# dwang0721/SfM-GMS

Hardware: AMD Instinct MI355X
Metric: gms_filtered_image_pairs_per_sec (higher is better)
Workload: dtype i32

## Files before the change

### include/gms.h

```cpp
#ifndef MI355_GMS_H
#define MI355_GMS_H

#include <stddef.h>
#include <stdint.h>

#ifdef __cplusplus
extern "C" {
#endif

#define GMS_OK             0
#define GMS_ERR_BAD_ARG   (-1)
#define GMS_ERR_DOMAIN    (-2)
#define GMS_ERR_HIP       (-3)
#define GMS_ERR_NO_DEVICE (-4)
#define GMS_ERR_CAPACITY  (-5)
#define GMS_ERR_IO        (-7)
#define GMS_ERR_NO_MODEL  (-8)
#define GMS_ERR_NOT_RESERVED (-6)


typedef struct gms_keypoint {
    float x, y;
    float size;
    float angle;
    float response;
    int32_t octave;
    int32_t class_id;
} gms_keypoint;

typedef struct gms_dmatch {
    int32_t queryIdx;
    int32_t trainIdx;
    int32_t imgIdx;
    float   distance;
} gms_dmatch;

typedef struct gms_pair {
    int32_t frame_a;
    int32_t frame_b;
    int32_t m;
    int32_t reserved;
    int64_t match_off;
} gms_pair;

typedef struct gms_pair_result {
    int32_t n_inliers;
    int32_t best_scale;
    int32_t best_rot;
    int32_t status;
} gms_pair_result;

typedef struct gms_ctx gms_ctx;

int gms_match(const gms_keypoint* kp1, int n1, int w1, int h1,
              const gms_keypoint* kp2, int n2, int w2, int h2,
              const gms_dmatch* matches, int m,
              int with_rotation, int with_scale, double threshold_factor,
              gms_dmatch* out, int* n_out);

int gms_match_ctx(gms_ctx* ctx,
                  const gms_keypoint* kp1, int n1, int w1, int h1,
                  const gms_keypoint* kp2, int n2, int w2, int h2,
                  const gms_dmatch* matches, int m,
                  int with_rotation, int with_scale, double threshold_factor,
                  gms_dmatch* out, int* n_out, gms_pair_result* result);

int  gms_ctx_create(int device, gms_ctx** out_ctx);
int  gms_ctx_destroy(gms_ctx* ctx);
int  gms_ctx_set_stream(gms_ctx* ctx, void* hip_stream);
int  gms_ctx_synchronize(gms_ctx* ctx);
int  gms_ctx_reserve(gms_ctx* ctx, int n_pairs, int max_m, int with_rotation, int with_scale);
#define GMS_QUERY_LAST_DEALT        1
#define GMS_QUERY_LAST_SCALE_PROBE  2
#define GMS_QUERY_LAST_KPT          3
#define GMS_QUERY_LAUNCHES          4
#define GMS_QUERY_CUS               5
#define GMS_QUERY_PREFETCH_TYPE     6
#define GMS_QUERY_PREFETCH_AHEAD    7
#define GMS_QUERY_STAGGER_TICKS     8
int  gms_ctx_query(gms_ctx* ctx, int what, int64_t* value);
#define GMS_OPTION_DEAL         1
#define GMS_OPTION_SCALE_PROBE  2
int  gms_ctx_set_option(gms_ctx* ctx, int option, int value);

#define GMS_FRAME_TABLE_HEADER_BYTES 16
int64_t gms_frame_table_bytes(int64_t total_kp);
int gms_normalize_device(gms_ctx* ctx, const gms_keypoint* d_kp, const int64_t* d_frame_off,
                         const int32_t* d_wh, int n_frames, int64_t total_kp, float* d_pts);

int gms_filter_device(gms_ctx* ctx, const float* d_pts, const int64_t* d_frame_off, int n_frames,
                      const gms_pair* d_pairs, int n_pairs, int max_m,
                      const gms_dmatch* d_matches,
                      int with_rotation, int with_scale, double threshold_factor,
                      gms_dmatch* d_out, gms_pair_result* d_results, uint8_t* d_mask);

int gms_filter_host_batch(gms_ctx* ctx, const gms_keypoint* kp, const int64_t* frame_off, const int32_t* wh,
                          int n_frames, const gms_pair* pairs, int n_pairs, const gms_dmatch* matches,
                          int with_rotation, int with_scale, double threshold_factor,
                          gms_dmatch* out, gms_pair_result* results);

#define GMS_DESC_NONE      (-1)
#define GMS_DESC_HAMMING256  0
#define GMS_DESC_L2_F32X128  1
int64_t gms_bf_prepared_bytes(int desc_kind, int64_t total_desc, int n_frames);
int gms_bf_prepare_device(gms_ctx* ctx, int desc_kind, const void* d_desc, const int64_t* d_frame_off, int n_frames,
                          int64_t total_desc, void* d_prepared);
int gms_bfmatch_device(gms_ctx* ctx, int desc_kind, const void* d_desc, const void* d_prepared, int64_t total_desc,
                       const int64_t* d_frame_off, int n_frames, const gms_pair* d_pairs, int n_pairs, int max_query,
                       gms_dmatch* d_matches);

typedef struct gms_bf_result {
    int64_t n_candidates;
    int64_t n_ratio;
    int64_t n_out;
    float   d_min;
    int32_t status;
} gms_bf_result;

size_t gms_bf_select_workspace_bytes(int n_pairs, int max_rows, int64_t total_backward_rows);
int gms_bf_select_device(gms_ctx* ctx, int desc_kind, const void* d_desc, const void* d_prepared, int64_t total_desc,
                         const int64_t* d_frame_off, int n_frames, const gms_pair* d_pairs, int n_pairs, int max_rows, int cross_check,
                         double distance_coef, int max_size, void* d_ws, size_t ws_bytes, gms_dmatch* d_out, gms_bf_result* d_bf_results,
                         gms_pair_result* d_pair_results);
int gms_bf_match_select(int desc_kind, const void* desc1, int n1, const void* desc2, int n2, int cross_check, double distance_coef,
                        int max_size, gms_dmatch* out, int64_t out_cap, int64_t* n_out, gms_bf_result* result);
int gms_bf_select_host_batch(gms_ctx* ctx, int desc_kind, const void* desc, const int64_t* frame_off, int n_frames, const gms_pair* pairs,
                             int n_pairs, int cross_check, double distance_coef, int max_size, gms_dmatch* out, gms_bf_result* results);

typedef struct gms_disparity_stats {
    int64_t count;
    int64_t sum_sq;
    int32_t max_abs;
    int32_t status;
} gms_disparity_stats;
int gms_disparity_device(gms_ctx* ctx, const gms_keypoint* d_kp1, int n1, const gms_keypoint* d_kp2, int n2,
                         const gms_dmatch* d_matches, const int32_t* d_n_matches, int max_matches, int width, int height,
                         const uint8_t* d_gt, int disp_ratio, uint8_t* d_disparity, uint32_t* d_work,
                         gms_disparity_stats* d_stats);
int gms_gather_points_device(gms_ctx* ctx, const gms_keypoint* d_kp1, int n1, const gms_keypoint* d_kp2, int n2,
                             const gms_dmatch* d_matches, const int32_t* d_n_matches, int max_matches,
                             float* d_coords1, float* d_coords2, int32_t* d_status);

typedef struct gms_triangulation_stats {
    double  sum_sq_err1, sum_sq_err2;
    int64_t count, behind;
} gms_triangulation_stats;
int gms_triangulate_device(gms_ctx* ctx, const double camera[4], const double dist[5], const double P1[12], const double P2[12],
                           const float* d_coords1, const float* d_coords2, const int32_t* d_n_matches, int max_matches,
                           double* d_points3d, gms_triangulation_stats* d_stats);

typedef struct gms_pose {
    double  R[9], t[3];
    int32_t n_good, which;
} gms_pose;
int gms_recover_pose_device(gms_ctx* ctx, const double E[9], const double camera[4], const float* d_coords1, const float* d_coords2,
                            const int32_t* d_n_matches, int max_matches, const uint8_t* d_in_mask, gms_pose* d_pose,
                            uint8_t* d_out_mask);

typedef struct gms_camera {
    double fx, fy, cx, cy;
    double k1, k2, p1, p2, k3;
} gms_camera;
typedef struct gms_two_view {
    double  E[9];
    double  R[9], t[3];
    double  sum_sq_err1, sum_sq_err2;
    int64_t n_finite, n_behind;
    int32_t n_points;
    int32_t n_ransac;
    int32_t ransac_iters;
    int32_t n_pose;
    int32_t pose_which;
    int32_t n_triangulated;
    int32_t status;
    int32_t reserved;
} gms_two_view;
int gms_gather_points_batch_device(gms_ctx* ctx, const gms_keypoint* d_kp, const int64_t* d_frame_off, int n_frames,
                                   const gms_pair* d_pairs, int n_pairs, int max_m, const gms_dmatch* d_filtered,
                                   const gms_pair_result* d_results, float* d_coords1, float* d_coords2, gms_two_view* d_tv);
int gms_find_essential_batch_device(gms_ctx* ctx, const gms_camera* camera, double prob, double threshold, int max_iters,
                                    const gms_pair* d_pairs, int n_pairs, const float* d_coords1, const float* d_coords2,
                                    uint8_t* d_mask, gms_two_view* d_tv);
int gms_recover_pose_batch_device(gms_ctx* ctx, const gms_camera* camera, int use_in_mask, const gms_pair* d_pairs, int n_pairs,
                                  const float* d_coords1, const float* d_coords2, uint8_t* d_mask, gms_two_view* d_tv);
int gms_triangulate_batch_device(gms_ctx* ctx, const gms_camera* camera, const gms_pair* d_pairs, int n_pairs,
                                 const float* d_coords1, const float* d_coords2, const uint8_t* d_mask, double* d_points3d,
                                 gms_two_view* d_tv);
int gms_two_view_batch_device(gms_ctx* ctx, const gms_camera* camera, double prob, double threshold, int max_iters,
                              const gms_keypoint* d_kp, const int64_t* d_frame_off, int n_frames, const gms_pair* d_pairs, int n_pairs,
                              int max_m, const gms_dmatch* d_filtered, const gms_pair_result* d_results, float* d_coords1,
                              float* d_coords2, uint8_t* d_mask, double* d_points3d, gms_two_view* d_tv);
int gms_disparity_batch_device(gms_ctx* ctx, const gms_keypoint* d_kp, const int64_t* d_frame_off, const int32_t* d_wh, int n_frames,
                               const gms_pair* d_pairs, int n_pairs, int max_m, const gms_dmatch* d_filtered,
                               const gms_pair_result* d_results, const uint8_t* d_gt, int64_t gt_stride, int disp_ratio,
                               uint8_t* d_disparity, int64_t map_stride, uint32_t* d_work, gms_disparity_stats* d_stats);

#define GMS_SFM_SKIPPED 1
typedef struct gms_sfm_plan_entry {
    int32_t registers;
    int32_t link;
    int32_t role;
    int32_t depth;
} gms_sfm_plan_entry;
typedef struct gms_sfm_view {
    double  R[9], t[3];
    int32_t registered;
    int32_t pair;
} gms_sfm_view;
typedef struct gms_sfm_pair_reg {
    double  r, S;
    int32_t n_links;
    int32_t depth, link, role;
    int32_t status;
    int32_t reserved;
} gms_sfm_pair_reg;
typedef struct gms_sfm_summary {
    int64_t n_tracks;
    int64_t n_points;
    int64_t n_multi;
    int32_t n_registered;
    int32_t n_ok_pairs;
} gms_sfm_summary;
int gms_sfm_plan(const gms_pair* pairs, int n_pairs, int n_frames, int root, gms_sfm_plan_entry* plan);
size_t gms_sfm_register_workspace_bytes(int n_frames, int n_pairs, int64_t total_kp, int64_t total_matches);
int gms_sfm_register_device(gms_ctx* ctx, const int64_t* d_frame_off, int n_frames, int64_t total_kp, const gms_pair* d_pairs,
                            const gms_sfm_plan_entry* d_plan, int n_pairs, int max_m, int64_t total_matches, const gms_dmatch* d_filtered,
                            const uint8_t* d_mask, const double* d_points3d, const gms_two_view* d_tv, int root, int min_links,
                            void* d_ws, size_t ws_bytes, gms_sfm_view* d_views, gms_sfm_pair_reg* d_reg, double* d_points_world,
                            int32_t* d_track, int64_t cloud_cap, double* d_cloud, int32_t* d_cloud_id, int32_t* d_cloud_obs,
                            int32_t* d_cloud_est, double* d_cloud_spread, gms_sfm_summary* d_summary);
int gms_sfm_register(const int64_t* frame_off, int n_frames, const gms_pair* pairs, int n_pairs, const gms_dmatch* filtered,
                     const uint8_t* mask, const double* points3d, const gms_two_view* tv, int root, int min_links, gms_sfm_view* views,
                     gms_sfm_pair_reg* reg, double* points_world, int32_t* track, int64_t cloud_cap, double* cloud, int32_t* cloud_id,
                     int32_t* cloud_obs, int32_t* cloud_est, double* cloud_spread, gms_sfm_summary* summary);

typedef struct gms_sfm_ba_params {
    double  lambda0, cg_tol, ftol, huber_px;
    int32_t n_iters, n_cg, retriangulate;
    int32_t reserved;
} gms_sfm_ba_params;
typedef struct gms_sfm_ba_summary {
// ... 265 lines not shown
```

### sfm-gms_amd/api.py

```python
import ctypes as C

import numpy as np

from .capi import load_library
from .types import (BF_RESULT_DTYPE, DMATCH_DTYPE, LOGOS_DICT_RESULT_DTYPE, KEYPOINT_DTYPE, PAIR_DTYPE, RESULT_DTYPE, GMS_OK, GMS_ERR_CAPACITY,
                    GmsError, SFM_PAIR_REG_DTYPE, SFM_PLAN_DTYPE, SFM_SUMMARY_DTYPE, SFM_VIEW_DTYPE, TWO_VIEW_DTYPE, concat_frames, desc_layout,
                    portrait_params, stereo_bm_params, stereo_sgm_params, GMS_ERR_BAD_ARG, RECTIFY_PLAN_DTYPE, STEREO_SGM_DENSE, RectifyPlan,
                    make_camera, rectify_plan_records)


def _as(arr, dtype, name):
    a = np.ascontiguousarray(arr)
    if a.dtype != dtype:
        raise TypeError(f"{name} must have dtype {dtype}, got {a.dtype}")
    return a


def _check(rc, lib, what):
    if rc != GMS_OK:
        msg = lib.gms_error_string(rc).decode()
        if rc == -3:
            msg += f" (hipError {lib.gms_last_hip_error()})"
        raise GmsError(rc, f"{what}: {msg}")


class GmsContext:

    def __init__(self, device=0):
        self._lib = load_library()
        h = C.c_void_p()
        _check(self._lib.gms_ctx_create(int(device), C.byref(h)), self._lib, "gms_ctx_create")
        self._h = h
        self.device = int(device)

    def close(self):
        if getattr(self, "_h", None):
            self._lib.gms_ctx_destroy(self._h)
            self._h = None

    def __del__(self):
        try:
            self.close()
        except Exception:
            pass

    def __enter__(self):
        return self

    def __exit__(self, *exc):
        self.close()

    @property
    def max_matches(self):
        return int(self._lib.gms_max_matches())

    def set_stream(self, hip_stream_handle):
        _check(self._lib.gms_ctx_set_stream(self._h, C.c_void_p(hip_stream_handle or 0)), self._lib, "set_stream")

    def synchronize(self):
        _check(self._lib.gms_ctx_synchronize(self._h), self._lib, "synchronize")

    def set_option(self, option, value):
        _check(self._lib.gms_ctx_set_option(self._h, int(option), int(value)), self._lib, "gms_ctx_set_option")

    def query(self, what):
        v = C.c_int64(0)
        _check(self._lib.gms_ctx_query(self._h, int(what), C.byref(v)), self._lib, "gms_ctx_query")
        return int(v.value)

    def match(self, size1, size2, keypoints1, keypoints2, matches1to2, withRotation=False, withScale=False,
              thresholdFactor=6.0, return_result=False):
        kp1 = _as(keypoints1, KEYPOINT_DTYPE, "keypoints1")
        kp2 = _as(keypoints2, KEYPOINT_DTYPE, "keypoints2")
        mt = _as(matches1to2, DMATCH_DTYPE, "matches1to2")
        out = np.empty(max(len(mt), 1), dtype=DMATCH_DTYPE)
        n_out = C.c_int(0)
        res = np.zeros(1, dtype=RESULT_DTYPE)
        rc = self._lib.gms_match_ctx(self._h, kp1.ctypes.data, len(kp1), int(size1[0]), int(size1[1]),
                                     kp2.ctypes.data, len(kp2), int(size2[0]), int(size2[1]),
                                     mt.ctypes.data, len(mt), int(bool(withRotation)), int(bool(withScale)),
                                     float(thresholdFactor), out.ctypes.data, C.byref(n_out), res.ctypes.data)
        _check(rc, self._lib, "gms_match_ctx")
        kept = out[: n_out.value].copy()
        return (kept, res[0]) if return_result else kept

    def filter_host_batch(self, keypoints_per_frame, sizes, pairs, matches, withRotation=False, withScale=False,
                          thresholdFactor=6.0, out=None, results=None):
        if isinstance(keypoints_per_frame, tuple):
            kp, frame_off = keypoints_per_frame
            n_kp = len(kp)
            kp = _as(kp, KEYPOINT_DTYPE, "keypoints") if n_kp else np.zeros(1, dtype=KEYPOINT_DTYPE)
            frame_off = np.ascontiguousarray(frame_off, dtype=np.int64)
            n_frames = len(np.asarray(sizes).reshape(-1, 2))
            if (frame_off.shape != (n_frames + 1,) or frame_off[0] != 0 or (np.diff(frame_off) < 0).any()
                    or frame_off[-1] > n_kp):
                raise ValueError("frame_off: one offset per frame and one more, from 0, never decreasing, the last at most len(keypoints)")
        else:
            kp, frame_off = concat_frames([_as(k, KEYPOINT_DTYPE, "keypoints") for k in keypoints_per_frame])
            kp = kp if len(kp) else np.zeros(1, dtype=KEYPOINT_DTYPE)
            n_frames = len(frame_off) - 1
        wh = np.ascontiguousarray(np.asarray(sizes, dtype=np.int32).reshape(-1, 2))
        if wh.shape[0] != n_frames:
            raise ValueError("one (width, height) per frame")
        pairs = _as(pairs, PAIR_DTYPE, "pairs")
        mt = _as(matches, DMATCH_DTYPE, "matches")
        if out is None:
            out = np.zeros(max(len(mt), 1), dtype=DMATCH_DTYPE)
        if results is None:
            results = np.zeros(max(len(pairs), 1), dtype=RESULT_DTYPE)
        if (out.dtype != DMATCH_DTYPE or results.dtype != RESULT_DTYPE or len(out) < len(mt) or len(results) < len(pairs)
                or not out.flags["C_CONTIGUOUS"] or not results.flags["C_CONTIGUOUS"]):
            raise ValueError("out / results: contiguous DMATCH_DTYPE / RESULT_DTYPE arrays of at least len(matches) / len(pairs)")
        rc = self._lib.gms_filter_host_batch(self._h, kp.ctypes.data, frame_off.ctypes.data, wh.ctypes.data, n_frames,
                                             pairs.ctypes.data, len(pairs), mt.ctypes.data, int(bool(withRotation)),
                                             int(bool(withScale)), float(thresholdFactor), out.ctypes.data, results.ctypes.data)
        _check(rc, self._lib, "gms_filter_host_batch")
        return out[: len(mt)], results[: len(pairs)]

    def reserve(self, n_pairs, max_m, withRotation=False, withScale=False):
        _check(self._lib.gms_ctx_reserve(self._h, int(n_pairs), int(max_m), int(bool(withRotation)), int(bool(withScale))),
               self._lib, "gms_ctx_reserve")

    def frame_table_bytes(self, total_kp):
        return int(self._lib.gms_frame_table_bytes(int(total_kp)))

    def normalize_device(self, d_kp, d_frame_off, d_wh, n_frames, total_kp, d_pts):
        _check(self._lib.gms_normalize_device(self._h, d_kp, d_frame_off, d_wh, int(n_frames), int(total_kp), d_pts),
               self._lib, "gms_normalize_device")

    def filter_device(self, d_pts, d_frame_off, n_frames, d_pairs, n_pairs, max_m, d_matches, d_out, d_results,
                      d_mask=None, withRotation=False, withScale=False, thresholdFactor=6.0):
        _check(self._lib.gms_filter_device(self._h, d_pts, d_frame_off, int(n_frames), d_pairs, int(n_pairs),
                                           int(max_m), d_matches, int(bool(withRotation)), int(bool(withScale)),
                                           float(thresholdFactor), d_out, d_results, d_mask or None),
               self._lib, "gms_filter_device")

    def bf_prepared_bytes(self, desc_kind, total_desc, n_frames):
        return int(self._lib.gms_bf_prepared_bytes(int(desc_kind), int(total_desc), int(n_frames)))

    def bf_prepare_device(self, desc_kind, d_desc, d_frame_off, n_frames, total_desc, d_prepared):
        _check(self._lib.gms_bf_prepare_device(self._h, int(desc_kind), d_desc, d_frame_off, int(n_frames), int(total_desc),
                                               d_prepared or None), self._lib, "gms_bf_prepare_device")

    def bfmatch_device(self, desc_kind, d_desc, d_prepared, total_desc, d_frame_off, n_frames, d_pairs, n_pairs, max_query,
                       d_matches):
        _check(self._lib.gms_bfmatch_device(self._h, int(desc_kind), d_desc, d_prepared or None, int(total_desc), d_frame_off,
                                            int(n_frames), d_pairs, int(n_pairs), int(max_query), d_matches),
               self._lib, "gms_bfmatch_device")

    def bf_select_workspace_bytes(self, n_pairs, max_rows, total_backward_rows):
        return int(self._lib.gms_bf_select_workspace_bytes(int(n_pairs), int(max_rows), int(total_backward_rows)))

    def bf_select_device(self, desc_kind, d_desc, d_prepared, total_desc, d_frame_off, n_frames, d_pairs, n_pairs, max_rows, cross_check,
                         distance_coef, max_size, d_ws, ws_bytes, d_out, d_bf_results, d_pair_results=None):
        _check(self._lib.gms_bf_select_device(self._h, int(desc_kind), d_desc or None, d_prepared or None, int(total_desc), d_frame_off,
                                              int(n_frames), d_pairs, int(n_pairs), int(max_rows), int(bool(cross_check)),
                                              float(distance_coef), int(max_size), d_ws, int(ws_bytes), d_out, d_bf_results,
                                              d_pair_results or None), self._lib, "gms_bf_select_device")

    def disparity_device(self, d_kp1, n1, d_kp2, n2, d_matches, d_n_matches, max_matches, width, height, d_gt, disp_ratio,
                         d_disparity, d_work, d_stats):
        _check(self._lib.gms_disparity_device(self._h, d_kp1, int(n1), d_kp2, int(n2), d_matches, d_n_matches, int(max_matches),
                                              int(width), int(height), d_gt or None, int(disp_ratio), d_disparity, d_work,
                                              d_stats), self._lib, "gms_disparity_device")

    def gather_points_device(self, d_kp1, n1, d_kp2, n2, d_matches, d_n_matches, max_matches, d_coords1, d_coords2, d_status):
        _check(self._lib.gms_gather_points_device(self._h, d_kp1, int(n1), d_kp2, int(n2), d_matches, d_n_matches,
                                                  int(max_matches), d_coords1, d_coords2, d_status),
               self._lib, "gms_gather_points_device")

    def triangulate_device(self, camera, dist, P1, P2, d_coords1, d_coords2, d_n_matches, max_matches, d_points3d, d_stats):
        cam = np.ascontiguousarray(camera, dtype=np.float64).reshape(4)
        dc = None if dist is None else np.ascontiguousarray(dist, dtype=np.float64).reshape(5)
        p1 = np.ascontiguousarray(P1, dtype=np.float64).reshape(12)
        p2 = np.ascontiguousarray(P2, dtype=np.float64).reshape(12)
        _check(self._lib.gms_triangulate_device(self._h, cam.ctypes.data, None if dc is None else dc.ctypes.data, p1.ctypes.data,
                                                p2.ctypes.data, d_coords1, d_coords2, d_n_matches, int(max_matches), d_points3d,
                                                d_stats), self._lib, "gms_triangulate_device")

    def recover_pose_device(self, E, camera, d_coords1, d_coords2, d_n_matches, max_matches, d_in_mask, d_pose, d_out_mask):
        e = np.ascontiguousarray(E, dtype=np.float64).reshape(9)
        cam = np.ascontiguousarray(camera, dtype=np.float64).reshape(4)
        _check(self._lib.gms_recover_pose_device(self._h, e.ctypes.data, cam.ctypes.data, d_coords1, d_coords2, d_n_matches,
                                                 int(max_matches), d_in_mask, d_pose, d_out_mask), self._lib, "gms_recover_pose_device")

    def gather_points_batch_device(self, d_kp, d_frame_off, n_frames, d_pairs, n_pairs, max_m, d_filtered, d_results, d_coords1,
                                   d_coords2, d_tv):
        _check(self._lib.gms_gather_points_batch_device(self._h, d_kp, d_frame_off, int(n_frames), d_pairs, int(n_pairs), int(max_m),
                                                        d_filtered, d_results, d_coords1, d_coords2, d_tv),
               self._lib, "gms_gather_points_batch_device")

    def find_essential_batch_device(self, camera, d_pairs, n_pairs, d_coords1, d_coords2, d_mask, d_tv, prob=0.999, threshold=1.0,
                                    max_iters=1000):
        _check(self._lib.gms_find_essential_batch_device(self._h, camera.ctypes.data, float(prob), float(threshold), int(max_iters),
                                                         d_pairs, int(n_pairs), d_coords1, d_coords2, d_mask, d_tv),
               self._lib, "gms_find_essential_batch_device")

    def recover_pose_batch_device(self, camera, d_pairs, n_pairs, d_coords1, d_coords2, d_mask, d_tv, use_in_mask=True):
        _check(self._lib.gms_recover_pose_batch_device(self._h, camera.ctypes.data, int(bool(use_in_mask)), d_pairs, int(n_pairs),
                                                       d_coords1, d_coords2, d_mask, d_tv), self._lib, "gms_recover_pose_batch_device")

    def triangulate_batch_device(self, camera, d_pairs, n_pairs, d_coords1, d_coords2, d_mask, d_points3d, d_tv):
        _check(self._lib.gms_triangulate_batch_device(self._h, camera.ctypes.data, d_pairs, int(n_pairs), d_coords1, d_coords2,
                                                      d_mask or None, d_points3d, d_tv), self._lib, "gms_triangulate_batch_device")

    def two_view_batch_device(self, camera, d_kp, d_frame_off, n_frames, d_pairs, n_pairs, max_m, d_filtered, d_results, d_coords1,
                              d_coords2, d_mask, d_points3d, d_tv, prob=0.999, threshold=1.0, max_iters=1000):
        _check(self._lib.gms_two_view_batch_device(self._h, camera.ctypes.data, float(prob), float(threshold), int(max_iters), d_kp,
                                                   d_frame_off, int(n_frames), d_pairs, int(n_pairs), int(max_m), d_filtered, d_results,
                                                   d_coords1, d_coords2, d_mask, d_points3d, d_tv), self._lib, "gms_two_view_batch_device")

    def disparity_batch_device(self, d_kp, d_frame_off, d_wh, n_frames, d_pairs, n_pairs, max_m, d_filtered, d_results, d_gt, gt_stride,
                               disp_ratio, d_disparity, map_stride, d_work, d_stats):
        _check(self._lib.gms_disparity_batch_device(self._h, d_kp, d_frame_off, d_wh, int(n_frames), d_pairs, int(n_pairs), int(max_m),
                                                    d_filtered, d_results, d_gt or None, int(gt_stride), int(disp_ratio), d_disparity,
                                                    int(map_stride), d_work, d_stats), self._lib, "gms_disparity_batch_device")

    def sfm_register_workspace_bytes(self, n_frames, n_pairs, total_kp, total_matches):
        return int(self._lib.gms_sfm_register_workspace_bytes(int(n_frames), int(n_pairs), int(total_kp), int(total_matches)))

    def sfm_register_device(self, d_frame_off, n_frames, total_kp, d_pairs, d_plan, n_pairs, max_m, total_matches, d_filtered, d_mask,
                            d_points3d, d_tv, root, min_links, d_ws, ws_bytes, d_views, d_reg, d_points_world, d_track, cloud_cap, d_cloud,
                            d_cloud_id, d_cloud_obs, d_cloud_est, d_cloud_spread, d_summary):
        _check(self._lib.gms_sfm_register_device(self._h, d_frame_off, int(n_frames), int(total_kp), d_pairs, d_plan, int(n_pairs), int(max_m),
                                                 int(total_matches), d_filtered, d_mask, d_points3d, d_tv, int(root), int(min_links), d_ws,
                                                 int(ws_bytes), d_views, d_reg, d_points_world, d_track, int(cloud_cap), d_cloud, d_cloud_id,
                                                 d_cloud_obs, d_cloud_est, d_cloud_spread, d_summary), self._lib, "gms_sfm_register_device")

    def sfm_ba_workspace_bytes(self, n_frames, n_pairs, total_kp, cloud_cap):
        return int(self._lib.gms_sfm_ba_workspace_bytes(int(n_frames), int(n_pairs), int(total_kp), int(cloud_cap)))

    def sfm_ba_device(self, camera, params, d_kp, d_frame_off, n_frames, total_kp, d_pairs, n_pairs, total_matches, d_filtered, d_mask, d_views,
                      d_reg, d_track, cloud_cap, d_cloud, d_cloud_id, d_reg_summary, d_ws, ws_bytes, d_views_out, d_cloud_out, d_track_status,
                      d_summary):
        _check(self._lib.gms_sfm_ba_device(self._h, None if camera is None else camera.ctypes.data, None if params is None else params.ctypes.data,
                                           d_kp, d_frame_off, int(n_frames), int(total_kp), d_pairs, int(n_pairs), int(total_matches), d_filtered,
                                           d_mask, d_views, d_reg, d_track, int(cloud_cap), d_cloud, d_cloud_id, d_reg_summary, d_ws, int(ws_bytes),
                                           d_views_out, d_cloud_out, d_track_status, d_summary), self._lib, "gms_sfm_ba_device")

    def detect_workspace_bytes(self, width, height, n_images, max_keypoints):
        return int(self._lib.gms_detect_workspace_bytes(int(width), int(height), int(n_images), int(max_keypoints)))

    def detect_batch_device(self, d_images, n_images, width, height, threshold, max_keypoints, d_ws, ws_bytes, d_kp, d_desc, d_counts):
        _check(self._lib.gms_detect_batch_device(self._h, d_images, int(n_images), int(width), int(height), int(threshold), int(max_keypoints),
                                                 d_ws, int(ws_bytes), d_kp, d_desc, d_counts), self._lib, "gms_detect_batch_device")

    def describe_device(self, d_image, width, height, d_kp, n, d_ws, ws_bytes, d_desc, d_status):
        _check(self._lib.gms_describe_device(self._h, d_image, int(width), int(height), d_kp, int(n), d_ws, int(ws_bytes), d_desc, d_status),
               self._lib, "gms_describe_device")

    def pyramid_level_sizes(self, width, height, n_levels):
        n_levels = int(n_levels)
        ww, hh = np.zeros(max(n_levels, 1), np.int32), np.zeros(max(n_levels, 1), np.int32)
        n = self._lib.gms_pyramid_level_sizes(int(width), int(height), n_levels, ww.ctypes.data, hh.ctypes.data)
        _check(min(n, 0), self._lib, "gms_pyramid_level_sizes")
        return [(int(ww[l]), int(hh[l])) for l in range(n)]

    def detect_pyramid_workspace_bytes(self, width, height, n_images, max_keypoints, n_levels):
        return int(self._lib.gms_detect_pyramid_workspace_bytes(int(width), int(height), int(n_images), int(max_keypoints), int(n_levels)))

    def detect_pyramid_batch_device(self, d_images, n_images, width, height, threshold, max_keypoints, n_levels, d_ws, ws_bytes, d_kp, d_desc,
                                    d_counts, d_level_counts):
        _check(self._lib.gms_detect_pyramid_batch_device(self._h, d_images, int(n_images), int(width), int(height), int(threshold),
                                                         int(max_keypoints), int(n_levels), d_ws, int(ws_bytes), d_kp, d_desc, d_counts,
                                                         d_level_counts), self._lib, "gms_detect_pyramid_batch_device")

    def pyramid_build_device(self, d_images, n_images, width, height, n_levels, d_levels, levels_bytes):
        _check(self._lib.gms_pyramid_build_device(self._h, d_images, int(n_images), int(width), int(height), int(n_levels), d_levels,
                                                  int(levels_bytes)), self._lib, "gms_pyramid_build_device")

    def detect_pyramid_grad_workspace_bytes(self, width, height, n_images, max_keypoints, n_levels):
        return int(self._lib.gms_detect_pyramid_grad_workspace_bytes(int(width), int(height), int(n_images), int(max_keypoints), int(n_levels)))

    def detect_pyramid_grad_batch_device(self, d_images, n_images, width, height, threshold, max_keypoints, n_levels, d_ws, ws_bytes, d_kp,
                                         d_desc, d_counts, d_level_counts, d_rows128):
        _check(self._lib.gms_detect_pyramid_grad_batch_device(self._h, d_images, int(n_images), int(width), int(height), int(threshold),
                                                              int(max_keypoints), int(n_levels), d_ws, int(ws_bytes), d_kp, d_desc, d_counts,
                                                              d_level_counts, d_rows128), self._lib, "gms_detect_pyramid_grad_batch_device")

    def describe_grad_device(self, d_image, width, height, d_kp, n, d_ws, ws_bytes, d_rows128, d_status):
        _check(self._lib.gms_describe_grad_device(self._h, d_image, int(width), int(height), d_kp, int(n), d_ws, int(ws_bytes), d_rows128,
                                                  d_status), self._lib, "gms_describe_grad_device")
# ... 712 lines not shown
```

### sfm-gms_amd/capi.py

```python
import ctypes as C
import os

_HERE = os.path.dirname(os.path.abspath(__file__))

vp, i32, i64, u64, sz, dbl, cstr, P = C.c_void_p, C.c_int, C.c_int64, C.c_uint64, C.c_size_t, C.c_double, C.c_char_p, C.POINTER

SIGNATURES = {
    "gms_match": (i32, [vp, i32, i32, i32, vp, i32, i32, i32, vp, i32, i32, i32, dbl, vp, P(i32)]),
    "gms_match_ctx": (i32, [vp, vp, i32, i32, i32, vp, i32, i32, i32, vp, i32, i32, i32, dbl, vp, P(i32), vp]),
    "gms_ctx_create": (i32, [i32, P(vp)]),
    "gms_ctx_destroy": (i32, [vp]),
    "gms_ctx_set_stream": (i32, [vp, vp]),
    "gms_ctx_synchronize": (i32, [vp]),
    "gms_ctx_reserve": (i32, [vp, i32, i32, i32, i32]),
    "gms_ctx_query": (i32, [vp, i32, P(i64)]),
    "gms_ctx_set_option": (i32, [vp, i32, i32]),
    "gms_frame_table_bytes": (i64, [i64]),
    "gms_normalize_device": (i32, [vp, vp, vp, vp, i32, i64, vp]),
    "gms_filter_device": (i32, [vp, vp, vp, i32, vp, i32, i32, vp, i32, i32, dbl, vp, vp, vp]),
    "gms_filter_host_batch": (i32, [vp, vp, vp, vp, i32, vp, i32, vp, i32, i32, dbl, vp, vp]),
    "gms_bf_prepared_bytes": (i64, [i32, i64, i32]),
    "gms_bf_prepare_device": (i32, [vp, i32, vp, vp, i32, i64, vp]),
    "gms_bfmatch_device": (i32, [vp, i32, vp, vp, i64, vp, i32, vp, i32, i32, vp]),
    "gms_disparity_device": (i32, [vp, vp, i32, vp, i32, vp, vp, i32, i32, i32, vp, i32, vp, vp, vp]),
    "gms_gather_points_device": (i32, [vp, vp, i32, vp, i32, vp, vp, i32, vp, vp, vp]),
    "gms_triangulate_device": (i32, [vp, vp, vp, vp, vp, vp, vp, vp, i32, vp, vp]),
    "gms_recover_pose_device": (i32, [vp, vp, vp, vp, vp, vp, i32, vp, vp, vp]),
    "gms_gather_points_batch_device": (i32, [vp, vp, vp, i32, vp, i32, i32, vp, vp, vp, vp, vp]),
    "gms_find_essential_batch_device": (i32, [vp, vp, dbl, dbl, i32, vp, i32, vp, vp, vp, vp]),
    "gms_recover_pose_batch_device": (i32, [vp, vp, i32, vp, i32, vp, vp, vp, vp]),
    "gms_triangulate_batch_device": (i32, [vp, vp, vp, i32, vp, vp, vp, vp, vp]),
    "gms_two_view_batch_device": (i32, [vp, vp, dbl, dbl, i32, vp, vp, i32, vp, i32, i32, vp, vp, vp, vp, vp, vp, vp]),
    "gms_disparity_batch_device": (i32, [vp, vp, vp, vp, i32, vp, i32, i32, vp, vp, vp, i64, i32, vp, i64, vp, vp]),
    "gms_sfm_plan": (i32, [vp, i32, i32, i32, vp]),
    "gms_sfm_register_workspace_bytes": (sz, [i32, i32, i64, i64]),
    "gms_sfm_register_device": (i32, [vp, vp, i32, i64, vp, vp, i32, i32, i64, vp, vp, vp, vp, i32, i32, vp, sz, vp, vp, vp, vp, i64, vp, vp, vp,
                                      vp, vp, vp]),
    "gms_sfm_register": (i32, [vp, i32, vp, i32, vp, vp, vp, vp, i32, i32, vp, vp, vp, vp, i64, vp, vp, vp, vp, vp, vp]),
    "gms_sfm_ba_workspace_bytes": (sz, [i32, i32, i64, i64]),
    "gms_sfm_ba_device": (i32, [vp, vp, vp, vp, vp, i32, i64, vp, i32, i64, vp, vp, vp, vp, vp, i64, vp, vp, vp, vp, sz, vp, vp, vp, vp]),
    "gms_sfm_ba": (i32, [vp, vp, vp, vp, i32, vp, i32, vp, vp, vp, vp, vp, i64, vp, vp, i64, vp, vp, vp, vp]),
    "gms_dataset_write": (i32, [cstr, vp]),
    "gms_dataset_read": (i32, [cstr, vp]),
    "gms_dataset_free": (None, [vp]),
    "gms_max_matches": (i32, []),
    "gms_last_hip_error": (i32, []),
    "gms_error_string": (cstr, [i32]),
    "gms_version": (cstr, []),
    "gms_selftest_threshold": (i32, [vp, vp, vp, vp, dbl, i32, vp]),
    "gms_selftest_five_point": (i32, [vp, vp, i32, vp, vp]),
    "gms_detect_workspace_bytes": (sz, [i32, i32, i32, i32]),
    "gms_detect_batch_device": (i32, [vp, vp, i32, i32, i32, i32, i32, vp, sz, vp, vp, vp]),
    "gms_describe_device": (i32, [vp, vp, i32, i32, vp, i32, vp, sz, vp, vp]),
    "gms_logos_match": (i32, [vp, i32, vp, i32, vp, vp, vp, i64, P(i64), vp]),
    "gms_logos_table_bytes": (i64, [i64, i32, i32]),
    "gms_logos_workspace_bytes": (sz, [i64, i32, i64]),
    "gms_logos_prepare_device": (i32, [vp, vp, vp, i32, i64, vp, i32, vp, sz, vp]),
    "gms_logos_filter_device": (i32, [vp, vp, vp, i32, vp, sz, vp, vp, vp]),
    "gms_logos_words_device": (i32, [vp, i32, vp, i64, vp, i32, vp]),
    "gms_logos_host_batch": (i32, [vp, vp, vp, i32, vp, i32, vp, i32, vp, vp]),
    "gms_bf_select_workspace_bytes": (sz, [i32, i32, i64]),
    "gms_bf_select_device": (i32, [vp, i32, vp, vp, i64, vp, i32, vp, i32, i32, i32, dbl, i32, vp, sz, vp, vp, vp]),
    "gms_bf_match_select": (i32, [i32, vp, i32, vp, i32, i32, dbl, i32, vp, i64, P(i64), vp]),
    "gms_bf_select_host_batch": (i32, [vp, i32, vp, vp, i32, vp, i32, i32, dbl, i32, vp, vp]),
    "gms_stereo_bm_workspace_bytes": (sz, [i32, i32, i32, vp]),
    "gms_stereo_bm_device": (i32, [vp, vp, vp, vp, i32, i32, i32, i32, vp, sz, vp, vp]),
    "gms_stereo_bm_normalize_device": (i32, [vp, vp, i32, i32, i32, vp]),
    "gms_stereo_bm": (i32, [vp, vp, vp, i32, i32, i32, vp, vp, vp]),
    "gms_stereo_sgm_workspace_bytes": (sz, [i32, i32, i32, vp]),
    "gms_stereo_sgm_device": (i32, [vp, vp, vp, vp, i32, i32, i32, i32, vp, sz, vp, vp]),
    "gms_stereo_sgm": (i32, [vp, vp, vp, i32, i32, i32, vp, vp, vp]),
    "gms_portrait_workspace_bytes": (sz, [i32, i32, i32, vp]),
    "gms_portrait_device": (i32, [vp, vp, vp, vp, i32, i32, i32, i32, i32, vp, sz, vp, vp, vp, vp]),
    "gms_median_blur_device": (i32, [vp, vp, i32, i32, i32, i32, i32, i32, vp]),
    "gms_portrait": (i32, [vp, vp, vp, i32, i32, vp, vp, vp, vp]),
    "gms_portrait_profile_device": (i32, [vp, vp, vp, vp, i32, i32, i32, i32, i32, vp, sz, vp, vp, vp, vp, vp]),
    "gms_median_blur": (i32, [vp, i32, i32, i32, i32, vp]),
    "gms_resize_device": (i32, [vp, vp, i32, i32, i32, i32, i32, vp, i32, i32, i32]),
    "gms_warp_affine_device": (i32, [vp, vp, i32, i32, i32, i32, i32, vp, i32, vp, i32, i32, i32]),
    "gms_rotation_matrix_2d": (i32, [dbl, dbl, dbl, dbl, vp]),
    "gms_resize": (i32, [vp, i32, i32, i32, vp, i32, i32]),
    "gms_warp_affine": (i32, [vp, i32, i32, i32, vp, vp, i32, i32]),
    "gms_img_rotate": (i32, [vp, i32, i32, i32, dbl, vp]),
    "gms_rectify_plan_host": (i32, [vp, vp, vp, i32, i32, i32, i32, vp]),
    "gms_rectify_plan_device": (i32, [vp, vp, vp, i32, i32, i32, i32, i32, vp]),
    "gms_rectify_q": (i32, [vp, vp]),
    "gms_rectify_device": (i32, [vp, vp, vp, i32, i32, i32, i32, i32, vp, i32, i32, vp, i32, i32, i32, vp]),
    "gms_rectify": (i32, [vp, vp, i32, vp, i32, i32, i32, vp, vp]),
    "gms_undistort": (i32, [vp, vp, i32, i32, i32, vp]),
    "gms_dense_cloud_workspace_bytes": (sz, [i32, i32, i32]),
    "gms_dense_cloud_device": (i32, [vp, vp, vp, vp, i32, i32, i32, i32, i32, vp, i32, i32, vp, vp, vp, i32, vp, sz, i32, vp, vp, vp, vp]),
    "gms_dense_pairs_workspace_bytes": (sz, [i32, i32, i32, i32, i32, i32, vp]),
    "gms_dense_pairs_device": (i32, [vp, vp, vp, vp, vp, i32, i32, i32, i32, vp, i32, i32, i32, vp, vp, vp, i32, vp, sz, vp, vp, vp, vp, vp, vp,
                                     i32, vp, vp, vp, vp]),
    "gms_dense_pair": (i32, [vp, vp, vp, vp, i32, i32, i32, vp, vp, i32, i32, i32, vp, vp, vp, vp, vp, vp, i32, vp, vp, vp, vp]),
    "gms_chess_candidates_workspace_bytes": (sz, [i32, i32, i32]),
    "gms_chess_candidates_device": (i32, [vp, vp, i32, i32, i32, i32, vp, sz, vp, vp]),
    "gms_corner_subpix_device": (i32, [vp, vp, i32, i32, i32, vp, vp, i32, i32, i32, dbl, vp]),
    "gms_find_chessboard_corners": (i32, [vp, i32, i32, i32, i32, vp, vp]),
    "gms_order_chessboard": (i32, [vp, i32, i32, vp, vp]),
    "gms_corner_subpix": (i32, [vp, i32, i32, vp, i32, i32, i32, dbl, vp]),
    "gms_calibrate_camera": (i32, [vp, vp, vp, i32, i32, i32, vp, vp, vp, vp, vp]),
    "gms_pyramid_level_sizes": (i32, [i32, i32, i32, vp, vp]),
    "gms_detect_pyramid_workspace_bytes": (sz, [i32, i32, i32, i32, i32]),
    "gms_detect_pyramid_batch_device": (i32, [vp, vp, i32, i32, i32, i32, i32, i32, vp, sz, vp, vp, vp, vp]),
    "gms_pyramid_build_device": (i32, [vp, vp, i32, i32, i32, i32, vp, sz]),
    "gms_detect_pyramid_grad_workspace_bytes": (sz, [i32, i32, i32, i32, i32]),
    "gms_detect_pyramid_grad_batch_device": (i32, [vp, vp, i32, i32, i32, i32, i32, i32, vp, sz, vp, vp, vp, vp, vp]),
    "gms_describe_grad_device": (i32, [vp, vp, i32, i32, vp, i32, vp, sz, vp, vp]),
    "gms_detect_dog_workspace_bytes": (sz, [i32, i32, i32, i32, i32]),
    "gms_detect_dog_batch_device": (i32, [vp, vp, i32, i32, i32, i32, i32, i32, vp, sz, vp, vp, vp, vp, vp]),
    "gms_dog_candidates_device": (i32, [vp, vp, i32, i32, i32, i32, vp]),
    "gms_detect_dog_refined_workspace_bytes": (sz, [i32, i32, i32, i32, i32]),
    "gms_detect_dog_refined_batch_device": (i32, [vp, vp, i32, i32, i32, i32, i32, i32, vp, sz, vp, vp, vp, vp, vp]),
    "gms_dog_offsets_device": (i32, [vp, vp, i32, i32, i32, i32, vp]),
    "gms_bgr_to_gray_device": (i32, [vp, vp, i32, i32, i32, vp]),
    "gms_detect_pack_device": (i32, [vp, vp, vp, vp, vp, i32, i32, vp, vp, vp, vp]),
    "gms_logos_dict_workspace_bytes": (sz, [i32, i64, i32, i32, i32, i32]),
    "gms_logos_dict_train_device": (i32, [vp, i32, vp, vp, i32, i64, i32, i32, i32, u64, vp, sz, vp, vp, vp]),
    "gms_logos_dict_train": (i32, [i32, vp, vp, i32, i32, i32, i32, u64, vp, vp, vp]),
}
EXPORTED_SYMBOLS = list(SIGNATURES)

_lib = None


def library_path():
    return os.path.join(_HERE, "csrc", "libgms_hip.so")


def load_library():
    global _lib
    if _lib is not None:
        return _lib
    path = library_path()
    if not os.path.exists(path):
        raise ImportError(f"{path} not found: the HIP extension is not built "
                          f"(run `python -c 'import __graft_entry__ as g; g.build()'`)")
    try:
        import torch
    except ImportError:
        pass
    lib = C.CDLL(path)
    for name, (restype, argtypes) in SIGNATURES.items():
        fn = getattr(lib, name)
        fn.restype, fn.argtypes = restype, argtypes
    _lib = lib
    return lib
```

### sfm-gms_amd/csrc/gms_capi.cpp

```cpp
#include <hip/hip_runtime.h>

#include <algorithm>
#include <atomic>
#include <cmath>
#include <condition_variable>
#include <cstdio>
#include <cstddef>
#include <cstdlib>
#include <cstring>
#include <mutex>
#include <new>
#include <thread>
#include <vector>

#include "block_layout.h"
#include "copy_pool.h"
#include "gms.h"
#include "gms_kernels.h"
#include "logos_batch.h"
#include "logos_dict_core.h"
#include "portrait_core.h"
#include "stereo_bm_core.h"
#include "sfm_ba_core.h"
#include "sfm_register_core.h"
#include "stereo_sgm_core.h"
#include "twoview_core.h"
#include "rectify_core.h"
#include "warp_core.h"
#include "calib_core.h"

static_assert(sizeof(gms_keypoint) == 28, "gms_keypoint must match cv::KeyPoint (stride 0x1c)");
static_assert(sizeof(gms_dmatch) == 16, "gms_dmatch must match cv::DMatch (stride 0x10)");
static_assert(sizeof(gms_pair) == 24, "gms_pair layout");
static_assert(sizeof(gms_pair_result) == 16, "gms_pair_result layout");
static_assert(sizeof(gms_two_view) == 232 && sizeof(gms_camera) == 72, "two-view records");

static thread_local int t_last_hip = 0;
namespace gms {
void record_hip_error(int e) { t_last_hip = e; }
}
#ifdef GMS_PHASE_TIMING
static unsigned long long* g_diag = nullptr;
extern "C" int gms_diag_set_buffer(void* d_buf) { g_diag = (unsigned long long*)d_buf; return 0; }
#endif

#define GMS_HIP(call)                         \
    do {                                      \
        hipError_t e_ = (call);               \
        if (e_ != hipSuccess) {               \
            t_last_hip = (int)e_;             \
            return GMS_ERR_HIP;               \
        }                                     \
    } while (0)
#define GMS_TRY(call)                \
    do {                             \
        const int rc_ = (call);      \
        if (rc_ != GMS_OK) return rc_; \
    } while (0)

namespace {

struct Knobs {
    bool dense_on = true, band_on = true, stream_on = true;
    int probe_nibble = 16;
    bool probe_nibble_set = false;
    int stagger_us = -1, deal = -1, scale_probe = -1, check_pairs = -1;
    int prefetch_type = 3, prefetch_ahead = 0;
    size_t band_ws_budget = (size_t)4 << 30;
};
const Knobs& knobs()
{
    static const Knobs k = [] {
        Knobs v;
        if (const char* e = std::getenv("GMS_DENSE")) v.dense_on = std::atoi(e) != 0;
        if (const char* e = std::getenv("GMS_BAND")) v.band_on = std::atoi(e) != 0;
        if (const char* e = std::getenv("GMS_STREAM")) v.stream_on = std::atoi(e) != 0;
        if (const char* e = std::getenv("GMS_PROBE_NIBBLE")) { v.probe_nibble = (int)std::strtol(e, nullptr, 0) & 24; v.probe_nibble_set = true; }
        if (const char* e = std::getenv("GMS_STAGGER_US")) v.stagger_us = std::atoi(e);
        if (const char* e = std::getenv("GMS_DEAL")) v.deal = std::atoi(e) != 0 ? 1 : 0;
        if (const char* e = std::getenv("GMS_SCALE_PROBE")) v.scale_probe = std::atoi(e) != 0 ? 1 : 0;
        if (const char* e = std::getenv("GMS_CHECK_PAIRS")) v.check_pairs = std::atoi(e) != 0 ? 1 : 0;
        if (const char* e = std::getenv("GMS_PREFETCH")) {
            v.prefetch_type = std::atoi(e);
            if (const char* comma = std::strchr(e, ',')) v.prefetch_ahead = std::atoi(comma + 1);
        }
        if (const char* e = std::getenv("GMS_BAND_WS_BYTES")) {
            const long long b = std::atoll(e);
            if (b > 0) v.band_ws_budget = (size_t)b;
        }
        return v;
    }();
    return k;
}

void right_grids(int rw[5], int rh[5])
{
    const double ratio[5] = {1.0, 1.0 / 2, 1.0 / std::sqrt(2.0), std::sqrt(2.0), 2.0};
    for (int s = 0; s < 5; ++s) {
        rw[s] = (int)std::lrint(gms::kLeftW * ratio[s]);
        rh[s] = (int)std::lrint(gms::kLeftH * ratio[s]);
    }
}

inline hipError_t device_alloc(void** p, size_t bytes) { return hipMalloc(p, bytes); }
inline hipError_t pinned_alloc(void** p, size_t bytes) { return hipHostMalloc(p, bytes, hipHostMallocDefault); }

template <hipError_t (*Alloc)(void**, size_t), hipError_t (*Free)(void*), size_t kMin>
struct GrowBuf {
    void* p = nullptr;
    size_t cap = 0;
    hipError_t reserve(size_t bytes)
    {
        if (bytes <= cap) return hipSuccess;
        release();
        const size_t want = bytes < kMin ? kMin : bytes + bytes / 4;
        const hipError_t e = Alloc(&p, want);
        if (e == hipSuccess) cap = want;
        return e;
    }
    void release()
    {
        if (p) (void)Free(p);
        p = nullptr;
        cap = 0;
    }
};
using DevBuf = GrowBuf<device_alloc, hipFree, 4096>;
using PinBuf = GrowBuf<pinned_alloc, hipHostFree, 65536>;

struct WsNeed {
    size_t partial = 0, big = 0, band = 0;
    size_t slice = 0, per_pair = 0;
    int kpt = 0, mcap = 0;
    bool stream = false;
};

}

struct Lane {
    hipStream_t stream = nullptr;
    PinBuf hin, hout;
    DevBuf din, dout;
    hipEvent_t ev_res = nullptr, ev_out = nullptr;
};

struct gms_ctx {
    int device = 0;
    hipStream_t own_stream = nullptr;
    hipStream_t stream = nullptr;
    std::mutex mu;
    DevBuf aux, big_ws, band_ws, partial_ws, pose_ws;
    uint32_t* verdict = nullptr;
    unsigned dense_launches = 0;
    int use_dealt = 0, use_probe = 0x1D | (16 << 8), last_dealt = 0, last_probe = 0, last_kpt = 0, last_stagger_ticks = 0;
    hipEvent_t verdict_event = nullptr;
    bool verdict_pending = false;
    unsigned filter_launches = 0;
    uint32_t overflow_seen = 0;
    int stream_penalty = 0;
    int opt_deal = -1, opt_probe = -1;
    DevBuf probe_stats;
    unsigned scale_launches = 0;
    hipEvent_t ws_event = nullptr;
    hipStream_t ws_stream = nullptr;
    bool ws_pending = false;
    Lane lane[3];
    gms::CopyPool* pool = nullptr;
    DevBuf tab_kp, tab_pts, tab_small;
    int n_cus = 256;
};

namespace {

int plan_workspace(const gms_ctx* c, int n_pairs, int max_m, bool rot, bool scale, bool need_mask_ws, bool allow_stream, WsNeed* w)
{
    *w = WsNeed();
    w->kpt = gms::filter_pick_kpt(max_m);
    if (w->kpt) {
        if (scale && knobs().dense_on) w->partial = (size_t)n_pairs * gms::kPartialStrideDw * 4;
        return GMS_OK;
    }
    if (max_m > gms::kBigMaxMatches) return GMS_ERR_CAPACITY;
    w->mcap = gms::big_mcap(max_m);
    const int n_wg = n_pairs < c->n_cus ? n_pairs : c->n_cus;
    w->big = (size_t)n_wg * gms::big_ws_stride_dwords(w->mcap) * 4;
    if (knobs().band_on) {
        gms::FilterParams p{};
        p.with_rotation = rot;
        p.with_scale = scale;
        right_grids(p.right_w, p.right_h);
        w->stream = knobs().stream_on && max_m <= gms::stream_max_matches() && allow_stream;
        w->per_pair = w->stream ? std::max(gms::stream_ws_bytes_per_pair(p, w->mcap, need_mask_ws), scale ? (size_t)0 : gms::stream_dense_ws_bytes_per_pair(w->mcap))
                                : (!rot && !scale) ? gms::band_ws_bytes_per_pair(w->mcap, need_mask_ws)
                                                   : gms::tile_ws_bytes_per_pair(p, w->mcap, need_mask_ws);
        size_t slice = knobs().band_ws_budget / w->per_pair;
        if (slice < 1) slice = 1;
        if (slice > (size_t)n_pairs) slice = (size_t)n_pairs;
        w->slice = slice;
        w->band = slice * w->per_pair;
    }
    return GMS_OK;
}

int grow_workspace(gms_ctx* c, const WsNeed& w, hipStream_t st)
{
    if (w.partial <= c->partial_ws.cap && w.big <= c->big_ws.cap && w.band <= c->band_ws.cap) return GMS_OK;
    hipStreamCaptureStatus cs = hipStreamCaptureStatusNone;
    if (hipStreamIsCapturing(st, &cs) == hipSuccess && cs != hipStreamCaptureStatusNone) return GMS_ERR_NOT_RESERVED;
    GMS_HIP(hipStreamSynchronize(st));
    if (c->ws_pending) {
        GMS_HIP(hipEventSynchronize(c->ws_event));
        c->ws_pending = false;
    }
    GMS_HIP(c->partial_ws.reserve(w.partial));
    GMS_HIP(c->big_ws.reserve(w.big));
    GMS_HIP(c->band_ws.reserve(w.band));
    return GMS_OK;
}

int grow_pose_ws(gms_ctx* c, size_t bytes, hipStream_t st)
{
    if (bytes <= c->pose_ws.cap) return GMS_OK;
    hipStreamCaptureStatus cs = hipStreamCaptureStatusNone;
    if (hipStreamIsCapturing(st, &cs) == hipSuccess && cs != hipStreamCaptureStatusNone) return GMS_ERR_NOT_RESERVED;
    GMS_HIP(hipStreamSynchronize(st));
    GMS_HIP(hipDeviceSynchronize());
    GMS_HIP(c->pose_ws.reserve(bytes));
    return GMS_OK;
}

int filter_launch(gms_ctx* c, hipStream_t st, const float* d_pts, const int64_t* d_frame_off, int n_frames,
                  const gms_pair* d_pairs, int n_pairs, int max_m, const gms_dmatch* d_matches,
                  int with_rotation, int with_scale, double threshold_factor,
                  gms_dmatch* d_out, gms_pair_result* d_results, uint8_t* d_mask, bool validate_pairs = true)
{
    if (n_pairs < 0 || max_m < 0 || n_frames < 0) return GMS_ERR_BAD_ARG;
    if (n_pairs == 0) return GMS_OK;
    if (!d_frame_off || !d_pairs || !d_results) return GMS_ERR_BAD_ARG;
    if (max_m > 0 && (!d_matches || !d_out || !d_pts)) return GMS_ERR_BAD_ARG;
    hipStreamCaptureStatus cs = hipStreamCaptureStatusNone;
    const bool capturing = hipStreamIsCapturing(st, &cs) == hipSuccess && cs != hipStreamCaptureStatusNone;
    if (gms::filter_pick_kpt(max_m) == 0 && !capturing) {
        const uint32_t now = ((volatile uint32_t*)c->verdict)[2];
        if (now != c->overflow_seen) {
            c->overflow_seen = now;
            c->stream_penalty = 64;
        } else if (c->stream_penalty > 0) {
            --c->stream_penalty;
        }
    }
    WsNeed w;
    GMS_TRY(plan_workspace(c, n_pairs, max_m, with_rotation != 0, with_scale != 0, d_mask == nullptr, c->stream_penalty == 0, &w));
    GMS_TRY(grow_workspace(c, w, st));
    const bool uses_ws = w.partial || w.big || w.band;
    if (uses_ws && !capturing && c->ws_pending && c->ws_stream != st) GMS_HIP(hipStreamWaitEvent(st, c->ws_event, 0));

    gms::FilterParams p{};
    const int kpt = w.kpt;
    p.table_slots = kpt ? gms::filter_table_slots(kpt) : 0;
    p.region_shift = kpt ? gms::filter_region_shift(kpt) : 0;
    p.pts = reinterpret_cast<const float2*>(reinterpret_cast<const char*>(d_pts) + gms::kTableHeaderBytes);
    p.frame_off = d_frame_off;
    p.n_frames = n_frames;
    p.pairs = d_pairs;
    p.n_pairs = n_pairs;
    p.stagger_blocks = c->n_cus;
    p.prefetch_type = knobs().prefetch_type;
    p.prefetch_ahead = knobs().prefetch_ahead > 0 ? knobs().prefetch_ahead : c->n_cus;
    p.matches = d_matches;
    p.out = d_out;
    p.results = d_results;
    p.mask = d_mask;
    p.with_rotation = with_rotation ? 1 : 0;
    p.with_scale = with_scale ? 1 : 0;
    p.threshold_factor = threshold_factor;
    p.pair_flags = nullptr;
    p.partial = nullptr;
    p.dealt = 0;
    right_grids(p.right_w, p.right_h);
    p.dense = (knobs().dense_on && !with_scale) ? 1 : 0;
    if (c->verdict_pending && !capturing && hipEventQuery(c->verdict_event) == hipSuccess) {
        c->use_dealt = c->verdict[0] != 0u ? 1 : 0;
        c->use_probe = (int)c->verdict[1];
        c->verdict_pending = false;
    }
    const int force_deal = c->opt_deal >= 0 ? c->opt_deal : knobs().deal, force_probe = c->opt_probe >= 0 ? c->opt_probe : knobs().scale_probe;
    const bool scales_matrix = kpt && with_scale && knobs().dense_on;
    p.dealt = ((p.dense || scales_matrix) && kpt && (force_deal >= 0 ? force_deal != 0 : c->use_dealt != 0)) ? 1 : 0;
    const bool scales_on_matrix = with_scale && knobs().dense_on;
    p.stagger_ticks = 0;
    if (n_pairs >= 4 * p.stagger_blocks && kpt && max_m >= 2048) {
        const double us10k = knobs().stagger_us >= 0 ? (double)knobs().stagger_us : (scales_on_matrix ? 0.0 : p.dense ? 16.0 : 72.0);
        p.stagger_ticks = (int)(us10k * 100.0 * max_m / 10000.0);
    }
#ifdef GMS_PHASE_TIMING
    p.diag = g_diag;
#endif
    p.probe_scales = 0;
    p.probe_stats = nullptr;
    {
        void* dflag = nullptr;
        p.overflow_events = hipHostGetDevicePointer(&dflag, c->verdict, 0) == hipSuccess ? (uint32_t*)dflag + 2 : nullptr;
    }
    if (kpt && with_scale) {
        const bool measuring = force_probe < 0 && !capturing && (c->scale_launches++ & 15u) == 0u;
        const int all = 0x1D | (24 << 8);
        const int mask = force_probe >= 0 ? (force_probe != 0 ? 0x1D | (knobs().probe_nibble << 8) : 0) : (measuring ? all : c->use_probe);
        p.probe_scales = mask & 0x1D;
        p.probe_nibble = (mask >> 8) & 24 & (knobs().probe_nibble_set ? knobs().probe_nibble : 24);
        p.probe_stats = measuring ? (uint32_t*)c->probe_stats.p : nullptr;
    }
    if (kpt && with_scale && knobs().dense_on) {
        p.partial = (uint32_t*)c->partial_ws.p;
        GMS_HIP(gms::launch_filter_scales(p, kpt, n_pairs, st));
        if (!capturing && p.probe_stats == nullptr && (c->dense_launches++ & 15u) == 0u) {
            void* dflag = nullptr;
            GMS_HIP(hipHostGetDevicePointer(&dflag, c->verdict, 0));
            GMS_HIP(gms::launch_order_probe(p, (uint32_t*)dflag, st));
            GMS_HIP(hipEventRecord(c->verdict_event, st));
            c->verdict_pending = true;
        }
        if (p.probe_stats != nullptr) {
            void* dflag = nullptr;
            GMS_HIP(hipHostGetDevicePointer(&dflag, c->verdict, 0));
            GMS_HIP(gms::launch_probe_verdict(p.probe_stats, (uint32_t*)dflag + 1, st));
            GMS_HIP(hipEventRecord(c->verdict_event, st));
            c->verdict_pending = true;
        }
    } else if (kpt) {
        GMS_HIP(gms::launch_filter(p, kpt, n_pairs, st));
        if (p.dense && !capturing && (c->dense_launches++ & 15u) == 0u) {
            void* dflag = nullptr;
            GMS_HIP(hipHostGetDevicePointer(&dflag, c->verdict, 0));
            GMS_HIP(gms::launch_order_probe(p, (uint32_t*)dflag, st));
            GMS_HIP(hipEventRecord(c->verdict_event, st));
            c->verdict_pending = true;
        }
    } else if (knobs().band_on) {
        const bool plain = !with_rotation && !with_scale;
        for (int s0 = 0; s0 < n_pairs; s0 += (int)w.slice) {
            gms::FilterParams ps = p;
            ps.pairs = d_pairs + s0;
            ps.results = d_results + s0;
            ps.n_pairs = (n_pairs - s0 < (int)w.slice) ? n_pairs - s0 : (int)w.slice;
            const uint32_t* flags = nullptr;
            if (w.stream && (with_scale || ps.n_pairs < c->n_cus)) GMS_HIP(gms::launch_filter_stream(ps, w.mcap, c->band_ws.p, &flags, st));
            else if (w.stream) GMS_HIP(gms::launch_filter_stream_dense(ps, w.mcap, c->band_ws.p, &flags, st));
            else if (plain) GMS_HIP(gms::launch_filter_band(ps, w.mcap, c->band_ws.p, &flags, st));
            else GMS_HIP(gms::launch_filter_tiles(ps, w.mcap, c->band_ws.p, &flags, st));
            ps.pair_flags = flags;
            const int wg = ps.n_pairs < c->n_cus ? ps.n_pairs : c->n_cus;
            GMS_HIP(gms::launch_filter_big(ps, w.mcap, wg, (uint32_t*)c->big_ws.p, st));
        }
    } else {
        const int n_wg = n_pairs < c->n_cus ? n_pairs : c->n_cus;
        GMS_HIP(gms::launch_filter_big(p, w.mcap, n_wg, (uint32_t*)c->big_ws.p, st));
    }
    c->last_dealt = p.dealt;
    c->last_probe = p.probe_scales | (p.probe_scales ? p.probe_nibble << 8 : 0);
    c->last_kpt = kpt;
    c->last_stagger_ticks = p.stagger_ticks;
    if (validate_pairs && n_pairs > 1 && !capturing && knobs().check_pairs != 0 && (knobs().check_pairs == 1 || (c->filter_launches & 15u) == 0u))
        GMS_HIP(gms::launch_check_pairs(d_pairs, n_pairs, d_results, (uint32_t*)c->probe_stats.p + 16 + (c->filter_launches & 7u), st));
    if (!capturing) ++c->filter_launches;
    if (uses_ws && !capturing) {
        GMS_HIP(hipEventRecord(c->ws_event, st));
        c->ws_stream = st;
        c->ws_pending = true;
    }
    return GMS_OK;
}

size_t align16(size_t x) { return (x + 15) & ~(size_t)15; }

using gms::CopyJob;
using gms::CopyPool;
using gms::pack_xy;

bool desc_kind_ok(int kind) { return kind == GMS_DESC_HAMMING256 || kind == GMS_DESC_L2_F32X128; }
size_t desc_row_bytes(int kind) { return kind == GMS_DESC_HAMMING256 ? 32 : 512; }

template <class Launch>
int on_ctx(gms_ctx* c, Launch&& launch)
{
    std::lock_guard<std::mutex> lock(c->mu);
    GMS_HIP(hipSetDevice(c->device));
    GMS_HIP(launch());
    return GMS_OK;
}

class DevBlock {
public:
    DevBlock(const gms::BlockLayout& layout, hipStream_t stream) : st_(stream) { err_ = hipMalloc(&p_, layout.total()); }
    ~DevBlock() { release(); }
    DevBlock(const DevBlock&) = delete;
    DevBlock& operator=(const DevBlock&) = delete;

    template <class T = void>
    T* at(size_t offset) const { return reinterpret_cast<T*>(static_cast<char*>(p_) + offset); }
    bool ok() const { return err_ == hipSuccess; }
    template <class Launch>
    void run(Launch&& launch)
    {
        if (!ok()) return;
        busy_ = true;
        err_ = launch(st_);
    }
    void in(size_t offset, const void* src, size_t bytes) { run([&](hipStream_t st) { return hipMemcpyAsync(at(offset), src, bytes, hipMemcpyHostToDevice, st); }); }
    void out(void* dst, size_t offset, size_t bytes) { run([&](hipStream_t st) { return hipMemcpyAsync(dst, at(offset), bytes, hipMemcpyDeviceToHost, st); }); }
    void sync() { wait([&] { return hipStreamSynchronize(st_); }); }
    void out_now(void* dst, size_t offset, size_t bytes) { wait([&] { return hipMemcpy(dst, at(offset), bytes, hipMemcpyDeviceToHost); }); }
    int finish()
    {
        release();
        GMS_HIP(err_);
        return GMS_OK;
    }

private:
    template <class Wait>
    void wait(Wait&& w)
    {
        if (ok()) err_ = w();
        busy_ = !ok();
    }
    void release()
    {
        if (!p_) return;
        if (busy_) {
            const hipError_t e = hipStreamSynchronize(st_);
            if (ok()) err_ = e;
        }
        (void)hipFree(p_);
        p_ = nullptr;
    }
    void* p_ = nullptr;
    hipStream_t st_;
    hipError_t err_;
    bool busy_ = false;
};

}

extern "C" {

const char* gms_version(void) { return "mi355-gms 0.2 (gfx950)"; }

int gms_last_hip_error(void) { return t_last_hip; }

const char* gms_error_string(int code)
{
    switch (code) {
    case GMS_OK: return "ok";
    case GMS_ERR_BAD_ARG: return "bad argument";
    case GMS_ERR_DOMAIN: return "input outside the domain on which the reference is defined";
    case GMS_ERR_HIP: return "HIP runtime error";
    case GMS_ERR_NO_DEVICE: return "no usable HIP device";
    case GMS_ERR_CAPACITY: return "too many matches per pair for this build";
    case GMS_ERR_IO: return "dataset file: cannot open, truncated, or not a GMSFRM01 file";
    case GMS_ERR_NO_MODEL: return "two-view stage: too few correspondences, or no essential matrix / pose found";
    case GMS_ERR_NOT_RESERVED: return "workspace not reserved for this shape (stream capture in progress)";
    default: return "unknown error";
    }
}

int gms_max_matches(void) { return gms::kBigMaxMatches; }

int gms_ctx_create(int device, gms_ctx** out_ctx)
{
    if (!out_ctx) return GMS_ERR_BAD_ARG;
    *out_ctx = nullptr;
    int n = 0;
    hipError_t e = hipGetDeviceCount(&n);
    if (e != hipSuccess || n <= 0) {
        t_last_hip = (int)e;
        return GMS_ERR_NO_DEVICE;
    }
    if (device < 0 || device >= n) return GMS_ERR_BAD_ARG;
    GMS_HIP(hipSetDevice(device));
    gms_ctx* c = new (std::nothrow) gms_ctx;
    if (!c) return GMS_ERR_BAD_ARG;
    c->device = device;
    const int rc = [c] {
        GMS_HIP(hipStreamCreateWithFlags(&c->own_stream, hipStreamNonBlocking));
        GMS_HIP(hipStreamCreateWithFlags(&c->lane[1].stream, hipStreamNonBlocking));
        GMS_HIP(hipStreamCreateWithFlags(&c->lane[2].stream, hipStreamNonBlocking));
        for (Lane& l : c->lane) {
            GMS_HIP(hipEventCreateWithFlags(&l.ev_res, hipEventDisableTiming));
            GMS_HIP(hipEventCreateWithFlags(&l.ev_out, hipEventDisableTiming));
        }
        GMS_HIP(hipEventCreateWithFlags(&c->ws_event, hipEventDisableTiming));
        GMS_HIP(hipEventCreateWithFlags(&c->verdict_event, hipEventDisableTiming));
        GMS_HIP(hipHostMalloc((void**)&c->verdict, 64, hipHostMallocDefault));
        c->verdict[0] = 0;
        c->verdict[1] = 0x1D | (16 << 8);
        c->verdict[2] = 0;
        GMS_HIP(c->probe_stats.reserve(128));
        GMS_HIP(hipMemset(c->probe_stats.p, 0, 128));
        GMS_HIP(gms::init_filter_kernels());
        GMS_HIP(gms::init_band_kernels());
        GMS_HIP(gms::init_stream_kernels());
        GMS_HIP(gms::init_big_kernels());
        return GMS_OK;
    }();
    if (rc != GMS_OK) {
        if (c->own_stream) (void)hipStreamDestroy(c->own_stream);
        if (c->lane[1].stream) (void)hipStreamDestroy(c->lane[1].stream);
        if (c->lane[2].stream) (void)hipStreamDestroy(c->lane[2].stream);
        for (Lane& l : c->lane) {
            if (l.ev_res) (void)hipEventDestroy(l.ev_res);
            if (l.ev_out) (void)hipEventDestroy(l.ev_out);
        }
        if (c->ws_event) (void)hipEventDestroy(c->ws_event);
        if (c->verdict_event) (void)hipEventDestroy(c->verdict_event);
        if (c->verdict) (void)hipHostFree(c->verdict);
        c->probe_stats.release();
        delete c;
        return rc;
    }
    c->stream = c->own_stream;
    hipDeviceProp_t prop;
    if (hipGetDeviceProperties(&prop, device) == hipSuccess && prop.multiProcessorCount > 0) c->n_cus = prop.multiProcessorCount;
    *out_ctx = c;
    return GMS_OK;
}

int gms_ctx_destroy(gms_ctx* c)
{
    if (!c) return GMS_OK;
    {
        std::lock_guard<std::mutex> lock(c->mu);
        (void)hipSetDevice(c->device);
        (void)hipStreamSynchronize(c->stream);
        (void)hipStreamSynchronize(c->own_stream);
        (void)hipStreamSynchronize(c->lane[1].stream);
        (void)hipStreamSynchronize(c->lane[2].stream);
        if (c->ws_pending) (void)hipEventSynchronize(c->ws_event);
        DevBuf* bufs[] = {&c->aux, &c->big_ws, &c->band_ws, &c->partial_ws, &c->pose_ws, &c->probe_stats, &c->tab_kp, &c->tab_pts, &c->tab_small};
        if (c->verdict) (void)hipHostFree(c->verdict);
        for (DevBuf* b : bufs) b->release();
        for (Lane& l : c->lane) {
            l.hin.release();
            l.hout.release();
            l.din.release();
            l.dout.release();
            (void)hipEventDestroy(l.ev_res);
            (void)hipEventDestroy(l.ev_out);
        }
        delete c->pool;
        c->pool = nullptr;
        (void)hipStreamDestroy(c->lane[1].stream);
        (void)hipStreamDestroy(c->lane[2].stream);
        (void)hipStreamDestroy(c->own_stream);
        (void)hipEventDestroy(c->ws_event);
        (void)hipEventDestroy(c->verdict_event);
    }
    delete c;
    return GMS_OK;
}

int gms_ctx_set_stream(gms_ctx* c, void* hip_stream)
{
    if (!c) return GMS_ERR_BAD_ARG;
    std::lock_guard<std::mutex> lock(c->mu);
    c->stream = hip_stream ? (hipStream_t)hip_stream : c->own_stream;
    return GMS_OK;
}

int gms_ctx_synchronize(gms_ctx* c)
{
    if (!c) return GMS_ERR_BAD_ARG;
    std::lock_guard<std::mutex> lock(c->mu);
    GMS_HIP(hipSetDevice(c->device));
    GMS_HIP(hipStreamSynchronize(c->stream));
    if (c->verdict_pending && hipEventQuery(c->verdict_event) == hipSuccess) {
        c->use_dealt = c->verdict[0] != 0u ? 1 : 0;
        c->use_probe = (int)c->verdict[1];
        c->verdict_pending = false;
    }
    return GMS_OK;
}

int gms_ctx_set_option(gms_ctx* c, int option, int value)
{
    if (!c || value < -1 || value > 1) return GMS_ERR_BAD_ARG;
    std::lock_guard<std::mutex> lock(c->mu);
    switch (option) {
    case GMS_OPTION_DEAL: c->opt_deal = value; return GMS_OK;
    case GMS_OPTION_SCALE_PROBE: c->opt_probe = value; return GMS_OK;
    default: return GMS_ERR_BAD_ARG;
    }
}

int gms_ctx_query(gms_ctx* c, int what, int64_t* value)
{
    if (!c || !value) return GMS_ERR_BAD_ARG;
    std::lock_guard<std::mutex> lock(c->mu);
    switch (what) {
    case GMS_QUERY_LAST_DEALT: *value = c->last_dealt; return GMS_OK;
    case GMS_QUERY_LAST_SCALE_PROBE: *value = c->last_probe; return GMS_OK;
    case GMS_QUERY_LAST_KPT: *value = c->last_kpt; return GMS_OK;
    case GMS_QUERY_LAUNCHES: *value = (int64_t)c->filter_launches; return GMS_OK;
    case GMS_QUERY_CUS: *value = c->n_cus; return GMS_OK;
    case GMS_QUERY_PREFETCH_TYPE: *value = knobs().prefetch_type; return GMS_OK;
    case GMS_QUERY_PREFETCH_AHEAD: *value = knobs().prefetch_ahead > 0 ? knobs().prefetch_ahead : c->n_cus; return GMS_OK;
    case GMS_QUERY_STAGGER_TICKS: *value = c->last_stagger_ticks; return GMS_OK;
    default: return GMS_ERR_BAD_ARG;
    }
}

int gms_ctx_reserve(gms_ctx* c, int n_pairs, int max_m, int with_rotation, int with_scale)
{
    if (!c || n_pairs < 0 || max_m < 0) return GMS_ERR_BAD_ARG;
    std::lock_guard<std::mutex> lock(c->mu);
    GMS_HIP(hipSetDevice(c->device));
    WsNeed w;
    GMS_TRY(plan_workspace(c, n_pairs, max_m, with_rotation != 0, with_scale != 0, true, true, &w));
    for (int variant = 1; variant < 4; ++variant) {
        WsNeed w2;
        GMS_TRY(plan_workspace(c, n_pairs, max_m, with_rotation != 0, with_scale != 0, (variant & 1) == 0, (variant & 2) == 0, &w2));
        w.band = std::max(w.band, w2.band);
    }
    GMS_TRY(grow_workspace(c, w, c->stream));
    return grow_pose_ws(c, (size_t)max_m + 48, c->stream);
}

int64_t gms_frame_table_bytes(int64_t total_kp) { return total_kp < 0 ? 0 : gms::kTableHeaderBytes + total_kp * 16 + 16; }

int gms_normalize_device(gms_ctx* c, const gms_keypoint* d_kp, const int64_t* d_frame_off,
                         const int32_t* d_wh, int n_frames, int64_t total_kp, float* d_pts)
{
    if (!c || n_frames < 0 || total_kp < 0) return GMS_ERR_BAD_ARG;
    if (total_kp == 0 || n_frames == 0) return GMS_OK;
    if (!d_kp || !d_frame_off || !d_wh || !d_pts) return GMS_ERR_BAD_ARG;
    return on_ctx(c, [&] { return gms::launch_normalize(d_kp, (int)sizeof(gms_keypoint), d_frame_off, d_wh, n_frames, total_kp, d_pts, c->stream); });
}

int gms_filter_device(gms_ctx* c, const float* d_pts, const int64_t* d_frame_off, int n_frames,
                      const gms_pair* d_pairs, int n_pairs, int max_m, const gms_dmatch* d_matches,
                      int with_rotation, int with_scale, double threshold_factor,
                      gms_dmatch* d_out, gms_pair_result* d_results, uint8_t* d_mask)
{
    if (!c) return GMS_ERR_BAD_ARG;
    std::lock_guard<std::mutex> lock(c->mu);
    GMS_HIP(hipSetDevice(c->device));
    return filter_launch(c, c->stream, d_pts, d_frame_off, n_frames, d_pairs, n_pairs, max_m, d_matches, with_rotation,
                         with_scale, threshold_factor, d_out, d_results, d_mask);
}

int gms_match_ctx(gms_ctx* c, const gms_keypoint* kp1, int n1, int w1, int h1,
                  const gms_keypoint* kp2, int n2, int w2, int h2, const gms_dmatch* matches, int m,
                  int with_rotation, int with_scale, double threshold_factor,
                  gms_dmatch* out, int* n_out, gms_pair_result* result)
{
    if (n_out) *n_out = 0;
    if (result) *result = gms_pair_result{0, -1, -1, GMS_OK};
    if (!c || !n_out) return GMS_ERR_BAD_ARG;
    if (n1 < 0 || n2 < 0 || m < 0 || w1 <= 0 || h1 <= 0 || w2 <= 0 || h2 <= 0) return GMS_ERR_BAD_ARG;
    if ((n1 > 0 && !kp1) || (n2 > 0 && !kp2) || (m > 0 && (!matches || !out))) return GMS_ERR_BAD_ARG;
    if (m > gms_max_matches()) return GMS_ERR_CAPACITY;

    std::lock_guard<std::mutex> lock(c->mu);
    GMS_HIP(hipSetDevice(c->device));
    hipStream_t st = c->stream;
    Lane& L = c->lane[0];
    struct alignas(8) CallHeader {
        int64_t foff[3];
        int32_t wh[4];
        gms_pair pair;
    };
    static_assert(sizeof(CallHeader) == 64 && offsetof(CallHeader, wh) == 24 && offsetof(CallHeader, pair) == 40, "header layout");
    const size_t nkp = (size_t)n1 + (size_t)n2;
    const size_t off_m = sizeof(CallHeader), off_xy = off_m + (size_t)m * sizeof(gms_dmatch);
    const size_t in_bytes = off_xy + nkp * 8;
    const size_t out_bytes = sizeof(gms_pair_result) + (size_t)m * sizeof(gms_dmatch);
    GMS_HIP(L.hin.reserve(in_bytes));
    GMS_HIP(L.hout.reserve(out_bytes));
    if (in_bytes > L.din.cap || out_bytes > L.dout.cap || (size_t)gms_frame_table_bytes((int64_t)nkp) > c->tab_pts.cap) GMS_HIP(hipDeviceSynchronize());
    GMS_HIP(L.din.reserve(in_bytes));
    GMS_HIP(L.dout.reserve(out_bytes));
    GMS_HIP(c->tab_pts.reserve((size_t)gms_frame_table_bytes((int64_t)nkp)));
    char* hin = (char*)L.hin.p;
    const CallHeader hdr = {{0, n1, (int64_t)n1 + n2}, {w1, h1, w2, h2}, {0, 1, m, 0, 0}};
    std::memcpy(hin, &hdr, sizeof hdr);
    if (m) std::memcpy(hin + off_m, matches, (size_t)m * sizeof(gms_dmatch));
    pack_xy(kp1, (size_t)n1, (float*)(hin + off_xy));
    pack_xy(kp2, (size_t)n2, (float*)(hin + off_xy) + 2 * (size_t)n1);
    const bool zero_copy = m <= 16384;
    const char* din = (const char*)L.din.p;
    char* dout = (char*)L.dout.p;
    if (zero_copy) {
        void *dev_in = nullptr, *dev_out = nullptr;
        GMS_HIP(hipHostGetDevicePointer(&dev_in, L.hin.p, 0));
        GMS_HIP(hipHostGetDevicePointer(&dev_out, L.hout.p, 0));
        din = (const char*)dev_in;
        dout = (char*)dev_out;
    } else {
        GMS_HIP(hipMemcpyAsync(L.din.p, hin, in_bytes, hipMemcpyHostToDevice, st));
    }
    const int64_t* d_foff = (const int64_t*)din;
    const int32_t* d_wh = (const int32_t*)(din + offsetof(CallHeader, wh));
    const gms_pair* d_pair = (const gms_pair*)(din + offsetof(CallHeader, pair));
    gms_pair_result* d_res = (gms_pair_result*)dout;
    gms_dmatch* d_out = (gms_dmatch*)(dout + sizeof(gms_pair_result));
    if (nkp) GMS_HIP(gms::launch_normalize(din + off_xy, 8, d_foff, d_wh, 2, (int64_t)nkp, (float*)c->tab_pts.p, st));
    GMS_TRY(filter_launch(c, st, (const float*)c->tab_pts.p, d_foff, 2, d_pair, 1, m, (const gms_dmatch*)(din + off_m),
                          with_rotation, with_scale, threshold_factor, d_out, d_res, nullptr));
    if (!zero_copy) GMS_HIP(hipMemcpyAsync(L.hout.p, L.dout.p, sizeof(gms_pair_result), hipMemcpyDeviceToHost, st));
    GMS_HIP(hipStreamSynchronize(st));
    const gms_pair_result r = *(const gms_pair_result*)L.hout.p;
    if (result) *result = r;
    if (r.status != GMS_OK) return r.status;
    if (r.n_inliers < 0 || r.n_inliers > m) return GMS_ERR_HIP;
    const size_t keep_bytes = (size_t)r.n_inliers * sizeof(gms_dmatch);
    if (!zero_copy && keep_bytes) {
        GMS_HIP(hipMemcpyAsync((char*)L.hout.p + sizeof(gms_pair_result), d_out, keep_bytes, hipMemcpyDeviceToHost, st));
        GMS_HIP(hipStreamSynchronize(st));
    }
    if (keep_bytes) std::memcpy(out, (const char*)L.hout.p + sizeof(gms_pair_result), keep_bytes);
    *n_out = r.n_inliers;
    return GMS_OK;
}

int gms_match(const gms_keypoint* kp1, int n1, int w1, int h1, const gms_keypoint* kp2, int n2, int w2, int h2,
              const gms_dmatch* matches, int m, int with_rotation, int with_scale, double threshold_factor,
              gms_dmatch* out, int* n_out)
{
    static std::mutex mu;
    static gms_ctx* def = nullptr;
    {
        std::lock_guard<std::mutex> lock(mu);
        if (!def) {
            int rc = gms_ctx_create(0, &def);
            if (rc != GMS_OK) {
                if (n_out) *n_out = 0;
                return rc;
            }
        }
    }
    return gms_match_ctx(def, kp1, n1, w1, h1, kp2, n2, w2, h2, matches, m, with_rotation, with_scale,
                         threshold_factor, out, n_out, nullptr);
}

int gms_filter_host_batch(gms_ctx* c, const gms_keypoint* kp, const int64_t* frame_off, const int32_t* wh, int n_frames,
                          const gms_pair* pairs, int n_pairs, const gms_dmatch* matches,
                          int with_rotation, int with_scale, double threshold_factor,
                          gms_dmatch* out, gms_pair_result* results)
{
    if (!c || n_frames < 0 || n_pairs < 0) return GMS_ERR_BAD_ARG;
    if (n_pairs == 0) return GMS_OK;
    if (!frame_off || !wh || !pairs || !results || n_frames == 0) return GMS_ERR_BAD_ARG;
    if (frame_off[0] != 0) return GMS_ERR_BAD_ARG;
    for (int f = 0; f < n_frames; ++f)
        if (frame_off[f + 1] < frame_off[f]) return GMS_ERR_BAD_ARG;
    const int64_t total_kp = frame_off[n_frames];
    if (total_kp < 0 || (total_kp > 0 && !kp)) return GMS_ERR_BAD_ARG;
    int max_m = 0;
    bool in_order = true;
    for (int i = 0; i < n_pairs; ++i) {
        if (pairs[i].m < 0 || pairs[i].match_off < 0) return GMS_ERR_BAD_ARG;
        if (pairs[i].m > gms_max_matches()) return GMS_ERR_CAPACITY;
        max_m = std::max(max_m, pairs[i].m);
        if (i + 1 < n_pairs && pairs[i].match_off + pairs[i].m > pairs[i + 1].match_off) in_order = false;
    }
    if (max_m > 0 && (!matches || !out)) return GMS_ERR_BAD_ARG;
    if (!in_order) {
        std::vector<std::pair<int64_t, int64_t>> r;
        r.reserve((size_t)n_pairs);
        for (int i = 0; i < n_pairs; ++i)
            if (pairs[i].m > 0) r.emplace_back(pairs[i].match_off, pairs[i].match_off + pairs[i].m);
        std::sort(r.begin(), r.end());
        for (size_t i = 1; i < r.size(); ++i)
            if (r[i - 1].second > r[i].first) return GMS_ERR_BAD_ARG;
    }

    std::lock_guard<std::mutex> lock(c->mu);
    GMS_HIP(hipSetDevice(c->device));
    c->lane[0].stream = c->own_stream;
    GMS_HIP(hipStreamSynchronize(c->stream));
    GMS_HIP(hipStreamSynchronize(c->lane[0].stream));
    GMS_HIP(hipStreamSynchronize(c->lane[1].stream));
    GMS_HIP(hipStreamSynchronize(c->lane[2].stream));

    const size_t kChunkMatches = (size_t)2 << 20;
    const int kChunkPairs = 8192;
    struct Chunk { int first, count; size_t matches; int max_m; };
    std::vector<Chunk> chunks;
    for (int i = 0; i < n_pairs;) {
        Chunk ch{i, 0, 0, 0};
        while (i < n_pairs && ch.count < kChunkPairs && (ch.count == 0 || ch.matches + (size_t)pairs[i].m <= kChunkMatches)) {
            ch.matches += (size_t)pairs[i].m;
            ch.max_m = std::max(ch.max_m, pairs[i].m);
            ++ch.count;
            ++i;
        }
        chunks.push_back(ch);
    }
    size_t cap_m = 0, cap_p = 0;
    for (const Chunk& ch : chunks) {
        cap_m = std::max(cap_m, ch.matches);
        cap_p = std::max(cap_p, (size_t)ch.count);
    }
    const size_t in_pairs_bytes = align16(cap_p * sizeof(gms_pair));
    const size_t in_bytes = std::max(in_pairs_bytes + cap_m * sizeof(gms_dmatch), (size_t)total_kp * 8);
    const size_t out_res_bytes = cap_p * sizeof(gms_pair_result) + 16;
    const size_t out_bytes = out_res_bytes + cap_m * sizeof(gms_dmatch);
    for (Lane& L : c->lane) {
        GMS_HIP(L.hin.reserve(&L == &c->lane[0] ? in_bytes : in_pairs_bytes + cap_m * sizeof(gms_dmatch)));
        GMS_HIP(L.hout.reserve(out_bytes));
        GMS_HIP(L.din.reserve(in_pairs_bytes + cap_m * sizeof(gms_dmatch)));
        GMS_HIP(L.dout.reserve(out_bytes));
    }
    {
        WsNeed w;
        GMS_TRY(plan_workspace(c, (int)cap_p, max_m, with_rotation != 0, with_scale != 0, true, true, &w));
        WsNeed w2;
        GMS_TRY(plan_workspace(c, (int)cap_p, max_m, with_rotation != 0, with_scale != 0, true, false, &w2));
        w.band = std::max(w.band, w2.band);
        GMS_TRY(grow_workspace(c, w, c->lane[0].stream));
    }
    if (!c->pool) c->pool = new (std::nothrow) CopyPool;
    if (!c->pool) return GMS_ERR_BAD_ARG;
    CopyPool& pool = *c->pool;
    std::vector<CopyJob> jobs;

    const size_t small_bytes = align16((size_t)(n_frames + 1) * 8) + (size_t)n_frames * 8;
    GMS_HIP(c->tab_kp.reserve((size_t)total_kp * 8));
    GMS_HIP(c->tab_pts.reserve((size_t)gms_frame_table_bytes(total_kp)));
    GMS_HIP(c->tab_small.reserve(small_bytes));
    {
        hipStream_t st = c->lane[0].stream;
        GMS_HIP(hipMemcpyAsync(c->tab_small.p, frame_off, (size_t)(n_frames + 1) * 8, hipMemcpyHostToDevice, st));
        GMS_HIP(hipMemcpyAsync((char*)c->tab_small.p + align16((size_t)(n_frames + 1) * 8), wh, (size_t)n_frames * 8,
                               hipMemcpyHostToDevice, st));
        if (total_kp) {
            jobs.push_back(CopyJob{c->lane[0].hin.p, kp, (size_t)total_kp * 8, 1});
            pool.run(jobs);
            jobs.clear();
            GMS_HIP(hipMemcpyAsync(c->tab_kp.p, c->lane[0].hin.p, (size_t)total_kp * 8, hipMemcpyHostToDevice, st));
            GMS_HIP(gms::launch_normalize(c->tab_kp.p, 8, (const int64_t*)c->tab_small.p,
                                          (const int32_t*)((char*)c->tab_small.p + align16((size_t)(n_frames + 1) * 8)),
                                          n_frames, total_kp, (float*)c->tab_pts.p, st));
        }
        GMS_HIP(hipStreamSynchronize(st));
    }
    const int64_t* d_foff = (const int64_t*)c->tab_small.p;

    auto in_matches = [&](Lane& L) { return (gms_dmatch*)((char*)L.din.p + in_pairs_bytes); };
    const size_t n_chunks = chunks.size();
    for (size_t k = 0; k < n_chunks + 2; ++k) {
        jobs.clear();
        if (k >= 2) {
            const Chunk& ch = chunks[k - 2];
            Lane& L = c->lane[(k - 2) % 3];
            GMS_HIP(hipEventSynchronize(L.ev_out));
            const gms_pair_result* res = (const gms_pair_result*)L.hout.p;
            const gms_dmatch* o = (const gms_dmatch*)((const char*)L.hout.p + out_res_bytes);
            std::memcpy(results + ch.first, res, (size_t)ch.count * sizeof(gms_pair_result));
            size_t at = 0;
            for (int i = 0; i < ch.count; ++i) {
                if (res[i].status != GMS_OK || res[i].n_inliers <= 0) continue;
                jobs.push_back(CopyJob{out + pairs[ch.first + i].match_off, o + at, (size_t)res[i].n_inliers * sizeof(gms_dmatch), 0});
                at += (size_t)res[i].n_inliers;
            }
        }
        if (k < n_chunks) {
            const Chunk& ch = chunks[k];
            Lane& L = c->lane[k % 3];
            gms_pair* hp = (gms_pair*)L.hin.p;
            gms_dmatch* hm = (gms_dmatch*)((char*)L.hin.p + in_pairs_bytes);
            size_t local = 0;
            for (int i = 0; i < ch.count; ++i) {
                const gms_pair& pr = pairs[ch.first + i];
                hp[i] = gms_pair{pr.frame_a, pr.frame_b, pr.m, 0, (int64_t)local};
                if (pr.m) jobs.push_back(CopyJob{hm + local, matches + pr.match_off, (size_t)pr.m * sizeof(gms_dmatch), 0});
                local += (size_t)pr.m;
            }
        }
        pool.run(jobs);
        if (k < n_chunks) {
            const Chunk& ch = chunks[k];
            Lane& L = c->lane[k % 3];
            gms_pair_result* d_res = (gms_pair_result*)L.dout.p;
            int64_t* d_total = (int64_t*)((char*)L.dout.p + out_res_bytes - 16);
            gms_dmatch* d_out = (gms_dmatch*)((char*)L.dout.p + out_res_bytes);
            GMS_HIP(hipMemcpyAsync(L.din.p, L.hin.p, in_pairs_bytes + ch.matches * sizeof(gms_dmatch), hipMemcpyHostToDevice, L.stream));
            GMS_TRY(filter_launch(c, L.stream, (const float*)c->tab_pts.p, d_foff, n_frames, (const gms_pair*)L.din.p, ch.count, ch.max_m,
                                  in_matches(L), with_rotation, with_scale, threshold_factor, d_out, d_res, nullptr,
                                  false ));
            GMS_HIP(gms::launch_compact_survivors((const gms_pair*)L.din.p, d_res, ch.count, d_out, in_matches(L), d_total, L.stream));
            GMS_HIP(hipMemcpyAsync(L.hout.p, L.dout.p, out_res_bytes, hipMemcpyDeviceToHost, L.stream));
            GMS_HIP(hipEventRecord(L.ev_res, L.stream));
        }
        if (k >= 1 && k - 1 < n_chunks) {
            const Chunk& ch = chunks[k - 1];
            Lane& L = c->lane[(k - 1) % 3];
            GMS_HIP(hipEventSynchronize(L.ev_res));
            const int64_t kept = *(const int64_t*)((const char*)L.hout.p + out_res_bytes - 16);
            if (kept < 0 || (size_t)kept > ch.matches) return GMS_ERR_HIP;
            if (kept)
                GMS_HIP(hipMemcpyAsync((char*)L.hout.p + out_res_bytes, in_matches(L), (size_t)kept * sizeof(gms_dmatch), hipMemcpyDeviceToHost, L.stream));
            GMS_HIP(hipEventRecord(L.ev_out, L.stream));
        }
    }
    return GMS_OK;
}

int64_t gms_bf_prepared_bytes(int desc_kind, int64_t total_desc, int n_frames)
{
    return (int64_t)gms::bf_prepared_bytes(desc_kind, total_desc, n_frames);
}

int gms_bf_prepare_device(gms_ctx* c, int desc_kind, const void* d_desc, const int64_t* d_frame_off, int n_frames,
                          int64_t total_desc, void* d_prepared)
{
    if (!c || n_frames < 0 || total_desc < 0) return GMS_ERR_BAD_ARG;
    if (!desc_kind_ok(desc_kind)) return GMS_ERR_BAD_ARG;
    if (total_desc == 0 || n_frames == 0) return GMS_OK;
    if (!d_desc || !d_frame_off || !d_prepared) return GMS_ERR_BAD_ARG;
    return on_ctx(c, [&] { return gms::launch_bf_prepare(desc_kind, d_desc, d_frame_off, n_frames, total_desc, d_prepared, c->stream); });
}

int gms_bfmatch_device(gms_ctx* c, int desc_kind, const void* d_desc, const void* d_prepared, int64_t total_desc,
                       const int64_t* d_frame_off, int n_frames, const gms_pair* d_pairs, int n_pairs, int max_query,
                       gms_dmatch* d_matches)
{
    if (!c || n_frames < 0 || n_pairs < 0 || max_query < 0 || total_desc < 0) return GMS_ERR_BAD_ARG;
    if (!desc_kind_ok(desc_kind)) return GMS_ERR_BAD_ARG;
    if (n_pairs == 0 || max_query == 0) return GMS_OK;
    if (!d_desc || !d_frame_off || !d_pairs || !d_matches) return GMS_ERR_BAD_ARG;
    if (desc_kind == GMS_DESC_L2_F32X128 && !d_prepared) return GMS_ERR_BAD_ARG;
    if (max_query > (1 << 22)) return GMS_ERR_CAPACITY;
    return on_ctx(c, [&] {
        return gms::launch_bf_match(desc_kind, d_desc, d_prepared, total_desc, d_frame_off, n_frames, d_pairs, n_pairs, max_query, d_matches,
                                    c->stream);
    });
}

size_t gms_bf_select_workspace_bytes(int n_pairs, int max_rows, int64_t total_backward_rows)
{
    if (n_pairs < 0 || max_rows < 0 || max_rows > (1 << 22) || total_backward_rows < 0) return 0;
    return gms::bf_select_ws_bytes(n_pairs, max_rows, total_backward_rows);
}

static bool bf_select_args_ok(int desc_kind, int cross_check, double coef, int max_size)
{
    return desc_kind_ok(desc_kind) && (cross_check == 0 || cross_check == 1) &&
           std::isfinite(coef) && coef >= 1.0 && max_size >= 0;
}

int gms_bf_select_device(gms_ctx* c, int desc_kind, const void* d_desc, const void* d_prepared, int64_t total_desc,
                         const int64_t* d_frame_off, int n_frames, const gms_pair* d_pairs, int n_pairs, int max_rows, int cross_check,
                         double distance_coef, int max_size, void* d_ws, size_t ws_bytes, gms_dmatch* d_out, gms_bf_result* d_bf_results,
                         gms_pair_result* d_pair_results)
{
    if (!c || n_frames < 0 || n_pairs < 0 || max_rows < 0 || max_rows > (1 << 22) || total_desc < 0) return GMS_ERR_BAD_ARG;
    if (!bf_select_args_ok(desc_kind, cross_check, distance_coef, max_size)) return GMS_ERR_BAD_ARG;
    if (n_pairs == 0) return GMS_OK;
    if (!d_frame_off || !d_pairs || !d_ws || !d_out || !d_bf_results || (total_desc > 0 && !d_desc)) return GMS_ERR_BAD_ARG;
    if (desc_kind == GMS_DESC_L2_F32X128 && total_desc > 0 && !d_prepared) return GMS_ERR_BAD_ARG;
    if (reinterpret_cast<uintptr_t>(d_ws) & 255u) return GMS_ERR_BAD_ARG;
    const size_t fixed = gms::bf_select_ws_bytes(n_pairs, max_rows, 0);
    if (ws_bytes < fixed) return GMS_ERR_BAD_ARG;
    const int64_t total_back = (int64_t)((ws_bytes - fixed) / 256) * 16;
    return on_ctx(c, [&] {
        return gms::launch_bf_select(desc_kind, d_desc, d_prepared, total_desc, d_frame_off, n_frames, d_pairs, n_pairs, max_rows, total_back,
                                     cross_check, distance_coef, max_size, d_ws, d_out, d_bf_results, d_pair_results, c->stream);
    });
}

int gms_bf_match_select(int desc_kind, const void* desc1, int n1, const void* desc2, int n2, int cross_check, double distance_coef,
                        int max_size, gms_dmatch* out, int64_t out_cap, int64_t* n_out, gms_bf_result* result)
{
    if (n_out) *n_out = 0;
    if (result) *result = gms_bf_result{0, 0, 0, 0.0f, GMS_OK};
    if (n1 < 0 || n2 < 0 || n1 > (1 << 22) || n2 > (1 << 22) || out_cap < 0 || out_cap > INT32_MAX || !n_out) return GMS_ERR_BAD_ARG;
    if (!bf_select_args_ok(desc_kind, cross_check, distance_coef, max_size)) return GMS_ERR_BAD_ARG;
    if ((n1 > 0 && !desc1) || (n2 > 0 && !desc2) || (out_cap > 0 && !out)) return GMS_ERR_BAD_ARG;
    const size_t row = desc_row_bytes(desc_kind);
    const int64_t total = (int64_t)n1 + n2;
    const int max_rows = std::max(n1, n2);
    const int64_t back_rows = cross_check ? n2 : n1;
    gms::BlockLayout lay;
    const size_t o_desc = lay.add(row * (size_t)total, 16), o_off = lay.add(3 * 8), o_pair = lay.add(sizeof(gms_pair));
    const size_t o_res = lay.add(sizeof(gms_bf_result)), o_prep = lay.add((size_t)gms::bf_prepared_bytes(desc_kind, total, 2), 16);
    const size_t o_ws = lay.add(gms::bf_select_ws_bytes(1, max_rows, back_rows)), o_out = lay.add(sizeof(gms_dmatch) * (size_t)out_cap, 16);
    DevBlock blk(lay, nullptr);
    const int64_t off[3] = {0, n1, total};
    const gms_pair pr{0, 1, (int32_t)out_cap, 0, 0};
    if (n1 > 0) blk.in(o_desc, desc1, row * (size_t)n1);
    if (n2 > 0) blk.in(o_desc + row * (size_t)n1, desc2, row * (size_t)n2);
    blk.in(o_off, off, sizeof(off));
    blk.in(o_pair, &pr, sizeof(pr));
    if (total > 0)
        blk.run([&](hipStream_t st) { return gms::launch_bf_prepare(desc_kind, blk.at(o_desc), blk.at<int64_t>(o_off), 2, total, blk.at(o_prep), st); });
// ... 1431 lines not shown
```

### sfm-gms_amd/csrc/gms_kernel_dense.hip

```cpp
#include <hip/hip_runtime.h>
#include <stdint.h>

#include <type_traits>

#include "gms_kernel_dense.h"
#include "gms_kernel_hash.h"

namespace gms {

template <int KPT, int NT, bool DEALT>
__device__ __forceinline__ bool dense_pair_rot(const FilterParams& p, uint32_t* smem, const int pair_idx, const int tid)
{
    constexpr int kMcap = KPT * NT;
    constexpr int kNRot = 8;
    constexpr int kChunk = (KPT % 5 == 0) ? 5 : 4;
    static_assert(KPT % kChunk == 0, "KPT must be a multiple of the chunk");
    const int lane = tid & 63;
    const int wave = tid >> 6;
    constexpr int kUnitsPerBlock = KPT * (NT / 64);
    constexpr bool dealt = DEALT;
    const int m_base = dealt ? ((((lane >> 3) * kUnitsPerBlock + wave) << 3) | (lane & 7)) : tid;
    const int m_stride = dealt ? (NT / 64) * 8 : NT;
    auto match_of = [&](int k) -> int { return m_base + k * m_stride; };

// ... 268 lines not shown
        {
            const uint4 z4 = make_uint4(0, 0, 0, 0);
            uint4* d4 = reinterpret_cast<uint4*>(smem);
            for (uint32_t i = tid; i < kDenseBytes / 16; i += NT) d4[i] = z4;
            if (tid < kLeftN) nl32[tid] = 0;
            if (tid == 0) misc[11] = 0;
        }
#pragma unroll
        for (int k = 0; k < KPT; ++k) code[k] &= ~(0xFFu << kDAccShift);
        __syncthreads();
        status = run_types(std::true_type{});
    }
    if (status != 0) {
        __syncthreads();
        return false;
    }


    int winner = -1;
    {
        uint32_t cnt[kNRot];
#pragma unroll
        for (int r = 0; r < kNRot; ++r) cnt[r] = 0;
#pragma unroll
        for (int k = 0; k < KPT; ++k)
#pragma unroll
            for (int r = 0; r < kNRot; ++r)
                cnt[r] += (uint32_t)__popcll(__ballot((code[k] >> (kDAccShift + r)) & 1u));
        if (lane == 0) {
#pragma unroll
            for (int r = 0; r < kNRot; ++r)
                if (cnt[r]) atomicAdd(&misc[r], cnt[r]);
        }
        __syncthreads();
        uint32_t best_count = 0;
#pragma unroll
        for (int r = 0; r < kNRot; ++r) {
            const uint32_t c = misc[r];
            if (c > best_count) {
                best_count = c;
                winner = r;
            }
        }
    }
    GMS_STAMP(7);

    constexpr int kWaves = NT / 64;
    uint32_t* cnt_tab = smem;
    unsigned long long keep[KPT];
#pragma unroll
    for (int k = 0; k < KPT; ++k) keep[k] = winner >= 0 ? __ballot((code[k] >> (kDAccShift + max(winner, 0))) & 1u) : 0ull;
    gms_dmatch* __restrict__ out = p.out + pr.match_off;
    uint8_t* mask_out = p.mask ? p.mask + pr.match_off : nullptr;
    uint32_t total = 0;
    if (!dealt) {
        constexpr int kScanRegs = (KPT * kWaves + 63) / 64;
#pragma unroll
        for (int k = 0; k < KPT; ++k)
            if (lane == 0) cnt_tab[k * kWaves + wave] = (uint32_t)__popcll(keep[k]);
        __syncthreads();
        uint32_t excl[kScanRegs];
#pragma unroll
        for (int v = 0; v < kScanRegs; ++v) {
            const int idx = v * 64 + lane;
            const uint32_t c = idx < KPT * kWaves ? cnt_tab[idx] : 0u;
            uint32_t incl = c;
#pragma unroll
            for (int d = 1; d < 64; d <<= 1) {
                const uint32_t t = __shfl_up(incl, d);
                if (lane >= d) incl += t;
            }
            excl[v] = total + incl - c;
            total += __shfl(incl, 63);
        }
        GMS_STAMP(8);
#pragma unroll
        for (int k = 0; k < KPT; ++k) {
            const int i = k * NT + tid;
            const int ch = k * kWaves + wave;
            static_assert(64 % kWaves == 0, "a wave's chunk never straddles two scan registers");
            const uint32_t base = __shfl(excl[(k * kWaves) >> 6], ch & 63);
            if (i < m) {
                const bool in = (keep[k] >> lane) & 1ull;
                if (mask_out) mask_out[i] = in ? 1 : 0;
                if (in) {
                    const uint32_t pos = base + (uint32_t)__popcll(keep[k] & ((1ull << lane) - 1ull));
                    *reinterpret_cast<uint4*>(&out[pos]) = kKeepRec ? rec[k] : *reinterpret_cast<const uint4*>(&matches[i]);
                }
            }
        }
    } else {
        constexpr int kUnits = KPT * NT / 8;
        static_assert(kUnits <= 2 * NT, "two scan entries per thread");
        uint32_t* wave_tot = misc + 16;
#pragma unroll
        for (int k = 0; k < KPT; ++k)
            if ((lane & 7) == 0) cnt_tab[match_of(k) >> 3] = (uint32_t)__popc((uint32_t)(keep[k] >> (lane & 56)) & 0xFFu);
        __syncthreads();
        {
            const uint32_t c0 = 2 * tid < kUnits ? cnt_tab[2 * tid] : 0u, c1 = 2 * tid + 1 < kUnits ? cnt_tab[2 * tid + 1] : 0u;
            uint32_t incl = c0 + c1;
#pragma unroll
            for (int d = 1; d < 64; d <<= 1) {
                const uint32_t t = __shfl_up(incl, d);
                if (lane >= d) incl += t;
            }
            if (lane == 63) wave_tot[wave] = incl;
            __syncthreads();
            uint32_t off = 0;
#pragma unroll
            for (int w = 0; w < kWaves; ++w) {
                const uint32_t tw = wave_tot[w];
                off += w < wave ? tw : 0u;
                total += tw;
            }
            if (2 * tid < kUnits) cnt_tab[2 * tid] = off + incl - c0 - c1;
            if (2 * tid + 1 < kUnits) cnt_tab[2 * tid + 1] = off + incl - c1;
        }
        __syncthreads();
        GMS_STAMP(8);
#pragma unroll
        for (int k = 0; k < KPT; ++k) {
            const int i = match_of(k);
            if (i < m) {
                const uint32_t byte = (uint32_t)(keep[k] >> (lane & 56)) & 0xFFu;
                const bool in = (byte >> (lane & 7)) & 1u;
                if (mask_out) mask_out[i] = in ? 1 : 0;
                if (in) {
                    const uint32_t pos = cnt_tab[i >> 3] + (uint32_t)__popc(byte & ((1u << (lane & 7)) - 1u));
                    *reinterpret_cast<uint4*>(&out[pos]) = kKeepRec ? rec[k] : *reinterpret_cast<const uint4*>(&matches[i]);
                }
            }
        }
    }
    GMS_STAMP(9);
    GMS_STAMP_FLUSH;
    if (tid == 0) {
        gms_pair_result r;
        r.n_inliers = (int)total;
        r.best_scale = total ? 0 : -1;
        r.best_rot = total ? winner + 1 : -1;
        r.status = GMS_OK;
        p.results[pair_idx] = r;
    }
    return true;
}

constexpr uint32_t kPEdgeX = 1u << 1, kPEdgeY = 1u << 3;
constexpr int kPEShift = 5;
constexpr int kPAtShift = 14;
static_assert(kDenseLdsBytes < (1u << 18), "an entry offset is 18 bits");
constexpr uint32_t kPZeroByte = 3u;

template <int KPT, int NT, bool DEALT>
__device__ __forceinline__ bool dense_pair_plain(const FilterParams& p, uint32_t* smem, const int pair_idx, const int tid)
{
    constexpr int kMcap = KPT * NT;
    constexpr int kChunk = (KPT % 5 == 0) ? 5 : 4;
    static_assert(KPT % kChunk == 0, "KPT must be a multiple of the chunk");
    static_assert(NT >= 2 * kLeftN, "verification: two lanes per left cell in one sweep");
    const int lane = tid & 63;
    const int wave = tid >> 6;
    constexpr int kUnitsPerBlock = KPT * (NT / 64);
    constexpr bool dealt = DEALT;
    const int m_base = dealt ? ((((lane >> 3) * kUnitsPerBlock + wave) << 3) | (lane & 7)) : tid;
    const int m_stride = dealt ? (NT / 64) * 8 : NT;
    auto match_of = [&](int k) -> int { return m_base + k * m_stride; };

    if ((uint32_t)(uintptr_t)((lds_u32_t*)smem) != 0u) return false;

    int64_t total_kp;
    const gms_pair pr = load_pair(p.pairs, pair_idx, p, total_kp);
    const int m = pr.m;
    if (p.with_scale || p.with_rotation || p.right_w[0] != kDenseRightW || p.right_h[0] != kDenseRightW || m <= 0 || m > kMcap ||
        pr.frame_a < 0 || pr.frame_a >= p.n_frames || pr.frame_b < 0 || pr.frame_b >= p.n_frames)
        return false;
    const FrameRangeWords fr_words = request_frame_ranges(p.frame_off, pr.frame_a, pr.frame_b);
    const gms_dmatch* __restrict__ matches = p.matches + pr.match_off;
    constexpr int kKeep = KPT <= 10 ? KPT : (DEALT ? 10 : 12);
    uint4 rec[kKeep];
    uint2 qt[KPT > kKeep ? KPT - kKeep : 1];
#pragma unroll
    for (int k = 0; k < KPT; ++k) {
        if (k < kKeep) { const u32x4_t rv = __builtin_nontemporal_load(reinterpret_cast<const u32x4_t*>(&matches[min(match_of(k), m - 1)])); rec[k] = make_uint4(rv.x, rv.y, rv.z, rv.w); }
        else qt[k - kKeep] = *reinterpret_cast<const uint2*>(&matches[min(match_of(k), m - 1)]);
    }
    int64_t offA, offB;
    int nA, nB;
    take_frame_ranges(fr_words, offA, nA, offB, nB);
    if (nA <= 0 || nB <= 0) return false;
    if (total_kp < 0 || offA + nA > total_kp || offB + nB > total_kp) return false;
    const uint16_t* __restrict__ lcodeA = reinterpret_cast<const uint16_t*>(p.pts + total_kp) + offA;
    const uint16_t* __restrict__ rcodeB = reinterpret_cast<const uint16_t*>(p.pts + total_kp) + total_kp + offB;

    uint32_t* nfine32 = smem + kDenseFineOff / 4;
    const uint8_t* nfine8 = reinterpret_cast<const uint8_t*>(nfine32);
    uint32_t* misc = smem + kDenseMiscOff / 4;
    uint32_t* trash = smem + kDenseTrashOff / 4;

    GMS_STAMP_DECL
#ifdef GMS_PHASE_TIMING
    ph_[14] = wall_clock64();
#endif
    if (tid < 32) misc[tid] = 0;
    if (tid < 16) trash[tid] = 0;
    if (tid < kFineN / 4) nfine32[tid] = 0;

    const uint32_t phA = (uint32_t)(reinterpret_cast<uintptr_t>(lcodeA) >> 1) & 7u, phB = (uint32_t)(reinterpret_cast<uintptr_t>(rcodeB) >> 1) & 7u;
    const uint32_t qA = (phA + (uint32_t)nA + 7u) >> 3, qB = (phB + (uint32_t)nB + 7u) >> 3;
    const bool staged = (qA + qB) * 16u <= kDenseBytes;
    const uint4* __restrict__ srcA = reinterpret_cast<const uint4*>(lcodeA - phA);
    const uint4* __restrict__ srcB = reinterpret_cast<const uint4*>(rcodeB - phB);
    constexpr int kStageRegs = 3;
    uint4 tb[kStageRegs];
#pragma unroll
    for (int i = 0; i < kStageRegs; ++i) {
        const uint32_t j = min((uint32_t)(i * NT + tid), qA + qB - 1u);
        const uint4* src = j < qA ? srcA + j : srcB + (j - qA);
        tb[i] = *src;
    }
    auto query_of = [&](int k) -> uint32_t { return k < kKeep ? rec[k < kKeep ? k : 0].x : qt[k < kKeep ? 0 : k - kKeep].x; };
    auto train_of = [&](int k) -> uint32_t { return k < kKeep ? rec[k < kKeep ? k : 0].y : qt[k < kKeep ? 0 : k - kKeep].y; };
    const uint32_t staged16 = staged ? qA + qB : 0u;
    {
        const uint4 z4 = make_uint4(0, 0, 0, 0);
        uint4* d4 = reinterpret_cast<uint4*>(smem);
        for (uint32_t i = (staged ? max(staged16, (uint32_t)(kStageRegs * NT)) : 0u) + tid; i < kDenseBytes / 16; i += NT) d4[i] = z4;
    }
    if (staged) {
        static_assert((size_t)kStageRegs * NT * 16 <= kDenseBytes, "the register-staged slots lie inside the matrix area");
        uint4* d4 = reinterpret_cast<uint4*>(smem);
#pragma unroll
        for (int i = 0; i < kStageRegs; ++i) {
            const bool in = (uint32_t)(i * NT + tid) < qA + qB;
            d4[i * NT + tid] = make_uint4(in ? tb[i].x : 0u, in ? tb[i].y : 0u, in ? tb[i].z : 0u, in ? tb[i].w : 0u);
        }
        for (uint32_t j = kStageRegs * NT + tid; j < qA + qB; j += NT) d4[j] = *(j < qA ? srcA + j : srcB + (j - qA));
    }
    const uint32_t ldsA = 2u * phA, ldsB = 16u * qA + 2u * phB;
    __syncthreads();
#ifdef GMS_PHASE_TIMING
    asm volatile("s_waitcnt vmcnt(0)" ::: "memory");
    GMS_STAMP(4);
    ph_[15] = wall_clock64();
#endif

    uint32_t code[KPT];
    const uint32_t cw_sink = (kDenseTrashOff + 4u * (uint32_t)(lane & 15)) << kPAtShift;
    {
        uint32_t ca[KPT], cb[KPT];
        if (staged) {
#pragma unroll
            for (int k = 0; k < KPT; ++k) ca[k] = ldsa_ld16(ldsA + 2u * min(query_of(k), (uint32_t)(nA - 1)));
#pragma unroll
            for (int k = 0; k < KPT; ++k) cb[k] = ldsa_ld16(ldsB + 2u * min(train_of(k), (uint32_t)(nB - 1)));
        } else {
#pragma unroll
            for (int k = 0; k < KPT; ++k) ca[k] = lcodeA[min(query_of(k), (uint32_t)(nA - 1))];
#pragma unroll
            for (int k = 0; k < KPT; ++k) cb[k] = rcodeB[min(train_of(k), (uint32_t)(nB - 1))];
        }
#ifdef GMS_PHASE_TIMING
        asm volatile("s_waitcnt vmcnt(0) lgkmcnt(0)" ::: "memory");
        GMS_STAMP(12);
#endif
        bool any_bad = false, spill = false;
#pragma unroll
        for (int k = 0; k < KPT; ++k) {
            const bool live = match_of(k) < m;
            const uint32_t e0 = cb[k] & kDEMask;
            const uint32_t cell = ca[k] >> kLCellShift;
            const bool ok = ((int)(query_of(k) < (uint32_t)nA) & (int)(train_of(k) < (uint32_t)nB) & (int)(cell != kLCellBad) & (int)((cb[k] & kRCodeBad) == 0u) & (int)(e0 != 0u)) != 0;
            const bool binned = live & ok & (cell < kLCellNever);
            const uint32_t sh = ((ca[k] & 1u) << 3) | ((ca[k] & 4u) << 2);
            const uint32_t old = ldsa_add_rtn(binned ? kDenseFineOff + 4u * cell : kDenseTrashOff + 4u * (uint32_t)(lane & 7), 1u << sh);
            spill |= binned & (((old >> sh) & 255u) == 255u);
            any_bad |= live & !ok;
            const uint32_t qe = (ca[k] & 21u) | ((ca[k] >> 4) & kPEdgeX) | ((ca[k] >> 3) & kPEdgeY);
            const uint32_t at1 = __umul24(cell, kDenseRow) + e0;
            code[k] = binned ? ((at1 << kPAtShift) | (e0 << kPEShift) | qe) : cw_sink;
        }
        if (any_bad) misc[8] = 1;
        if (spill) misc[13] = 1;
    }
    GMS_STAMP(13);
    __syncthreads();
    GMS_STAMP(0);

    {
        const uint4 z4 = make_uint4(0, 0, 0, 0);
        uint4* d4 = reinterpret_cast<uint4*>(smem);
        for (uint32_t i = tid; i < staged16; i += NT) d4[i] = z4;
        if (tid < 16) trash[tid] = 0x80000000u;
    }
    __syncthreads();
    GMS_STAMP(2);
    if (misc[8] != 0) {
        __syncthreads();
        return false;
    }
    const bool spilled = misc[13] != 0;

    const bool thr_fast = threshold_fast_ok(p.threshold_factor);
    const uint32_t f2i = dense_factor_sq(p.threshold_factor);
    uint32_t acc = 0;

    const uint32_t vi = (uint32_t)tid >> 1;
    const uint32_t viy = (vi * 3277u) >> 16, vix = vi - 20u * viy;
    const bool vodd = (tid & 1) != 0;

    const uint32_t* __restrict__ pf_base = nullptr;
    uint32_t pf_lines = 0, pf_sink = 0, pf_sink2 = 0;
    {
        const int nxt = pair_idx + p.prefetch_ahead;
        if (p.prefetch_ahead > 0 && nxt < p.n_pairs) {
            const gms_pair pn = load_pair(p.pairs, nxt);
            if (pn.m > 0 && pn.m <= kMcap && pn.match_off >= 0 && pn.frame_a >= 0 && pn.frame_a < p.n_frames && pn.frame_b >= 0 &&
                pn.frame_b < p.n_frames) {
                pf_base = reinterpret_cast<const uint32_t*>(p.matches + pn.match_off);
                pf_lines = min(((uint32_t)pn.m * 16u + 127u) >> 7, 2u * NT);
            }
        }
    }

    auto run_types = [&](auto crowded_c) -> int {
    constexpr bool CROWDED = decltype(crowded_c)::value;
    for (int g = 0; g < 4; ++g) {
        const int gx = g & 1, gy = g >> 1;
        const uint32_t q_mask = (uint32_t)(gx + 20 * gy);
        const uint32_t x_mask = (gx ? kPEdgeX : 0u) | (gy ? kPEdgeY : 0u);
        const uint32_t key_tag = (uint32_t)g << kDTagShift;
        const uint32_t nl_cur = kDenseFineOff + (uint32_t)(g & 1) * (kLeftN * 2u);
        if (!CROWDED && g == p.prefetch_type && pf_lines) {
            if ((uint32_t)tid < pf_lines) pf_sink = pf_base[32u * (uint32_t)tid];
            if ((uint32_t)tid + NT < pf_lines) pf_sink2 = pf_base[32u * ((uint32_t)tid + NT)];
        }
        if (!CROWDED && tid < kLeftN) {
            const uint32_t n = dense_nleft_cm(nfine8, tid % kLeftW, tid / kLeftW, gx, gy);
            if (n > 255u) misc[11] = 1;
            ldsa_st8(kDenseNleftOff + (uint32_t)tid, n);
        }

        uint32_t ae[KPT];
#pragma unroll
        for (int k0 = 0; k0 < KPT; k0 += kChunk) {
            uint32_t old[kChunk], at[kChunk], cg[kChunk], sh[kChunk];
#pragma unroll
            for (int c = 0; c < kChunk; ++c) {
                const uint32_t cw = code[k0 + c];
                cg[c] = (cw & x_mask) ? cw_sink : cw;
                at[c] = mad24_vsv(cg[c] & q_mask, kDenseRow, cg[c] >> kPAtShift);
                sh[c] = at[c] << 3;
                asm("" : "+v"(sh[c]));
                old[c] = ldsa_add_rtn(at[c] & ~3u, 1u << (sh[c] & 31u));
                if (CROWDED) {
                    const uint32_t l = (((at[c] - ((cg[c] >> kPEShift) & kDEMask)) >> 2) * 649u) >> 16;
                    ldsa_add(nl_cur + 4u * (l >> 1), 1u << ((l & 1u) << 4));
                }
            }
            __builtin_amdgcn_sched_barrier(0);
#pragma unroll
            for (int c = 0; c < kChunk; ++c) {
                const uint32_t e = (cg[c] >> kPEShift) & kDEMask;
                const uint32_t before = __builtin_amdgcn_ubfe(old[c], sh[c], 8);
                if (CROWDED && e != 0u && before == 255u) misc[12] = 1;
                ldsa_max(at[c] - e, key_tag | (before << 11) | e);
                asm("v_lshl_or_b32 %0, %1, 18, %2" : "=v"(ae[k0 + c]) : "v"(e), "v"(at[c]));
            }
        }
        GMS_STAMP(3);
        __syncthreads();
        GMS_STAMP(11);
        if (!CROWDED && misc[11] != 0) return 1;
        if (CROWDED && misc[12] != 0) return 2;

        if (tid < 2 * kLeftN) {
            const int s1 = vodd ? -1 : 1;
            const uint32_t nlb = (CROWDED ? nl_cur + 2u * vi : kDenseNleftOff + vi);
            const uint32_t hdr = vi * kDenseRow;
            const uint32_t ni = CROWDED ? ldsa_ld16(nlb) : ldsa_ld8(nlb);
            const uint32_t hdr_word = ldsa_ld32(hdr);
            uint32_t nl4[4];
            {
                constexpr int kD[4] = {-21, -20, -19, -1};
#pragma unroll
                for (int c = 0; c < 4; ++c) {
                    const uint32_t na = nlb + (uint32_t)((CROWDED ? 2 : 1) * s1 * kD[c]);
                    nl4[c] = CROWDED ? ldsa_ld16(na) : ldsa_ld8(na);
                }
            }
            if (__ballot(ni != 0) != 0ull) {
                const uint32_t best = hdr_word & ((1u << kDTagShift) - 1u);
                const uint32_t ej = ni ? (best & kDEMask) : (uint32_t)(kDenseRightN + 3);
                const uint32_t j = (uint32_t)(kDenseRightN + 3) - ej;
                const uint32_t jy = (j * 3277u) >> 16, jx = j - 20u * jy;
                const uint32_t lo = vodd ? 19u : 0u, hi = 19u - lo;
                const bool okA = (vix != lo) & (jx != lo);
                const bool okB = (vix != hi) & (jx != hi);
                const bool okC = (viy != lo) & (jy != lo);
                const int s403 = vodd ? -403 : 403;
                const uint32_t base = hdr + ej;
                uint32_t score = 0, tn = 0;
                auto side = [&](int c, int d, bool valid) {
                    const uint32_t a = valid ? base + (uint32_t)(s403 * d) : kPZeroByte;
                    score += ldsa_ld8(a);
                    tn += valid ? ((nl4[c] << 4) | 1u) : 0u;
                };
                side(0, -21, okA & okC);
                side(1, -20, okC);
                side(2, -19, okB & okC);
                side(3, -1, okA);
                score += dpp_xor1(score);
                tn += dpp_xor1(tn);
                score += (best >> 11) + 1u;
                tn += (ni << 4) | 1u;
                if (ni != 0 && !vodd) {
                    const bool rej = CROWDED ? threshold_rejects(tn >> 4, tn & 15u, score, p.threshold_factor, thr_fast)
                                             : dense_threshold_rejects(tn >> 4, tn & 15u, score, p.threshold_factor, thr_fast, f2i);
                    ldsa_st32(hdr, rej ? 0u : ej);
                }
            }
        }
        __syncthreads();
        GMS_STAMP(5);

        uint32_t cur = 0;
#pragma unroll
        for (int k = 0; k < KPT; ++k) {
            const uint32_t at = ae[k] & 0x3FFFFu, e = ae[k] >> 18;
            const uint32_t cr = ldsa_ld32(at - e);
            ldsa_st8(at, 0u);
            cur = shift_in_equal(cur, cr, e);
        }
        acc |= cur;
        if (CROWDED && tid < kLeftN / 2) ldsa_st32(kDenseFineOff + (uint32_t)((g + 1) & 1) * (kLeftN * 2u) + 4u * (uint32_t)tid, 0u);
        __syncthreads();
        GMS_STAMP(6);
    }
    return 0;
    };

    int status = 1;
    if (!spilled) status = run_types(std::false_type{});
    if (status == 1) {
        __syncthreads();
        {
            const uint4 z4 = make_uint4(0, 0, 0, 0);
            uint4* d4 = reinterpret_cast<uint4*>(smem);
            for (uint32_t i = tid; i < kDenseBytes / 16; i += NT) d4[i] = z4;
            if (tid < kLeftN) nfine32[tid] = 0;
            if (tid == 0) misc[11] = 0;
        }
        acc = 0;
        if (tid < 16) trash[tid] = 0x80000000u;
        __syncthreads();
        status = run_types(std::true_type{});
    }
    if (status != 0) {
        __syncthreads();
        return false;
    }
    GMS_STAMP(7);
    if (p.prefetch_type == 4 && pf_lines) {
        if ((uint32_t)tid < pf_lines) pf_sink = pf_base[32u * (uint32_t)tid];
        if ((uint32_t)tid + NT < pf_lines) pf_sink2 = pf_base[32u * ((uint32_t)tid + NT)];
    }
    if (p.prefetch_type != 4 && (pf_sink ^ pf_sink2) == 0x9E3779B9u && p.n_pairs < 0) trash[0] = pf_sink;

    constexpr int kWaves = NT / 64;
    uint32_t* cnt_tab = smem;
    unsigned long long keep[KPT];
#pragma unroll
    for (int k = 0; k < KPT; ++k) keep[k] = __ballot((acc >> (KPT - 1 - k)) & 1u);
    gms_dmatch* __restrict__ out = p.out + pr.match_off;
    uint8_t* mask_out = p.mask ? p.mask + pr.match_off : nullptr;
    uint32_t total = 0;
    if (!dealt) {
        uint32_t row_base[KPT];

        constexpr int kScanRegs = (KPT * kWaves + 63) / 64;
        static_assert(kWaves == 16, "one DPP row per k");
#pragma unroll
        for (int k = 0; k < KPT; ++k)
            if (lane == 0) cnt_tab[k * kWaves + wave] = (uint32_t)__popcll(keep[k]);
        __syncthreads();
        uint32_t excl[kScanRegs];
#pragma unroll
        for (int v = 0; v < kScanRegs; ++v) {
            const int idx = v * 64 + lane;
            const uint32_t c = idx < KPT * kWaves ? cnt_tab[idx] : 0u;
            uint32_t incl = c;
            incl += (uint32_t)__builtin_amdgcn_update_dpp(0, (int)incl, 0x111, 0xF, 0xF, true);
            incl += (uint32_t)__builtin_amdgcn_update_dpp(0, (int)incl, 0x112, 0xF, 0xF, true);
            incl += (uint32_t)__builtin_amdgcn_update_dpp(0, (int)incl, 0x114, 0xF, 0xF, true);
            incl += (uint32_t)__builtin_amdgcn_update_dpp(0, (int)incl, 0x118, 0xF, 0xF, true);
            excl[v] = incl - c;
            (void)idx;
#pragma unroll
            for (int r = 0; r < 4; ++r) {
                const int k = v * 4 + r;
                if (k < KPT) {
                    row_base[k] = total;
                    total += (uint32_t)__builtin_amdgcn_readlane((int)incl, r * 16 + 15);
                }
            }
        }
        GMS_STAMP(8);
        const int wave_s = __builtin_amdgcn_readfirstlane(wave);
        auto put = [&](int k, const uint4& rv) {
            const int i = k * NT + tid;
            const uint32_t base = row_base[k] + (uint32_t)__builtin_amdgcn_readlane((int)excl[k >> 2], (k & 3) * 16 + wave_s);
            if (i < m) {
                const bool in = (keep[k] >> lane) & 1ull;
                if (mask_out) mask_out[i] = in ? 1 : 0;
                if (in) {
                    const uint32_t pos = base + (uint32_t)__popcll(keep[k] & ((1ull << lane) - 1ull));
                    __builtin_nontemporal_store(u32x4_t{rv.x, rv.y, rv.z, rv.w}, reinterpret_cast<u32x4_t*>(&out[pos]));
                }
            }
        };
#pragma unroll
        for (int k = 0; k < kKeep; ++k) put(k, rec[k]);
        constexpr int kBatch = 2;
#pragma unroll
        for (int k0 = kKeep; k0 < KPT; k0 += kBatch) {
            uint4 again[kBatch];
#pragma unroll
            for (int j = 0; j < kBatch; ++j) {
                const int k = k0 + j < KPT ? k0 + j : KPT - 1, i = k * NT + tid;
                again[j] = *reinterpret_cast<const uint4*>(&matches[(i < m && ((keep[k] >> lane) & 1ull)) ? i : 0]);
            }
#pragma unroll
            for (int j = 0; j < kBatch; ++j) asm volatile("" : "+v"(again[j].x), "+v"(again[j].y), "+v"(again[j].z), "+v"(again[j].w));
#pragma unroll
            for (int j = 0; j < kBatch; ++j)
                if (k0 + j < KPT) put(k0 + j, again[j]);
        }
    } else {
        constexpr int kUnits = KPT * NT / 8;
        static_assert(kUnits <= 2 * NT, "two scan entries per thread");
        uint32_t* wave_tot = misc + 16;
#pragma unroll
        for (int k = 0; k < KPT; ++k)
            if ((lane & 7) == 0) cnt_tab[match_of(k) >> 3] = (uint32_t)__popc((uint32_t)(keep[k] >> (lane & 56)) & 0xFFu);
        __syncthreads();
        {
            const uint32_t c0 = 2 * tid < kUnits ? cnt_tab[2 * tid] : 0u, c1 = 2 * tid + 1 < kUnits ? cnt_tab[2 * tid + 1] : 0u;
            uint32_t incl = c0 + c1;
#pragma unroll
            for (int d = 1; d < 64; d <<= 1) {
                const uint32_t t = __shfl_up(incl, d);
                if (lane >= d) incl += t;
            }
            if (lane == 63) wave_tot[wave] = incl;
            __syncthreads();
            uint32_t off = 0;
#pragma unroll
            for (int w = 0; w < kWaves; ++w) {
                const uint32_t tw = wave_tot[w];
                off += w < wave ? tw : 0u;
                total += tw;
            }
            if (2 * tid < kUnits) cnt_tab[2 * tid] = off + incl - c0 - c1;
            if (2 * tid + 1 < kUnits) cnt_tab[2 * tid + 1] = off + incl - c1;
        }
        __syncthreads();
        GMS_STAMP(8);
        auto put = [&](int k, const uint4& rv) {
            const int i = match_of(k);
            if (i < m) {
                const uint32_t byte = (uint32_t)(keep[k] >> (lane & 56)) & 0xFFu;
                const bool in = (byte >> (lane & 7)) & 1u;
                if (mask_out) mask_out[i] = in ? 1 : 0;
                if (in) {
                    const uint32_t pos = cnt_tab[i >> 3] + (uint32_t)__popc(byte & ((1u << (lane & 7)) - 1u));
                    __builtin_nontemporal_store(u32x4_t{rv.x, rv.y, rv.z, rv.w}, reinterpret_cast<u32x4_t*>(&out[pos]));
                }
            }
        };
#pragma unroll
        for (int k = 0; k < kKeep; ++k) put(k, rec[k]);
        constexpr int kBatch = 2;
#pragma unroll
        for (int k0 = kKeep; k0 < KPT; k0 += kBatch) {
            uint4 again[kBatch];
#pragma unroll
            for (int j = 0; j < kBatch; ++j) {
                const int k = k0 + j < KPT ? k0 + j : KPT - 1, i = match_of(k);
                const bool in = i < m && (((uint32_t)(keep[k] >> (lane & 56)) >> (lane & 7)) & 1u) != 0u;
                again[j] = *reinterpret_cast<const uint4*>(&matches[in ? i : 0]);
            }
#pragma unroll
            for (int j = 0; j < kBatch; ++j) asm volatile("" : "+v"(again[j].x), "+v"(again[j].y), "+v"(again[j].z), "+v"(again[j].w));
#pragma unroll
            for (int j = 0; j < kBatch; ++j)
                if (k0 + j < KPT) put(k0 + j, again[j]);
        }
    }
    GMS_STAMP(9);
    GMS_STAMP_FLUSH;
    if (p.prefetch_type == 4 && (pf_sink ^ pf_sink2) == 0x9E3779B9u && p.n_pairs < 0) trash[0] = pf_sink;
    if (tid == 0) {
        gms_pair_result r;
        r.n_inliers = (int)total;
        r.best_scale = total ? 0 : -1;
        r.best_rot = total ? 1 : -1;
        r.status = GMS_OK;
        p.results[pair_idx] = r;
    }
    return true;
}

template <int KPT, bool ROT, int NT, bool DEALT>
__global__ void __launch_bounds__(NT)
filter_kernel_dense(FilterParams p)
{
    extern __shared__ __attribute__((aligned(16))) uint32_t smem[];
    first_round_stagger(p);
    bool done;
    if constexpr (ROT) done = dense_pair_rot<KPT, NT, DEALT>(p, smem, (int)blockIdx.x, (int)threadIdx.x);
    else done = dense_pair_plain<KPT, NT, DEALT>(p, smem, (int)blockIdx.x, (int)threadIdx.x);
    if (!done) hash_pair<KPT, ROT, NT>(p, smem, (int)blockIdx.x, (int)threadIdx.x);
}

__global__ void threshold_kernel(const int32_t* T, const int32_t* n, const int32_t* score, double factor,
                                 int count, uint8_t* out)
{
    int i = blockIdx.x * blockDim.x + threadIdx.x;
    if (i < count) {
        const uint32_t t = (uint32_t)T[i], nn = (uint32_t)n[i], sc = (uint32_t)score[i];
        const bool general = threshold_rejects(t, nn, sc, factor, threshold_fast_ok(factor));
        uint8_t r = general ? 1 : 0;
        if (t <= 9u * 255u && sc <= 9u * 255u && nn >= 1u && nn <= 9u &&
            dense_threshold_rejects(t, nn, sc, factor, threshold_fast_ok(factor), dense_factor_sq(factor)) != general)
            r = 2;
        out[i] = r;
    }
}

hipError_t launch_threshold(const int32_t* d_T, const int32_t* d_n, const int32_t* d_score, double factor,
                            int count, uint8_t* d_out, hipStream_t stream)
{
    if (count <= 0) return hipSuccess;
    hipLaunchKernelGGL(threshold_kernel, dim3((count + 255) / 256), dim3(256), 0, stream, d_T, d_n, d_score,
                       factor, count, d_out);
    return hipGetLastError();
}

hipError_t launch_filter_dense(const FilterParams& p, int kpt, int n_pairs, size_t lds_bytes, hipStream_t stream)
{
    const size_t lds = lds_bytes > kDenseLdsBytes ? lds_bytes : (size_t)kDenseLdsBytes;
    return dispatch_kpt_rot(kpt, p.with_rotation != 0, [&](auto k, auto rot) {
        constexpr int KPT = decltype(k)::value;
        constexpr bool ROT = decltype(rot)::value;
        if (p.dealt) hipLaunchKernelGGL((filter_kernel_dense<KPT, ROT, kThreads, true>), dim3((unsigned)n_pairs), dim3(kThreads), lds, stream, p);
        else hipLaunchKernelGGL((filter_kernel_dense<KPT, ROT, kThreads, false>), dim3((unsigned)n_pairs), dim3(kThreads), lds, stream, p);
        return hipGetLastError();
    });
}

hipError_t init_dense_kernels()
{
    return for_each_kpt_rot([](auto k, auto rot) {
        constexpr int KPT = decltype(k)::value;
        constexpr bool ROT = decltype(rot)::value;
        const hipError_t e = allow_full_lds(filter_kernel_dense<KPT, ROT, kThreads, false>);
        return e != hipSuccess ? e : allow_full_lds(filter_kernel_dense<KPT, ROT, kThreads, true>);
    });
}

}
```

### sfm-gms_amd/csrc/gms_kernels.h

```cpp
#pragma once
#include <hip/hip_runtime.h>
#include <stddef.h>
#include <stdint.h>

#include "gms.h"
#include "logos_dict_core.h"
#include "ws_layout.h"

namespace gms {

constexpr int kThreads = 1024;
constexpr size_t kLdsBytes = 160 * 1024;
constexpr uint32_t kPartialHeaderDw = 4;
constexpr uint32_t kPartialStrideDw = kPartialHeaderDw + 16 * 1024 / 32;

constexpr uint32_t kTableMagic0 = 0x46534D47u, kTableMagic1 = 0x31424154u;
constexpr int kTableHeaderBytes = 16;

struct FilterParams {
    const float2* pts;
    const int64_t* frame_off;
    int n_frames;
    const gms_pair* pairs;
    int n_pairs;
    int stagger_ticks;
    int stagger_blocks;
    const gms_dmatch* matches;
    gms_dmatch* out;
    gms_pair_result* results;
    uint8_t* mask;
    uint32_t table_slots;
    int region_shift;
    int with_rotation, with_scale;
    uint32_t* partial;
    const uint32_t* pair_flags;
    int dealt;
    int probe_scales;
    int probe_nibble;
    uint32_t* probe_stats;
    uint32_t* overflow_events;
    int prefetch_type, prefetch_ahead;
    int dense;
    double threshold_factor;
    int right_w[5], right_h[5];
#ifdef GMS_PHASE_TIMING
    unsigned long long* diag;
#endif
};

hipError_t init_filter_kernels();
hipError_t init_band_kernels();
hipError_t init_big_kernels();
int        filter_pick_kpt(int max_m);
uint32_t   filter_table_slots(int kpt);
int        filter_region_shift(int kpt);
size_t     filter_lds_bytes(int kpt, uint32_t table_slots);
hipError_t launch_normalize(const void* d_kp, int kp_stride_bytes, const int64_t* d_frame_off, const int32_t* d_wh,
                            int n_frames, int64_t total_kp, float* d_pts, hipStream_t stream);
hipError_t launch_filter(const FilterParams& p, int kpt, int n_pairs, hipStream_t stream);
hipError_t launch_filter_hash(const FilterParams& p, int kpt, int n_pairs, size_t lds_bytes, hipStream_t stream);
hipError_t launch_filter_dense(const FilterParams& p, int kpt, int n_pairs, size_t lds_bytes, hipStream_t stream);
hipError_t init_hash_kernels();
hipError_t init_dense_kernels();
hipError_t init_scales_kernels();
hipError_t launch_order_probe(const FilterParams& p, uint32_t* flag, hipStream_t stream);
hipError_t launch_probe_verdict(uint32_t* stats, uint32_t* flag, hipStream_t stream);
hipError_t launch_check_pairs(const gms_pair* d_pairs, int n_pairs, gms_pair_result* d_results, uint32_t* d_flag, hipStream_t stream);
hipError_t launch_filter_scales(const FilterParams& p, int kpt, int n_pairs, hipStream_t stream);
hipError_t launch_compact_survivors(const gms_pair* d_pairs, const gms_pair_result* d_results, int n_pairs, const gms_dmatch* d_out,
                                    gms_dmatch* d_packed, int64_t* d_total, hipStream_t stream);
constexpr int kBigMaxMatches = 1 << 22;
constexpr int kBigLdsMaskMatches = 262144;
int        big_mcap(int max_m);
size_t     big_ws_stride_dwords(int mcap);
hipError_t launch_filter_big(const FilterParams& p, int mcap, int n_workgroups, uint32_t* ws, hipStream_t stream);
size_t     band_ws_bytes_per_pair(int mcap, bool need_mask);
hipError_t launch_filter_band(const FilterParams& p, int mcap, void* ws, const uint32_t** flags_out, hipStream_t stream);
size_t     tile_ws_bytes_per_pair(const FilterParams& p, int mcap, bool need_mask);
hipError_t launch_filter_tiles(const FilterParams& p, int mcap, void* ws, const uint32_t** flags_out, hipStream_t stream);
hipError_t init_stream_kernels();
int        stream_max_matches();
size_t     stream_ws_bytes_per_pair(const FilterParams& p, int mcap, bool need_mask);
hipError_t launch_filter_stream(const FilterParams& p, int mcap, void* ws, const uint32_t** flags_out, hipStream_t stream);
size_t     stream_dense_ws_bytes_per_pair(int mcap);
hipError_t launch_filter_stream_dense(const FilterParams& p, int mcap, void* ws, const uint32_t** flags_out, hipStream_t stream);
size_t     bf_prepared_bytes(int kind, int64_t total, int n_frames);
hipError_t launch_bf_prepare(int kind, const void* d_desc, const int64_t* d_frame_off, int n_frames, int64_t total, void* d_prep,
                             hipStream_t stream);
hipError_t launch_bf_match(int kind, const void* d_desc, const void* d_prep, int64_t total, const int64_t* d_frame_off, int n_frames,
                           const gms_pair* d_pairs, int n_pairs, int max_query, gms_dmatch* d_matches, hipStream_t stream);
size_t     bf_select_ws_bytes(int n_pairs, int64_t max_rows, int64_t total_back);
hipError_t launch_bf_select(int kind, const void* d_desc, const void* d_prep, int64_t total, const int64_t* d_frame_off, int n_frames,
                            const gms_pair* d_pairs, int n_pairs, int max_rows, int64_t total_back, int cross, double coef, int max_size,
                            void* d_ws, gms_dmatch* d_out, gms_bf_result* d_res, gms_pair_result* d_pres, hipStream_t stream);
hipError_t launch_disparity(const gms_keypoint* d_kp1, int n1, const gms_keypoint* d_kp2, int n2, const gms_dmatch* d_matches,
                            const int32_t* d_n_matches, int max_matches, int w, int h, const uint8_t* d_gt, int disp_ratio,
                            uint8_t* d_disparity, uint32_t* d_work, gms_disparity_stats* d_stats, hipStream_t stream);
hipError_t launch_gather_points(const gms_keypoint* d_kp1, int n1, const gms_keypoint* d_kp2, int n2, const gms_dmatch* d_matches,
                                const int32_t* d_n_matches, int max_matches, float* d_coords1, float* d_coords2, int32_t* d_status,
                                hipStream_t stream);
hipError_t launch_triangulate(const double* camera, const double* dist, const double* P1, const double* P2, const float* d_coords1,
                              const float* d_coords2, const int32_t* d_n_matches, int max_matches, double* d_points3d,
                              gms_triangulation_stats* d_stats, hipStream_t stream);
hipError_t launch_recover_pose(const double* camera, const double P[4][12], double dist_thresh, const float* d_coords1, const float* d_coords2,
                               const int32_t* d_n_matches, int max_matches, const uint8_t* d_in_mask, gms_pose* d_pose, uint8_t* d_out_mask,
                               void* d_work, hipStream_t stream);
hipError_t launch_gather_batch(const gms_keypoint* d_kp, const int64_t* d_frame_off, int n_frames, const gms_pair* d_pairs, int n_pairs, int max_m,
                               const gms_dmatch* d_filtered, const gms_pair_result* d_results, float* d_coords1, float* d_coords2,
                               gms_two_view* d_tv, hipStream_t stream);
hipError_t launch_find_essential_batch(const gms_camera& cam, double prob, double threshold, int max_iters, const gms_pair* d_pairs, int n_pairs,
                                       const float* d_coords1, const float* d_coords2, uint8_t* d_mask, gms_two_view* d_tv, hipStream_t stream);
hipError_t launch_five_point_selftest(const double* d_pts, int n_samples, double* d_models, int* d_counts, hipStream_t stream);
hipError_t launch_recover_pose_batch(const gms_camera& cam, double dist_thresh, int use_in_mask, const gms_pair* d_pairs, int n_pairs,
                                     const float* d_coords1, const float* d_coords2, uint8_t* d_mask, gms_two_view* d_tv, hipStream_t stream);
hipError_t launch_triangulate_batch(const gms_camera& cam, const gms_pair* d_pairs, int n_pairs, const float* d_coords1, const float* d_coords2,
                                    const uint8_t* d_mask, double* d_points3d, gms_two_view* d_tv, hipStream_t stream);
hipError_t launch_disparity_batch(const gms_keypoint* d_kp, const int64_t* d_frame_off, const int32_t* d_wh, int n_frames, const gms_pair* d_pairs,
                                  int n_pairs, int max_m, const gms_dmatch* d_filtered, const gms_pair_result* d_results, const uint8_t* d_gt,
                                  int64_t gt_stride, int disp_ratio, uint8_t* d_disparity, int64_t map_stride, uint32_t* d_work,
                                  gms_disparity_stats* d_stats, hipStream_t stream);
size_t     detect_workspace_bytes(int w, int h, int n_images, int max_keypoints);
hipError_t launch_detect(const uint8_t* d_images, int n_images, int w, int h, int threshold, int max_keypoints, void* d_ws,
                         gms_keypoint* d_kp, uint8_t* d_desc, int32_t* d_counts, hipStream_t stream);
hipError_t launch_describe(const uint8_t* d_image, int w, int h, gms_keypoint* d_kp, int n, void* d_ws, uint8_t* d_desc, int32_t* d_status,
                           hipStream_t stream);
void       pyramid_quotas(const int* widths, const int* heights, int n, int max_keypoints, int* quotas);
struct PyramidRun {
    enum Detector { kFast, kDog } detector;
    int strength;
    bool refined;
};
size_t     detect_pyramid_workspace_bytes(int w, int h, int n_images, int max_keypoints, int n_levels, bool refined);
hipError_t launch_pyramid_build(const uint8_t* d_images, int n_images, int w, int h, int n_levels, uint8_t* d_levels, hipStream_t stream);
hipError_t launch_detect_pyramid(const PyramidRun& run, const uint8_t* d_images, int n_images, int w, int h, int max_keypoints, int n_levels, void* d_ws,
                                 gms_keypoint* d_kp, uint8_t* d_desc, float* d_rows128, int32_t* d_counts, int32_t* d_level_counts, hipStream_t stream);
hipError_t launch_detect_maps(const uint8_t* d_images, int n_images, int w, int h, void* d_ws, hipStream_t stream);
hipError_t launch_grad_level(int n_images, int w, int h, int quota, void* d_det_ws, const int32_t* d_level_counts, int level, int out_stride,
                             gms_keypoint* d_kp, float* d_rows128, hipStream_t stream);
hipError_t launch_describe_grad(const uint8_t* d_image, int w, int h, gms_keypoint* d_kp, int n, void* d_ws, float* d_rows128, int32_t* d_status,
                                hipStream_t stream);
hipError_t launch_dog_maps(const uint8_t* d_images, int n_images, int w, int h, int contrast, uint8_t* d_cand, uint16_t* d_box, uint32_t* d_hist,
                           uint16_t* d_codes, hipStream_t stream);
hipError_t launch_bgr_to_gray(const uint8_t* d_bgr, int n, int w, int h, uint8_t* d_gray, hipStream_t stream);
hipError_t launch_detect_pack(const gms_keypoint* d_kp_blocks, const uint8_t* d_rows32_blocks, const float* d_rows128_blocks, const int32_t* d_counts,
                              int n, int max_keypoints, gms_keypoint* d_kp, uint8_t* d_rows32, float* d_rows128, int64_t* d_frame_off,
                              hipStream_t stream);
hipError_t launch_logos_prepare(const gms_keypoint* d_kp, const int64_t* d_frame_off, int n_frames, int64_t total_kp, const int32_t* d_words,
                                int n_words, void* d_ws, size_t ws_bytes, void* d_table, int n_cus, hipStream_t stream);
hipError_t launch_logos_filter(const void* d_table, const gms_pair* d_pairs, int n_pairs, void* d_ws, size_t ws_bytes, gms_dmatch* d_out,
                               gms_logos_result* d_lres, gms_pair_result* d_pres, int n_cus, hipStream_t stream);
hipError_t launch_logos_words(int kind, const void* d_desc, int64_t total, const void* d_dict, int n_words, int32_t* d_words, int n_cus,
                              hipStream_t stream);
size_t     logos_dict_ws_bytes(const logos_dict::Params& p);
hipError_t launch_logos_dict_train(const logos_dict::Params& p, const void* d_desc, const int64_t* d_set_off, void* d_ws, void* d_dict,
                                   gms_logos_dict_result* d_results, int32_t* d_labels, hipStream_t stream);
size_t     stereo_bm_ws_bytes(int n, int W, int H);
hipError_t launch_stereo_bm(const gms_stereo_bm_params& p, const uint8_t* d_left, const uint8_t* d_right, int n, int W, int H, int pitch,
                            void* d_ws, int16_t* d_disp, int32_t* d_cost, hipStream_t stream);
hipError_t launch_stereo_bm_normalize(const int16_t* d_disp, int n, int W, int H, uint8_t* d_out, hipStream_t stream);
hipError_t launch_stereo_bm_prefilter(const gms_stereo_bm_params& p, const uint8_t* d_left, const uint8_t* d_right, int n, int W, int H,
                                      int pitch, uint8_t* pre, hipStream_t stream);
hipError_t launch_stereo_bm_validate(const gms_stereo_bm_params& p, int n, int W, int H, int16_t* d_disp, const int32_t* wcost,
                                     int32_t* d_cost, hipStream_t stream);
size_t     sfm_register_ws_bytes(int n_pairs, int64_t total_kp, int64_t total_m);
hipError_t launch_sfm_register(const int64_t* d_frame_off, int n_frames, int64_t total_kp, const gms_pair* d_pairs,
                               const gms_sfm_plan_entry* d_plan, int n_pairs, int max_m, int64_t total_m, const gms_dmatch* d_filtered,
                               const uint8_t* d_mask, const double* d_points3d, const gms_two_view* d_tv, int root, int min_links,
                               void* d_ws, gms_sfm_view* d_views, gms_sfm_pair_reg* d_reg, double* d_world, int32_t* d_track,
                               int64_t cloud_cap, double* d_cloud, int32_t* d_cloud_id, int32_t* d_cloud_obs, int32_t* d_cloud_est,
                               double* d_cloud_spread, gms_sfm_summary* d_summary, hipStream_t stream);
size_t     sfm_ba_ws_bytes(int n_frames, int64_t total_kp, int64_t cloud_cap);
hipError_t launch_sfm_ba(const gms_camera& camera, const gms_sfm_ba_params& prm, const gms_keypoint* d_kp, const int64_t* d_frame_off,
                         int n_frames, int64_t total_kp, const gms_pair* d_pairs, int n_pairs, int64_t total_m, const gms_dmatch* d_filtered,
                         const uint8_t* d_mask, const gms_sfm_view* d_views, const gms_sfm_pair_reg* d_reg, const int32_t* d_track,
                         int64_t cloud_cap, const double* d_cloud, const int32_t* d_cloud_id, const gms_sfm_summary* d_reg_summary, void* d_ws,
                         gms_sfm_view* d_views_out, double* d_cloud_out, int32_t* d_track_status, gms_sfm_ba_summary* d_summary,
                         hipStream_t stream);
size_t     stereo_sgm_ws_bytes(const gms_stereo_sgm_params& p, int n, int W, int H);
hipError_t launch_stereo_sgm(const gms_stereo_sgm_params& p, const uint8_t* d_left, const uint8_t* d_right, int n, int W, int H, int pitch,
                             void* d_ws, int16_t* d_disp, int32_t* d_cost, hipStream_t stream);
size_t     portrait_ws_bytes(int n, int W, int H);
hipError_t launch_portrait(const gms_portrait_params& p, const uint8_t* d_bgr, const uint8_t* d_disp, int n, int W, int H, int pitch_bgr,
                           int pitch_disp, void* d_ws, uint8_t* d_out, uint8_t* d_mask, uint8_t* d_selected, uint8_t* d_blurred,
                           hipStream_t stream, hipEvent_t* stage_events = nullptr);
hipError_t launch_median_blur(const uint8_t* d_src, int n, int W, int H, int channels, int pitch, int ksize, uint8_t* d_dst,
                              hipStream_t stream);
hipError_t launch_resize(const uint8_t* d_src, int n, int sw, int sh, int channels, int src_pitch, uint8_t* d_dst, int dw, int dh,
                         int dst_pitch, hipStream_t stream);
hipError_t launch_warp_affine(const uint8_t* d_src, int n, int sw, int sh, int channels, int src_pitch, const double* d_M, int n_matrices,
                              uint8_t* d_dst, int dw, int dh, int dst_pitch, hipStream_t stream);
hipError_t launch_rectify_plan(const gms_camera& camera, const gms_two_view* d_tv, int n_pairs, int W, int H, int out_w, int out_h,
                               gms_rectify_plan* d_plans, hipStream_t stream);
hipError_t launch_rectify(const gms_camera& camera, const uint8_t* d_src, int n, int sw, int sh, int channels, int src_pitch,
                          const gms_rectify_plan* d_plans, int n_plans, int which, uint8_t* d_dst, int dw, int dh, int dst_pitch,
                          uint8_t* d_valid, hipStream_t stream);
size_t     dense_cloud_ws_bytes(int n_pairs, int W, int H);
hipError_t launch_dense_cloud(const int16_t* d_disp16, const uint8_t* d_valid, const uint8_t* d_image, int channels, int image_pitch,
                              int n_pairs, int W, int H, const gms_rectify_plan* d_plans, int filtered16, int min_disp16,
                              const gms_pair* d_pairs, const gms_sfm_pair_reg* d_reg, const gms_sfm_view* d_views, int n_frames, void* d_ws,
                              int cap, float* d_xyz, uint8_t* d_color, int32_t* d_pixel, int32_t* d_count, hipStream_t stream);
size_t     chess_candidates_ws_bytes(int n, int w, int h);
hipError_t launch_chess_candidates(const uint8_t* d_images, int n, int w, int h, int max_candidates, void* d_ws,
                                   gms_chess_candidate* d_out, int32_t* d_counts, hipStream_t stream);
hipError_t launch_corner_subpix(const uint8_t* d_images, int n_images, int w, int h, const int32_t* d_image_of, double* d_corners,
                                int n_corners, int max_iter, double eps, int32_t* d_status, hipStream_t stream);
hipError_t launch_threshold(const int32_t* d_T, const int32_t* d_n, const int32_t* d_score, double factor,
                            int count, uint8_t* d_out, hipStream_t stream);

}
```

### sfm-gms_amd/csrc/gms_kernels.hip

```cpp
#include <hip/hip_runtime.h>
#include <stdint.h>

#include "gms_kernel_dense.h"

namespace gms {

__device__ __forceinline__ void keypoint_codes(float2 n, uint16_t& lcode, uint16_t& rcode, uint32_t& scode)
{
    const bool bad = max(__float_as_uint(n.x), __float_as_uint(n.y)) >= 0x49800000u;
    const float x = bad ? 0.0f : n.x, y = bad ? 0.0f : n.y;
    const float fx = 20.0f * x, fy = 20.0f * y;
    const uint32_t hx = (uint32_t)(int)(fx + fx), hy = (uint32_t)(int)(fy + fy);
    const uint32_t q = (hx & 1u) + 20u * (hy & 1u);
    const uint32_t edge = (hx == 39u ? 1u << 5 : 0u) | (hy == 39u ? 1u << 6 : 0u);
    const uint32_t l1 = (hy >> 1) * (uint32_t)kLeftW + (hx >> 1);
    const bool never = max(hx, hy) >= 40u;
    lcode = (uint16_t)(bad ? kLCellBad << kLCellShift : (never ? kLCellNever << kLCellShift : (q | edge | (l1 << kLCellShift))));
    const uint32_t r0x = (uint32_t)(int)fx, r0y = (uint32_t)(int)fy;
    const uint32_t e0 = (r0x < 20u && r0y < 20u) ? 403u - (r0y * 20u + r0x) : 0u;
    rcode = (uint16_t)(e0 | (bad ? kRCodeBad : 0u));
    const uint32_t r3x = (uint32_t)(int)(28.0f * x), r3y = (uint32_t)(int)(28.0f * y);
    const uint32_t odd40 = ((uint32_t)(int)(40.0f * x) & 1u) | (((uint32_t)(int)(40.0f * y) & 1u) << 1);
    const bool in_grids = r0x < 20u && r0y < 20u && r3x < 28u && r3y < 28u;
    scode = (bad || !in_grids) ? kSCodeBad : ((r0y * 20u + r0x) | ((r3y * 28u + r3x) << 9) | (odd40 << 19));
}

__global__ void __launch_bounds__(256)
normalize_kernel(const char* __restrict__ kp, int kp_stride, const int64_t* __restrict__ frame_off,
                 const int32_t* __restrict__ wh, int n_frames, int64_t total, float2* __restrict__ pts)
{
    if (blockIdx.x == 0 && threadIdx.x == 0) {
        uint32_t* h = reinterpret_cast<uint32_t*>(pts) - kTableHeaderBytes / 4;
        h[0] = kTableMagic0;
        h[1] = kTableMagic1;
        *reinterpret_cast<int64_t*>(h + 2) = total;
    }
    uint16_t* __restrict__ lcode = reinterpret_cast<uint16_t*>(pts + total);
    uint16_t* __restrict__ rcode = lcode + total;
    uint32_t* __restrict__ scode = reinterpret_cast<uint32_t*>(rcode + total);
    int64_t i = (int64_t)blockIdx.x * blockDim.x + threadIdx.x;
    int64_t stride = (int64_t)gridDim.x * blockDim.x;
    for (; i < total; i += stride) {
        int lo = 0, hi = n_frames - 1;
        while (lo < hi) {
            int mid = (lo + hi + 1) >> 1;
            if (frame_off[mid] <= i) lo = mid; else hi = mid - 1;
        }
        float w = (float)wh[2 * lo], h = (float)wh[2 * lo + 1];
        const float* p = reinterpret_cast<const float*>(kp + i * kp_stride);
        float2 o;
        o.x = p[0] / w + 0.0f;
        o.y = p[1] / h + 0.0f;
        pts[i] = o;
        uint16_t lc, rc;
        uint32_t sc;
        keypoint_codes(o, lc, rc, sc);
        lcode[i] = lc;
        rcode[i] = rc;
        scode[i] = sc;
    }
}

__global__ void __launch_bounds__(1024)
order_probe_kernel(FilterParams p, uint32_t* __restrict__ flag)
{
    __shared__ uint32_t s_same, s_seen;
    const int tid = (int)threadIdx.x, lane = tid & 63, wave = tid >> 6;
    if (tid == 0) s_same = s_seen = 0;
    __syncthreads();
    const int pi = (int)(((long long)wave * p.n_pairs) >> 4);
    const gms_pair pr = p.pairs[pi];
    if (pr.m >= 128 && pr.frame_a >= 0 && pr.frame_a < p.n_frames) {
        const int64_t offA = p.frame_off[pr.frame_a];
        const int nA = (int)(p.frame_off[pr.frame_a + 1] - offA);
        const int64_t total_kp = table_total_kp(p);
        const bool table_ok = total_kp >= 0 && nA > 0 && offA + nA <= total_kp;
        const uint16_t* __restrict__ lcode = reinterpret_cast<const uint16_t*>(p.pts + (table_ok ? total_kp : 0)) + offA;
        const int start = (pr.m >> 1) & ~63;
        const uint32_t q = (uint32_t)p.matches[pr.match_off + start + lane].queryIdx;
        const uint32_t lc = table_ok ? (uint32_t)lcode[min(q, (uint32_t)(nA - 1))] >> kLCellShift : kLCellNever;
        const uint32_t cell = lc >= kLCellNever ? 0x10000u + (uint32_t)lane : lc;
        const uint32_t next = (uint32_t)__shfl_down((int)cell, 1);
        const unsigned long long same = __ballot(lane < 63 && cell == next);
        if (lane == 0) {
            atomicAdd(&s_same, (uint32_t)__popcll(same));
            atomicAdd(&s_seen, 63u);
        }
    }
    __syncthreads();
    if (tid == 0 && s_seen != 0) *flag = 4u * s_same > s_seen ? 1u : 0u;
}

size_t filter_lds_bytes(int kpt, uint32_t table_slots)
{
    const size_t mcap = (size_t)kpt * kThreads;
    size_t dwords = table_slots + 5 * 1664 + 8 * kLeftN + (mcap >> 5) + (mcap >> 6) + 1 + 48 + 4 + 132 + 12;
    return dwords * 4;
}

int filter_region_shift(int kpt) { return kpt <= 10 ? 0 : 2; }

uint32_t filter_table_slots(int kpt)
{
    const uint32_t mcap = (uint32_t)kpt * kThreads;
    return (mcap + (mcap >> filter_region_shift(kpt)) + 7 * kLeftN + 3u) & ~3u;
}

int filter_pick_kpt(int max_m)
{
    static const int kKpt[] = {4, 10, 16};
    for (int k : kKpt)
        if (max_m <= k * kThreads && filter_lds_bytes(k, filter_table_slots(k)) <= kLdsBytes) return k;
    return 0;
}

__global__ void __launch_bounds__(256)
pairs_in_order_kernel(const gms_pair* __restrict__ pairs, int n_pairs, uint32_t* __restrict__ flag)
{
    const int i = (int)(blockIdx.x * 256u + threadIdx.x);
    bool bad = false;
    if (i + 1 < n_pairs) {
        const gms_pair a = pairs[i], b = pairs[i + 1];
        bad = a.match_off + (int64_t)max(a.m, 0) > b.match_off;
    }
    if (__ballot(bad) != 0ull && (threadIdx.x & 63) == 0) atomicOr(flag, 1u);
}

__global__ void __launch_bounds__(256)
pairs_overlap_kernel(const gms_pair* __restrict__ pairs, int n_pairs, const uint32_t* __restrict__ flag,
                     gms_pair_result* __restrict__ results)
{
    if (*flag == 0u) return;
    __shared__ int64_t s_lo[256], s_hi[256];
    const int i = (int)(blockIdx.x * 256u + threadIdx.x);
    int64_t lo = 0, hi = 0;
    if (i < n_pairs) {
        const gms_pair a = pairs[i];
        lo = a.match_off;
        hi = a.match_off + (int64_t)max(a.m, 0);
    }
    bool clash = false;
    for (int base = 0; base < n_pairs; base += 256) {
        const int j = base + (int)threadIdx.x;
        int64_t l = 0, h = 0;
        if (j < n_pairs) {
            const gms_pair b = pairs[j];
            l = b.match_off;
            h = b.match_off + (int64_t)max(b.m, 0);
        }
        __syncthreads();
        s_lo[threadIdx.x] = l;
        s_hi[threadIdx.x] = h;
        __syncthreads();
        const int n_tile = min(256, n_pairs - base);
        for (int t = 0; t < n_tile; ++t) {
            const int64_t tl = s_lo[t], th = s_hi[t];
            clash |= (base + t != i) & (tl < hi) & (lo < th) & (tl < th) & (lo < hi);
        }
    }
    if (i < n_pairs && clash) results[i].status = GMS_ERR_BAD_ARG;
}

hipError_t launch_check_pairs(const gms_pair* d_pairs, int n_pairs, gms_pair_result* d_results, uint32_t* d_flag, hipStream_t stream)
{
    if (n_pairs < 2) return hipSuccess;
    hipError_t e = hipMemsetAsync(d_flag, 0, 4, stream);
    if (e != hipSuccess) return e;
    const unsigned blocks = (unsigned)((n_pairs + 255) / 256);
    hipLaunchKernelGGL(pairs_in_order_kernel, dim3(blocks), dim3(256), 0, stream, d_pairs, n_pairs, d_flag);
    hipLaunchKernelGGL(pairs_overlap_kernel, dim3(blocks), dim3(256), 0, stream, d_pairs, n_pairs, d_flag, d_results);
    return hipGetLastError();
}

__global__ void __launch_bounds__(256)
compact_survivors_kernel(const gms_pair* __restrict__ pairs, const gms_pair_result* __restrict__ results, int n_pairs,
                         const gms_dmatch* __restrict__ out, gms_dmatch* __restrict__ packed, int64_t* __restrict__ total)
{
    __shared__ unsigned long long s_part[4];
    const int i = (int)blockIdx.x, tid = (int)threadIdx.x;
    unsigned long long sum = 0;
    for (int j = tid; j < i; j += 256) {
        const gms_pair_result r = results[j];
        sum += (r.status == GMS_OK && r.n_inliers > 0) ? (unsigned long long)r.n_inliers : 0ull;
    }
    for (int d = 32; d > 0; d >>= 1) sum += __shfl_down(sum, d);
    if ((tid & 63) == 0) s_part[tid >> 6] = sum;
    __syncthreads();
    const unsigned long long off = s_part[0] + s_part[1] + s_part[2] + s_part[3];
    const gms_pair_result r = results[i];
    const int k = (r.status == GMS_OK && r.n_inliers > 0) ? r.n_inliers : 0;
    const uint4* __restrict__ src = reinterpret_cast<const uint4*>(out + pairs[i].match_off);
    uint4* __restrict__ dst = reinterpret_cast<uint4*>(packed + off);
    for (int j = tid; j < k; j += 256) dst[j] = src[j];
    if (i == n_pairs - 1 && tid == 0) *total = (int64_t)(off + (unsigned long long)k);
}

hipError_t launch_compact_survivors(const gms_pair* d_pairs, const gms_pair_result* d_results, int n_pairs, const gms_dmatch* d_out,
                                    gms_dmatch* d_packed, int64_t* d_total, hipStream_t stream)
{
    if (n_pairs <= 0) return hipSuccess;
    hipLaunchKernelGGL(compact_survivors_kernel, dim3((unsigned)n_pairs), dim3(256), 0, stream, d_pairs, d_results, n_pairs, d_out, d_packed, d_total);
    return hipGetLastError();
}

__global__ void probe_verdict_kernel(uint32_t* stats, uint32_t* flag)
{
    uint32_t mask = *flag;
    for (int s = 0; s < 5; ++s) {
        const uint32_t kept = stats[2 * s], skipped = stats[2 * s + 1];
        if (kept + skipped >= 8u) mask = (mask & ~(1u << s)) | (skipped >= kept ? 1u << s : 0u);
        stats[2 * s] = stats[2 * s + 1] = 0u;
    }
    for (int s = 3; s < 5; ++s) {
        const uint32_t kept = stats[4 + 2 * s], skipped = stats[5 + 2 * s];
        if (kept + skipped >= 8u) mask = (mask & ~(1u << (8 + s))) | (skipped >= kept ? 1u << (8 + s) : 0u);
        stats[4 + 2 * s] = stats[5 + 2 * s] = 0u;
    }
    *flag = mask;
}

hipError_t launch_probe_verdict(uint32_t* stats, uint32_t* flag, hipStream_t stream)
{
    hipLaunchKernelGGL(probe_verdict_kernel, dim3(1), dim3(1), 0, stream, stats, flag);
    return hipGetLastError();
}

hipError_t launch_order_probe(const FilterParams& p, uint32_t* flag, hipStream_t stream)
{
    if (p.n_pairs <= 0) return hipSuccess;
    hipLaunchKernelGGL(order_probe_kernel, dim3(1), dim3(1024), 0, stream, p, flag);
    return hipGetLastError();
}

hipError_t launch_normalize(const void* d_kp, int kp_stride_bytes, const int64_t* d_frame_off, const int32_t* d_wh,
                            int n_frames, int64_t total_kp, float* d_pts, hipStream_t stream)
{
    if (total_kp <= 0) return hipSuccess;
    int64_t blocks = (total_kp + 255) / 256;
    if (blocks > 8192) blocks = 8192;
    hipLaunchKernelGGL(normalize_kernel, dim3((unsigned)blocks), dim3(256), 0, stream, reinterpret_cast<const char*>(d_kp),
                       kp_stride_bytes, d_frame_off, d_wh, n_frames, total_kp,
                       reinterpret_cast<float2*>(reinterpret_cast<char*>(d_pts) + kTableHeaderBytes));
    return hipGetLastError();
}

hipError_t init_filter_kernels()
{
    hipError_t e = init_hash_kernels();
    if (e == hipSuccess) e = init_dense_kernels();
    if (e == hipSuccess) e = init_scales_kernels();
    return e;
}

hipError_t launch_filter(const FilterParams& p, int kpt, int n_pairs, hipStream_t stream)
{
    if (n_pairs <= 0) return hipSuccess;
    const size_t lds = filter_lds_bytes(kpt, p.table_slots);
    return p.dense ? launch_filter_dense(p, kpt, n_pairs, lds, stream) : launch_filter_hash(p, kpt, n_pairs, lds, stream);
}

}
```

Measured before the change: 11.49 million.

## Precompute per-frame left-cell histograms and reuse them for identity-ordered match sets

When the frame table is built, two extra kernels now compute per-frame side records: a histogram of left-grid cells, flags, and a stamp that ties the records to the table contents. The dense filter gains an IDENT path that loads the precomputed histogram instead of rebuilding it when a pair's matches are identity-ordered (queryIdx equals index and the match count equals the frame's keypoint count). The order probe sets a verdict for this identity case, and a device-side miss counter turns the path off when the assumption fails. The trade-off is extra work at normalize time, a larger frame table tail and more host bookkeeping, plus reliance on stamp validation to stay correct.

```diff
diff --git a/include/gms.h b/include/gms.h
--- a/include/gms.h
+++ b/include/gms.h
@@ -78,15 +78,20 @@
 #define GMS_QUERY_PREFETCH_TYPE     6
 #define GMS_QUERY_PREFETCH_AHEAD    7
 #define GMS_QUERY_STAGGER_TICKS     8
+#define GMS_QUERY_LAST_IDENT        9
+#define GMS_QUERY_IDENT_MISSES     10
 int  gms_ctx_query(gms_ctx* ctx, int what, int64_t* value);
 #define GMS_OPTION_DEAL         1
 #define GMS_OPTION_SCALE_PROBE  2
+#define GMS_OPTION_IDENT        3
 int  gms_ctx_set_option(gms_ctx* ctx, int option, int value);
 
 #define GMS_FRAME_TABLE_HEADER_BYTES 16
 int64_t gms_frame_table_bytes(int64_t total_kp);
 int gms_normalize_device(gms_ctx* ctx, const gms_keypoint* d_kp, const int64_t* d_frame_off,
                          const int32_t* d_wh, int n_frames, int64_t total_kp, float* d_pts);
+#define GMS_SIDE_RECORD_BYTES 1632
+int gms_ctx_read_side_records(gms_ctx* ctx, void* dst, size_t dst_bytes, int* n_frames);
 
 int gms_filter_device(gms_ctx* ctx, const float* d_pts, const int64_t* d_frame_off, int n_frames,
                       const gms_pair* d_pairs, int n_pairs, int max_m,
diff --git a/sfm-gms_amd/api.py b/sfm-gms_amd/api.py
--- a/sfm-gms_amd/api.py
+++ b/sfm-gms_amd/api.py
@@ -24,7 +24,14 @@
         raise GmsError(rc, f"{what}: {msg}")
 
 
+SIDE_RECORD_DTYPE = np.dtype([("off", "<i8"), ("n", "<i4"), ("flags", "<u4"), ("stamp", "<u8"), ("pad", "<u4", (2,)), ("hist", "<u4", (400,))])
+assert SIDE_RECORD_DTYPE.itemsize == 1632
+
+
 class GmsContext:
+
+    OPTION_DEAL, OPTION_SCALE_PROBE, OPTION_IDENT = 1, 2, 3
+    QUERY_LAST_IDENT, QUERY_IDENT_MISSES = 9, 10
 
     def __init__(self, device=0):
         self._lib = load_library()
@@ -128,6 +135,13 @@
         _check(self._lib.gms_normalize_device(self._h, d_kp, d_frame_off, d_wh, int(n_frames), int(total_kp), d_pts),
                self._lib, "gms_normalize_device")
 
+    def read_side_records(self, max_frames):
+        buf = np.zeros(max(int(max_frames), 1), dtype=SIDE_RECORD_DTYPE)
+        n = C.c_int(0)
+        _check(self._lib.gms_ctx_read_side_records(self._h, buf.ctypes.data, int(max_frames) * SIDE_RECORD_DTYPE.itemsize, C.byref(n)),
+               self._lib, "gms_ctx_read_side_records")
+        return buf[: min(int(n.value), int(max_frames))]
+
     def filter_device(self, d_pts, d_frame_off, n_frames, d_pairs, n_pairs, max_m, d_matches, d_out, d_results,
                       d_mask=None, withRotation=False, withScale=False, thresholdFactor=6.0):
         _check(self._lib.gms_filter_device(self._h, d_pts, d_frame_off, int(n_frames), d_pairs, int(n_pairs),
diff --git a/sfm-gms_amd/capi.py b/sfm-gms_amd/capi.py
--- a/sfm-gms_amd/capi.py
+++ b/sfm-gms_amd/capi.py
@@ -17,6 +17,7 @@
     "gms_ctx_set_option": (i32, [vp, i32, i32]),
     "gms_frame_table_bytes": (i64, [i64]),
     "gms_normalize_device": (i32, [vp, vp, vp, vp, i32, i64, vp]),
+    "gms_ctx_read_side_records": (i32, [vp, vp, sz, P(i32)]),
     "gms_filter_device": (i32, [vp, vp, vp, i32, vp, i32, i32, vp, i32, i32, dbl, vp, vp, vp]),
     "gms_filter_host_batch": (i32, [vp, vp, vp, vp, i32, vp, i32, vp, i32, i32, dbl, vp, vp]),
     "gms_bf_prepared_bytes": (i64, [i32, i64, i32]),
diff --git a/sfm-gms_amd/csrc/gms_capi.cpp b/sfm-gms_amd/csrc/gms_capi.cpp
--- a/sfm-gms_amd/csrc/gms_capi.cpp
+++ b/sfm-gms_amd/csrc/gms_capi.cpp
@@ -64,7 +64,7 @@
     bool dense_on = true, band_on = true, stream_on = true;
     int probe_nibble = 16;
     bool probe_nibble_set = false;
-    int stagger_us = -1, deal = -1, scale_probe = -1, check_pairs = -1;
+    int stagger_us = -1, deal = -1, scale_probe = -1, check_pairs = -1, ident = -1;
     int prefetch_type = 3, prefetch_ahead = 0;
     size_t band_ws_budget = (size_t)4 << 30;
 };
@@ -78,6 +78,7 @@
         if (const char* e = std::getenv("GMS_PROBE_NIBBLE")) { v.probe_nibble = (int)std::strtol(e, nullptr, 0) & 24; v.probe_nibble_set = true; }
         if (const char* e = std::getenv("GMS_STAGGER_US")) v.stagger_us = std::atoi(e);
         if (const char* e = std::getenv("GMS_DEAL")) v.deal = std::atoi(e) != 0 ? 1 : 0;
+        if (const char* e = std::getenv("GMS_IDENT")) v.ident = std::atoi(e) != 0 ? 1 : 0;
         if (const char* e = std::getenv("GMS_SCALE_PROBE")) v.scale_probe = std::atoi(e) != 0 ? 1 : 0;
         if (const char* e = std::getenv("GMS_CHECK_PAIRS")) v.check_pairs = std::atoi(e) != 0 ? 1 : 0;
         if (const char* e = std::getenv("GMS_PREFETCH")) {
@@ -158,7 +159,12 @@
     unsigned filter_launches = 0;
     uint32_t overflow_seen = 0;
     int stream_penalty = 0;
-    int opt_deal = -1, opt_probe = -1;
+    int opt_deal = -1, opt_probe = -1, opt_ident = -1;
+    DevBuf side;
+    int side_frames = 0;
+    uint64_t side_stamp = 0;
+    int use_ident = 0, last_ident = 0;
+    uint32_t ident_misses_seen = 0;
     DevBuf probe_stats;
     unsigned scale_launches = 0;
     hipEvent_t ws_event = nullptr;
@@ -226,6 +232,31 @@
     GMS_HIP(hipStreamSynchronize(st));
     GMS_HIP(hipDeviceSynchronize());
     GMS_HIP(c->pose_ws.reserve(bytes));
+    return GMS_OK;
+}
+
+int build_frame_table(gms_ctx* c, hipStream_t st, const void* d_kp, int kp_stride_bytes, const int64_t* d_frame_off, const int32_t* d_wh,
+                      int n_frames, int64_t total_kp, float* d_pts)
+{
+    if (total_kp <= 0) return GMS_OK;
+    const size_t need = (size_t)(n_frames > 0 ? n_frames : 0) * sizeof(gms::SideRecord);
+    bool with_side = n_frames > 0 && need <= gms::kSideMaxBytes;
+    if (with_side && need > c->side.cap) {
+        hipStreamCaptureStatus cs = hipStreamCaptureStatusNone;
+        if (hipStreamIsCapturing(st, &cs) == hipSuccess && cs != hipStreamCaptureStatusNone) {
+            with_side = false;
+        } else {
+            GMS_HIP(hipDeviceSynchronize());
+            GMS_HIP(c->side.reserve(need));
+        }
+    }
+    const uint64_t stamp = with_side ? 1 : 0;
+    c->side_stamp = 0;
+    c->side_frames = 0;
+    GMS_HIP(gms::launch_normalize(d_kp, kp_stride_bytes, d_frame_off, d_wh, n_frames, total_kp, d_pts,
+                                  with_side ? (gms::SideRecord*)c->side.p : nullptr, stamp, st));
+    c->side_stamp = stamp;
+    c->side_frames = with_side ? n_frames : 0;
     return GMS_OK;
 }
 
@@ -282,8 +313,22 @@
     if (c->verdict_pending && !capturing && hipEventQuery(c->verdict_event) == hipSuccess) {
         c->use_dealt = c->verdict[0] != 0u ? 1 : 0;
         c->use_probe = (int)c->verdict[1];
+        c->use_ident = c->verdict[3] != 0u ? 1 : 0;
         c->verdict_pending = false;
     }
+    if (!capturing) {
+        const uint32_t now = ((volatile uint32_t*)c->verdict)[4];
+        if (now != c->ident_misses_seen) {
+            c->ident_misses_seen = now;
+            c->use_ident = 0;
+        }
+    }
+    const int force_ident = c->opt_ident >= 0 ? c->opt_ident : knobs().ident;
+    p.side = (const gms::SideRecord*)c->side.p;
+    p.side_frames = c->side_frames;
+    p.side_stamp = c->side_stamp;
+    p.ident = (p.dense && kpt && !with_rotation && c->side.p != nullptr && c->side_frames >= 1 && c->side_stamp != 0 &&
+               (force_ident >= 0 ? force_ident != 0 : c->use_ident != 0)) ? 1 : 0;
     const int force_deal = c->opt_deal >= 0 ? c->opt_deal : knobs().deal, force_probe = c->opt_probe >= 0 ? c->opt_probe : knobs().scale_probe;
     const bool scales_matrix = kpt && with_scale && knobs().dense_on;
     p.dealt = ((p.dense || scales_matrix) && kpt && (force_deal >= 0 ? force_deal != 0 : c->use_dealt != 0)) ? 1 : 0;
@@ -301,6 +346,7 @@
     {
         void* dflag = nullptr;
         p.overflow_events = hipHostGetDevicePointer(&dflag, c->verdict, 0) == hipSuccess ? (uint32_t*)dflag + 2 : nullptr;
+        p.ident_misses = p.overflow_events ? p.overflow_events + 2 : nullptr;
     }
     if (kpt && with_scale) {
         const bool measuring = force_probe < 0 && !capturing && (c->scale_launches++ & 15u) == 0u;
@@ -316,7 +362,7 @@
         if (!capturing && p.probe_stats == nullptr && (c->dense_launches++ & 15u) == 0u) {
             void* dflag = nullptr;
             GMS_HIP(hipHostGetDevicePointer(&dflag, c->verdict, 0));
-            GMS_HIP(gms::launch_order_probe(p, (uint32_t*)dflag, st));
+            GMS_HIP(gms::launch_order_probe(p, (uint32_t*)dflag, (uint32_t*)dflag + 3, st));
             GMS_HIP(hipEventRecord(c->verdict_event, st));
             c->verdict_pending = true;
         }
@@ -332,7 +378,7 @@
         if (p.dense && !capturing && (c->dense_launches++ & 15u) == 0u) {
             void* dflag = nullptr;
             GMS_HIP(hipHostGetDevicePointer(&dflag, c->verdict, 0));
-            GMS_HIP(gms::launch_order_probe(p, (uint32_t*)dflag, st));
+            GMS_HIP(gms::launch_order_probe(p, (uint32_t*)dflag, (uint32_t*)dflag + 3, st));
             GMS_HIP(hipEventRecord(c->verdict_event, st));
             c->verdict_pending = true;
         }
@@ -357,6 +403,7 @@
         GMS_HIP(gms::launch_filter_big(p, w.mcap, n_wg, (uint32_t*)c->big_ws.p, st));
     }
     c->last_dealt = p.dealt;
+    c->last_ident = p.ident;
     c->last_probe = p.probe_scales | (p.probe_scales ? p.probe_nibble << 8 : 0);
     c->last_kpt = kpt;
     c->last_stagger_ticks = p.stagger_ticks;
@@ -495,8 +542,11 @@
         c->verdict[0] = 0;
         c->verdict[1] = 0x1D | (16 << 8);
         c->verdict[2] = 0;
+        c->verdict[3] = 0;
+        c->verdict[4] = 0;
         GMS_HIP(c->probe_stats.reserve(128));
         GMS_HIP(hipMemset(c->probe_stats.p, 0, 128));
+        GMS_HIP(c->side.reserve(2048 * sizeof(gms::SideRecord)));
         GMS_HIP(gms::init_filter_kernels());
         GMS_HIP(gms::init_band_kernels());
         GMS_HIP(gms::init_stream_kernels());
@@ -515,6 +565,7 @@
         if (c->verdict_event) (void)hipEventDestroy(c->verdict_event);
         if (c->verdict) (void)hipHostFree(c->verdict);
         c->probe_stats.release();
+        c->side.release();
         delete c;
         return rc;
     }
@@ -536,7 +587,7 @@
         (void)hipStreamSynchronize(c->lane[1].stream);
         (void)hipStreamSynchronize(c->lane[2].stream);
         if (c->ws_pending) (void)hipEventSynchronize(c->ws_event);
-        DevBuf* bufs[] = {&c->aux, &c->big_ws, &c->band_ws, &c->partial_ws, &c->pose_ws, &c->probe_stats, &c->tab_kp, &c->tab_pts, &c->tab_small};
+        DevBuf* bufs[] = {&c->aux, &c->big_ws, &c->band_ws, &c->partial_ws, &c->pose_ws, &c->probe_stats, &c->tab_kp, &c->tab_pts, &c->tab_small, &c->side};
         if (c->verdict) (void)hipHostFree(c->verdict);
         for (DevBuf* b : bufs) b->release();
         for (Lane& l : c->lane) {
@@ -576,6 +627,7 @@
     if (c->verdict_pending && hipEventQuery(c->verdict_event) == hipSuccess) {
         c->use_dealt = c->verdict[0] != 0u ? 1 : 0;
         c->use_probe = (int)c->verdict[1];
+        c->use_ident = c->verdict[3] != 0u ? 1 : 0;
         c->verdict_pending = false;
     }
     return GMS_OK;
@@ -588,6 +640,7 @@
     switch (option) {
     case GMS_OPTION_DEAL: c->opt_deal = value; return GMS_OK;
     case GMS_OPTION_SCALE_PROBE: c->opt_probe = value; return GMS_OK;
+    case GMS_OPTION_IDENT: c->opt_ident = value; return GMS_OK;
     default: return GMS_ERR_BAD_ARG;
     }
 }
@@ -605,6 +658,8 @@
     case GMS_QUERY_PREFETCH_TYPE: *value = knobs().prefetch_type; return GMS_OK;
     case GMS_QUERY_PREFETCH_AHEAD: *value = knobs().prefetch_ahead > 0 ? knobs().prefetch_ahead : c->n_cus; return GMS_OK;
     case GMS_QUERY_STAGGER_TICKS: *value = c->last_stagger_ticks; return GMS_OK;
+    case GMS_QUERY_LAST_IDENT: *value = c->last_ident; return GMS_OK;
+    case GMS_QUERY_IDENT_MISSES: *value = (int64_t)((volatile uint32_t*)c->verdict)[4]; return GMS_OK;
     default: return GMS_ERR_BAD_ARG;
     }
 }
@@ -633,7 +688,22 @@
     if (!c || n_frames < 0 || total_kp < 0) return GMS_ERR_BAD_ARG;
     if (total_kp == 0 || n_frames == 0) return GMS_OK;
     if (!d_kp || !d_frame_off || !d_wh || !d_pts) return GMS_ERR_BAD_ARG;
-    return on_ctx(c, [&] { return gms::launch_normalize(d_kp, (int)sizeof(gms_keypoint), d_frame_off, d_wh, n_frames, total_kp, d_pts, c->stream); });
+    std::lock_guard<std::mutex> lock(c->mu);
+    GMS_HIP(hipSetDevice(c->device));
+    return build_frame_table(c, c->stream, d_kp, (int)sizeof(gms_keypoint), d_frame_off, d_wh, n_frames, total_kp, d_pts);
+}
+
+int gms_ctx_read_side_records(gms_ctx* c, void* dst, size_t dst_bytes, int* n_frames)
+{
+    static_assert(sizeof(gms::SideRecord) == GMS_SIDE_RECORD_BYTES, "the public size of a side record");
+    if (!c || !n_frames || (dst_bytes && !dst)) return GMS_ERR_BAD_ARG;
+    std::lock_guard<std::mutex> lock(c->mu);
+    GMS_HIP(hipSetDevice(c->device));
+    GMS_HIP(hipStreamSynchronize(c->stream));
+    *n_frames = c->side_stamp != 0 ? c->side_frames : 0;
+    const size_t bytes = std::min(dst_bytes, (size_t)*n_frames * sizeof(gms::SideRecord));
+    if (bytes) GMS_HIP(hipMemcpy(dst, c->side.p, bytes, hipMemcpyDeviceToHost));
+    return GMS_OK;
 }
 
 int gms_filter_device(gms_ctx* c, const float* d_pts, const int64_t* d_frame_off, int n_frames,
@@ -703,7 +773,7 @@
     const gms_pair* d_pair = (const gms_pair*)(din + offsetof(CallHeader, pair));
     gms_pair_result* d_res = (gms_pair_result*)dout;
     gms_dmatch* d_out = (gms_dmatch*)(dout + sizeof(gms_pair_result));
-    if (nkp) GMS_HIP(gms::launch_normalize(din + off_xy, 8, d_foff, d_wh, 2, (int64_t)nkp, (float*)c->tab_pts.p, st));
+    if (nkp) GMS_TRY(build_frame_table(c, st, din + off_xy, 8, d_foff, d_wh, 2, (int64_t)nkp, (float*)c->tab_pts.p));
     GMS_TRY(filter_launch(c, st, (const float*)c->tab_pts.p, d_foff, 2, d_pair, 1, m, (const gms_dmatch*)(din + off_m),
                           with_rotation, with_scale, threshold_factor, d_out, d_res, nullptr));
     if (!zero_copy) GMS_HIP(hipMemcpyAsync(L.hout.p, L.dout.p, sizeof(gms_pair_result), hipMemcpyDeviceToHost, st));
@@ -838,9 +908,9 @@
             pool.run(jobs);
             jobs.clear();
             GMS_HIP(hipMemcpyAsync(c->tab_kp.p, c->lane[0].hin.p, (size_t)total_kp * 8, hipMemcpyHostToDevice, st));
-            GMS_HIP(gms::launch_normalize(c->tab_kp.p, 8, (const int64_t*)c->tab_small.p,
-                                          (const int32_t*)((char*)c->tab_small.p + align16((size_t)(n_frames + 1) * 8)),
-                                          n_frames, total_kp, (float*)c->tab_pts.p, st));
+            GMS_TRY(build_frame_table(c, st, c->tab_kp.p, 8, (const int64_t*)c->tab_small.p,
+                                      (const int32_t*)((char*)c->tab_small.p + align16((size_t)(n_frames + 1) * 8)),
+                                      n_frames, total_kp, (float*)c->tab_pts.p));
         }
         GMS_HIP(hipStreamSynchronize(st));
     }
diff --git a/sfm-gms_amd/csrc/gms_kernel_dense.hip b/sfm-gms_amd/csrc/gms_kernel_dense.hip
--- a/sfm-gms_amd/csrc/gms_kernel_dense.hip
+++ b/sfm-gms_amd/csrc/gms_kernel_dense.hip
@@ -444,8 +444,12 @@
 static_assert(kDenseLdsBytes < (1u << 18), "an entry offset is 18 bits");
 constexpr uint32_t kPZeroByte = 3u;
 
-template <int KPT, int NT, bool DEALT>
-__device__ __forceinline__ bool dense_pair_plain(const FilterParams& p, uint32_t* smem, const int pair_idx, const int tid)
+constexpr int kPairGeneral = 0;
+constexpr int kPairDone = 1;
+constexpr int kPairNotIdent = 2;
+
+template <int KPT, int NT, bool DEALT, bool IDENT>
+__device__ __forceinline__ int dense_pair_plain(const FilterParams& p, uint32_t* smem, const int pair_idx, const int tid)
 {
     constexpr int kMcap = KPT * NT;
     constexpr int kChunk = (KPT % 5 == 0) ? 5 : 4;
@@ -459,15 +463,25 @@
     const int m_stride = dealt ? (NT / 64) * 8 : NT;
     auto match_of = [&](int k) -> int { return m_base + k * m_stride; };
 
-    if ((uint32_t)(uintptr_t)((lds_u32_t*)smem) != 0u) return false;
+    if ((uint32_t)(uintptr_t)((lds_u32_t*)smem) != 0u) return kPairGeneral;
 
     int64_t total_kp;
     const gms_pair pr = load_pair(p.pairs, pair_idx, p, total_kp);
     const int m = pr.m;
     if (p.with_scale || p.with_rotation || p.right_w[0] != kDenseRightW || p.right_h[0] != kDenseRightW || m <= 0 || m > kMcap ||
         pr.frame_a < 0 || pr.frame_a >= p.n_frames || pr.frame_b < 0 || pr.frame_b >= p.n_frames)
-        return false;
+        return kPairGeneral;
     const FrameRangeWords fr_words = request_frame_ranges(p.frame_off, pr.frame_a, pr.frame_b);
+    uint4 side_h0 = make_uint4(0, 0, 0, 0);
+    uint2 side_h1 = make_uint2(0, 0), tab_stamp = make_uint2(0, 0);
+    uint32_t side_hist = 0;
+    if constexpr (IDENT) {
+        const SideRecord* __restrict__ sr = p.side + min(pr.frame_a, p.side_frames - 1);
+        side_h0 = *reinterpret_cast<const uint4*>(sr);
+        side_h1 = *reinterpret_cast<const uint2*>(&sr->stamp);
+        tab_stamp = *reinterpret_cast<const uint2*>(total_kp >= 0 ? p.pts + 2 * total_kp : p.pts - 2);
+        side_hist = sr->hist[min(tid, kLeftN - 1)];
+    }
     const gms_dmatch* __restrict__ matches = p.matches + pr.match_off;
     constexpr int kKeep = KPT <= 10 ? KPT : (DEALT ? 10 : 12);
     uint4 rec[kKeep];
@@ -480,10 +494,21 @@
     int64_t offA, offB;
     int nA, nB;
     take_frame_ranges(fr_words, offA, nA, offB, nB);
-    if (nA <= 0 || nB <= 0) return false;
-    if (total_kp < 0 || offA + nA > total_kp || offB + nB > total_kp) return false;
+    if (nA <= 0 || nB <= 0) return kPairGeneral;
+    if (total_kp < 0 || offA + nA > total_kp || offB + nB > total_kp) return kPairGeneral;
     const uint16_t* __restrict__ lcodeA = reinterpret_cast<const uint16_t*>(p.pts + total_kp) + offA;
     const uint16_t* __restrict__ rcodeB = reinterpret_cast<const uint16_t*>(p.pts + total_kp) + total_kp + offB;
+    uint32_t side_flags = 0;
+    if constexpr (IDENT) {
+        asm volatile("" : "+v"(side_h0.x), "+v"(side_h0.y), "+v"(side_h0.z), "+v"(side_h0.w), "+v"(side_h1.x), "+v"(side_h1.y), "+v"(tab_stamp.x), "+v"(tab_stamp.y));
+        const int64_t side_off = (int64_t)(((uint64_t)(uint32_t)uniform((int)side_h0.y) << 32) | (uint32_t)uniform((int)side_h0.x));
+        const int side_n = uniform((int)side_h0.z);
+        side_flags = (uint32_t)uniform((int)side_h0.w);
+        const uint64_t s_side = ((uint64_t)(uint32_t)uniform((int)side_h1.y) << 32) | (uint32_t)uniform((int)side_h1.x);
+        const uint64_t s_tab = ((uint64_t)(uint32_t)uniform((int)tab_stamp.y) << 32) | (uint32_t)uniform((int)tab_stamp.x);
+        if (p.side_stamp == 0 || s_side == 0 || s_side != s_tab || side_off != offA || side_n != nA || m != nA)
+            return kPairNotIdent;
+    }
 
     uint32_t* nfine32 = smem + kDenseFineOff / 4;
     const uint8_t* nfine8 = reinterpret_cast<const uint8_t*>(nfine32);
@@ -496,20 +521,25 @@
 #endif
     if (tid < 32) misc[tid] = 0;
     if (tid < 16) trash[tid] = 0;
-    if (tid < kFineN / 4) nfine32[tid] = 0;
+    if (IDENT ? tid < kLeftN : tid < kFineN / 4) nfine32[tid] = IDENT ? side_hist : 0u;
 
     const uint32_t phA = (uint32_t)(reinterpret_cast<uintptr_t>(lcodeA) >> 1) & 7u, phB = (uint32_t)(reinterpret_cast<uintptr_t>(rcodeB) >> 1) & 7u;
-    const uint32_t qA = (phA + (uint32_t)nA + 7u) >> 3, qB = (phB + (uint32_t)nB + 7u) >> 3;
+    const uint32_t qA = IDENT ? 0u : (phA + (uint32_t)nA + 7u) >> 3, qB = (phB + (uint32_t)nB + 7u) >> 3;
     const bool staged = (qA + qB) * 16u <= kDenseBytes;
     const uint4* __restrict__ srcA = reinterpret_cast<const uint4*>(lcodeA - phA);
     const uint4* __restrict__ srcB = reinterpret_cast<const uint4*>(rcodeB - phB);
-    constexpr int kStageRegs = 3;
+    constexpr int kStageRegs = IDENT ? 2 : 3;
     uint4 tb[kStageRegs];
 #pragma unroll
     for (int i = 0; i < kStageRegs; ++i) {
         const uint32_t j = min((uint32_t)(i * NT + tid), qA + qB - 1u);
         const uint4* src = j < qA ? srcA + j : srcB + (j - qA);
         tb[i] = *src;
+    }
+    uint32_t ca_id[IDENT ? KPT : 1];
+    if constexpr (IDENT) {
+#pragma unroll
+        for (int k = 0; k < KPT; ++k) ca_id[k] = lcodeA[min(match_of(k), nA - 1)];
     }
     auto query_of = [&](int k) -> uint32_t { return k < kKeep ? rec[k < kKeep ? k : 0].x : qt[k < kKeep ? 0 : k - kKeep].x; };
     auto train_of = [&](int k) -> uint32_t { return k < kKeep ? rec[k < kKeep ? k : 0].y : qt[k < kKeep ? 0 : k - kKeep].y; };
@@ -530,6 +560,19 @@
         for (uint32_t j = kStageRegs * NT + tid; j < qA + qB; j += NT) d4[j] = *(j < qA ? srcA + j : srcB + (j - qA));
     }
     const uint32_t ldsA = 2u * phA, ldsB = 16u * qA + 2u * phB;
+    constexpr uint32_t kLeftNone = 0xFFFFFFFFu;
+    uint32_t lw[IDENT ? KPT : 1];
+    bool moved = false;
+    if constexpr (IDENT) {
+#pragma unroll
+        for (int k = 0; k < KPT; ++k) {
+            const uint32_t c = ca_id[k], cell = c >> kLCellShift;
+            const bool live = match_of(k) < m;
+            const uint32_t qe = (c & 21u) | ((c >> 4) & kPEdgeX) | ((c >> 3) & kPEdgeY);
+            lw[k] = (live & (cell < kLCellNever)) ? ((__umul24(cell, kDenseRow) << kPAtShift) | qe) : kLeftNone;
+            moved |= live & (query_of(k) != (uint32_t)match_of(k));
+        }
+    }
     __syncthreads();
 #ifdef GMS_PHASE_TIMING
     asm volatile("s_waitcnt vmcnt(0)" ::: "memory");
@@ -541,14 +584,22 @@
     const uint32_t cw_sink = (kDenseTrashOff + 4u * (uint32_t)(lane & 15)) << kPAtShift;
     {
         uint32_t ca[KPT], cb[KPT];
+        if constexpr (IDENT) {
+#pragma unroll
+            for (int k = 0; k < KPT; ++k) ca[k] = 0;
+        }
         if (staged) {
-#pragma unroll
-            for (int k = 0; k < KPT; ++k) ca[k] = ldsa_ld16(ldsA + 2u * min(query_of(k), (uint32_t)(nA - 1)));
+            if constexpr (!IDENT) {
+#pragma unroll
+                for (int k = 0; k < KPT; ++k) ca[k] = ldsa_ld16(ldsA + 2u * min(query_of(k), (uint32_t)(nA - 1)));
+            }
 #pragma unroll
             for (int k = 0; k < KPT; ++k) cb[k] = ldsa_ld16(ldsB + 2u * min(train_of(k), (uint32_t)(nB - 1)));
         } else {
-#pragma unroll
-            for (int k = 0; k < KPT; ++k) ca[k] = lcodeA[min(query_of(k), (uint32_t)(nA - 1))];
+            if constexpr (!IDENT) {
+#pragma unroll
+                for (int k = 0; k < KPT; ++k) ca[k] = lcodeA[min(query_of(k), (uint32_t)(nA - 1))];
+            }
 #pragma unroll
             for (int k = 0; k < KPT; ++k) cb[k] = rcodeB[min(train_of(k), (uint32_t)(nB - 1))];
         }
@@ -556,17 +607,25 @@
         asm volatile("s_waitcnt vmcnt(0) lgkmcnt(0)" ::: "memory");
         GMS_STAMP(12);
 #endif
-        bool any_bad = false, spill = false;
+        bool any_bad = IDENT && (side_flags & kSideBadLeft) != 0u, spill = false;
 #pragma unroll
         for (int k = 0; k < KPT; ++k) {
             const bool live = match_of(k) < m;
             const uint32_t e0 = cb[k] & kDEMask;
             const uint32_t cell = ca[k] >> kLCellShift;
-            const bool ok = ((int)(query_of(k) < (uint32_t)nA) & (int)(train_of(k) < (uint32_t)nB) & (int)(cell != kLCellBad) & (int)((cb[k] & kRCodeBad) == 0u) & (int)(e0 != 0u)) != 0;
-            const bool binned = live & ok & (cell < kLCellNever);
-            const uint32_t sh = ((ca[k] & 1u) << 3) | ((ca[k] & 4u) << 2);
-            const uint32_t old = ldsa_add_rtn(binned ? kDenseFineOff + 4u * cell : kDenseTrashOff + 4u * (uint32_t)(lane & 7), 1u << sh);
-            spill |= binned & (((old >> sh) & 255u) == 255u);
+            bool ok, binned;
+            if constexpr (IDENT) {
+                ok = ((int)(train_of(k) < (uint32_t)nB) & (int)((cb[k] & kRCodeBad) == 0u) & (int)(e0 != 0u)) != 0;
+                any_bad |= live & !ok;
+                code[k] = (ok & (lw[k] != kLeftNone)) ? lw[k] + __umul24(e0, (1u << kPAtShift) | (1u << kPEShift)) : cw_sink;
+                continue;
+            } else {
+                ok = ((int)(query_of(k) < (uint32_t)nA) & (int)(train_of(k) < (uint32_t)nB) & (int)(cell != kLCellBad) & (int)((cb[k] & kRCodeBad) == 0u) & (int)(e0 != 0u)) != 0;
+                binned = live & ok & (cell < kLCellNever);
+                const uint32_t sh = ((ca[k] & 1u) << 3) | ((ca[k] & 4u) << 2);
+                const uint32_t old = ldsa_add_rtn(binned ? kDenseFineOff + 4u * cell : kDenseTrashOff + 4u * (uint32_t)(lane & 7), 1u << sh);
+                spill |= binned & (((old >> sh) & 255u) == 255u);
+            }
             any_bad |= live & !ok;
             const uint32_t qe = (ca[k] & 21u) | ((ca[k] >> 4) & kPEdgeX) | ((ca[k] >> 3) & kPEdgeY);
             const uint32_t at1 = __umul24(cell, kDenseRow) + e0;
@@ -574,6 +633,7 @@
         }
         if (any_bad) misc[8] = 1;
         if (spill) misc[13] = 1;
+        if (IDENT && moved) misc[10] = 1;
     }
     GMS_STAMP(13);
     __syncthreads();
@@ -587,11 +647,15 @@
     }
     __syncthreads();
     GMS_STAMP(2);
+    if (IDENT && misc[10] != 0) {
+        __syncthreads();
+        return kPairNotIdent;
+    }
     if (misc[8] != 0) {
         __syncthreads();
-        return false;
-    }
-    const bool spilled = misc[13] != 0;
+        return kPairGeneral;
+    }
+    const bool spilled = IDENT ? (side_flags & kSideSpill) != 0u : misc[13] != 0;
 
     const bool thr_fast = threshold_fast_ok(p.threshold_factor);
     const uint32_t f2i = dense_factor_sq(p.threshold_factor);
@@ -624,8 +688,10 @@
         const uint32_t key_tag = (uint32_t)g << kDTagShift;
         const uint32_t nl_cur = kDenseFineOff + (uint32_t)(g & 1) * (kLeftN * 2u);
         if (!CROWDED && g == p.prefetch_type && pf_lines) {
-            if ((uint32_t)tid < pf_lines) pf_sink = pf_base[32u * (uint32_t)tid];
-            if ((uint32_t)tid + NT < pf_lines) pf_sink2 = pf_base[32u * ((uint32_t)tid + NT)];
+            uint32_t pt = (uint32_t)tid;
+            if constexpr (IDENT && KPT > 10) asm volatile("" : "+v"(pt));
+            if (pt < pf_lines) pf_sink = pf_base[32u * pt];
+            if (pt + NT < pf_lines) pf_sink2 = pf_base[32u * (pt + NT)];
         }
         if (!CROWDED && tid < kLeftN) {
             const uint32_t n = dense_nleft_cm(nfine8, tid % kLeftW, tid / kLeftW, gx, gy);
@@ -750,7 +816,7 @@
     }
     if (status != 0) {
         __syncthreads();
-        return false;
+        return kPairGeneral;
     }
     GMS_STAMP(7);
     if (p.prefetch_type == 4 && pf_lines) {
@@ -900,18 +966,29 @@
         r.status = GMS_OK;
         p.results[pair_idx] = r;
     }
-    return true;
+    return kPairDone;
 }
 
-template <int KPT, bool ROT, int NT, bool DEALT>
+template <int KPT, bool ROT, int NT, bool DEALT, bool IDENT>
 __global__ void __launch_bounds__(NT)
 filter_kernel_dense(FilterParams p)
 {
+    static_assert(!(ROT && IDENT), "the identity-query body is dense_pair_plain's");
     extern __shared__ __attribute__((aligned(16))) uint32_t smem[];
     first_round_stagger(p);
     bool done;
-    if constexpr (ROT) done = dense_pair_rot<KPT, NT, DEALT>(p, smem, (int)blockIdx.x, (int)threadIdx.x);
-    else done = dense_pair_plain<KPT, NT, DEALT>(p, smem, (int)blockIdx.x, (int)threadIdx.x);
+    if constexpr (ROT) {
+        done = dense_pair_rot<KPT, NT, DEALT>(p, smem, (int)blockIdx.x, (int)threadIdx.x);
+    } else {
+        int r = dense_pair_plain<KPT, NT, DEALT, IDENT>(p, smem, (int)blockIdx.x, (int)threadIdx.x);
+        if constexpr (IDENT) {
+            if (r == kPairNotIdent) {
+                if (threadIdx.x == 0 && p.ident_misses) atomicAdd(p.ident_misses, 1u);
+                r = dense_pair_plain<KPT, NT, DEALT, false>(p, smem, (int)blockIdx.x, (int)threadIdx.x);
+            }
+        }
+        done = r == kPairDone;
+    }
     if (!done) hash_pair<KPT, ROT, NT>(p, smem, (int)blockIdx.x, (int)threadIdx.x);
 }
 
@@ -945,8 +1022,15 @@
     return dispatch_kpt_rot(kpt, p.with_rotation != 0, [&](auto k, auto rot) {
         constexpr int KPT = decltype(k)::value;
         constexpr bool ROT = decltype(rot)::value;
-        if (p.dealt) hipLaunchKernelGGL((filter_kernel_dense<KPT, ROT, kThreads, true>), dim3((unsigned)n_pairs), dim3(kThreads), lds, stream, p);
-        else hipLaunchKernelGGL((filter_kernel_dense<KPT, ROT, kThreads, false>), dim3((unsigned)n_pairs), dim3(kThreads), lds, stream, p);
+        if constexpr (!ROT) {
+            if (p.ident && p.side != nullptr && p.side_frames >= 1 && p.side_stamp != 0) {
+                if (p.dealt) hipLaunchKernelGGL((filter_kernel_dense<KPT, false, kThreads, true, true>), dim3((unsigned)n_pairs), dim3(kThreads), lds, stream, p);
+                else hipLaunchKernelGGL((filter_kernel_dense<KPT, false, kThreads, false, true>), dim3((unsigned)n_pairs), dim3(kThreads), lds, stream, p);
+                return hipGetLastError();
+            }
+        }
+        if (p.dealt) hipLaunchKernelGGL((filter_kernel_dense<KPT, ROT, kThreads, true, false>), dim3((unsigned)n_pairs), dim3(kThreads), lds, stream, p);
+        else hipLaunchKernelGGL((filter_kernel_dense<KPT, ROT, kThreads, false, false>), dim3((unsigned)n_pairs), dim3(kThreads), lds, stream, p);
         return hipGetLastError();
     });
 }
@@ -956,8 +1040,13 @@
     return for_each_kpt_rot([](auto k, auto rot) {
         constexpr int KPT = decltype(k)::value;
         constexpr bool ROT = decltype(rot)::value;
-        const hipError_t e = allow_full_lds(filter_kernel_dense<KPT, ROT, kThreads, false>);
-        return e != hipSuccess ? e : allow_full_lds(filter_kernel_dense<KPT, ROT, kThreads, true>);
+        hipError_t e = allow_full_lds(filter_kernel_dense<KPT, ROT, kThreads, false, false>);
+        if (e == hipSuccess) e = allow_full_lds(filter_kernel_dense<KPT, ROT, kThreads, true, false>);
+        if constexpr (!ROT) {
+            if (e == hipSuccess) e = allow_full_lds(filter_kernel_dense<KPT, false, kThreads, false, true>);
+            if (e == hipSuccess) e = allow_full_lds(filter_kernel_dense<KPT, false, kThreads, true, true>);
+        }
+        return e;
     });
 }
 
diff --git a/sfm-gms_amd/csrc/gms_kernels.h b/sfm-gms_amd/csrc/gms_kernels.h
--- a/sfm-gms_amd/csrc/gms_kernels.h
+++ b/sfm-gms_amd/csrc/gms_kernels.h
@@ -16,6 +16,19 @@
 
 constexpr uint32_t kTableMagic0 = 0x46534D47u, kTableMagic1 = 0x31424154u;
 constexpr int kTableHeaderBytes = 16;
+
+struct SideRecord {
+    int64_t off;
+    int32_t n;
+    uint32_t flags;
+    uint64_t stamp;
+    uint32_t pad[2];
+    uint32_t hist[400];
+};
+static_assert(sizeof(SideRecord) == 1632 && sizeof(SideRecord) % 16 == 0, "side records are read in uint4s");
+constexpr uint32_t kSideBadLeft = 1u;
+constexpr uint32_t kSideSpill = 2u;
+constexpr size_t kSideMaxBytes = (size_t)64 << 20;
 
 struct FilterParams {
     const float2* pts;
@@ -41,6 +54,11 @@
     uint32_t* overflow_events;
     int prefetch_type, prefetch_ahead;
     int dense;
+    int ident;
+    int side_frames;
+    const SideRecord* side;
+    uint64_t side_stamp;
+    uint32_t* ident_misses;
     double threshold_factor;
     int right_w[5], right_h[5];
 #ifdef GMS_PHASE_TIMING
@@ -56,14 +74,14 @@
 int        filter_region_shift(int kpt);
 size_t     filter_lds_bytes(int kpt, uint32_t table_slots);
 hipError_t launch_normalize(const void* d_kp, int kp_stride_bytes, const int64_t* d_frame_off, const int32_t* d_wh,
-                            int n_frames, int64_t total_kp, float* d_pts, hipStream_t stream);
+                            int n_frames, int64_t total_kp, float* d_pts, SideRecord* d_side, uint64_t stamp, hipStream_t stream);
 hipError_t launch_filter(const FilterParams& p, int kpt, int n_pairs, hipStream_t stream);
 hipError_t launch_filter_hash(const FilterParams& p, int kpt, int n_pairs, size_t lds_bytes, hipStream_t stream);
 hipError_t launch_filter_dense(const FilterParams& p, int kpt, int n_pairs, size_t lds_bytes, hipStream_t stream);
 hipError_t init_hash_kernels();
 hipError_t init_dense_kernels();
 hipError_t init_scales_kernels();
-hipError_t launch_order_probe(const FilterParams& p, uint32_t* flag, hipStream_t stream);
+hipError_t launch_order_probe(const FilterParams& p, uint32_t* flag, uint32_t* ident_flag, hipStream_t stream);
 hipError_t launch_probe_verdict(uint32_t* stats, uint32_t* flag, hipStream_t stream);
 hipError_t launch_check_pairs(const gms_pair* d_pairs, int n_pairs, gms_pair_result* d_results, uint32_t* d_flag, hipStream_t stream);
 hipError_t launch_filter_scales(const FilterParams& p, int kpt, int n_pairs, hipStream_t stream);
diff --git a/sfm-gms_amd/csrc/gms_kernels.hip b/sfm-gms_amd/csrc/gms_kernels.hip
--- a/sfm-gms_amd/csrc/gms_kernels.hip
+++ b/sfm-gms_amd/csrc/gms_kernels.hip
@@ -27,13 +27,16 @@
 
 __global__ void __launch_bounds__(256)
 normalize_kernel(const char* __restrict__ kp, int kp_stride, const int64_t* __restrict__ frame_off,
-                 const int32_t* __restrict__ wh, int n_frames, int64_t total, float2* __restrict__ pts)
+                 const int32_t* __restrict__ wh, int n_frames, int64_t total, float2* __restrict__ pts, uint64_t stamp)
 {
     if (blockIdx.x == 0 && threadIdx.x == 0) {
         uint32_t* h = reinterpret_cast<uint32_t*>(pts) - kTableHeaderBytes / 4;
         h[0] = kTableMagic0;
         h[1] = kTableMagic1;
         *reinterpret_cast<int64_t*>(h + 2) = total;
+        uint64_t* tail = reinterpret_cast<uint64_t*>(pts + 2 * total);
+        tail[0] = stamp;
+        tail[1] = 0;
     }
     uint16_t* __restrict__ lcode = reinterpret_cast<uint16_t*>(pts + total);
     uint16_t* __restrict__ rcode = lcode + total;
@@ -61,12 +64,82 @@
     }
 }
 
+__device__ __forceinline__ uint64_t mix64(uint64_t x)
+{
+    x += 0x9E3779B97F4A7C15ull;
+    x = (x ^ (x >> 30)) * 0xBF58476D1CE4E5B9ull;
+    x = (x ^ (x >> 27)) * 0x94D049BB133111EBull;
+    return x ^ (x >> 31);
+}
+
 __global__ void __launch_bounds__(1024)
-order_probe_kernel(FilterParams p, uint32_t* __restrict__ flag)
-{
-    __shared__ uint32_t s_same, s_seen;
+side_records_kernel(const int64_t* __restrict__ frame_off, int64_t total, const float2* __restrict__ pts, uint64_t stamp,
+                    SideRecord* __restrict__ side)
+{
+    __shared__ uint32_t s_hist[kLeftN];
+    __shared__ uint32_t s_flags;
+    __shared__ unsigned long long s_sum;
+    const int tid = (int)threadIdx.x, f = (int)blockIdx.x;
+    if (tid < kLeftN) s_hist[tid] = 0;
+    if (tid == 0) s_flags = 0;
+    if (tid == 0) s_sum = 0;
+    __syncthreads();
+    const int64_t off = frame_off[f], end = frame_off[f + 1];
+    const bool inside = off >= 0 && end >= off && end <= total && end - off <= (int64_t)0x7FFFFFFF;
+    const int n = inside ? (int)(end - off) : 0;
+    const uint16_t* __restrict__ lcode = reinterpret_cast<const uint16_t*>(pts + total) + (inside ? off : 0);
+    uint32_t flags = 0;
+    uint64_t sum = 0;
+    for (int i = tid; i < n; i += 1024) {
+        const uint32_t c = lcode[i];
+        sum += mix64(((uint64_t)(uint32_t)i << 16) | c);
+        const uint32_t cell = c >> kLCellShift;
+        if (cell == kLCellBad) flags |= kSideBadLeft;
+        if (cell < (uint32_t)kLeftN) {
+            const uint32_t sh = ((c & 1u) << 3) | ((c & 4u) << 2);
+            const uint32_t old = atomicAdd(&s_hist[cell], 1u << sh);
+            if (((old >> sh) & 255u) == 255u) flags |= kSideSpill;
+        }
+    }
+    if (flags) atomicOr(&s_flags, flags);
+    if (sum) atomicAdd(&s_sum, (unsigned long long)sum);
+    __syncthreads();
+    SideRecord* __restrict__ r = side + f;
+    if (tid < kLeftN) r->hist[tid] = s_hist[tid];
+    if (tid == 0) {
+        r->off = off;
+        r->n = inside ? n : -1;
+        r->flags = s_flags;
+        r->stamp = stamp != 0 ? (uint64_t)s_sum : 0;
+        r->pad[0] = r->pad[1] = 0;
+    }
+}
+
+__global__ void __launch_bounds__(1024)
+table_stamp_kernel(SideRecord* __restrict__ side, int n_frames, int64_t total, float2* __restrict__ pts)
+{
+    __shared__ unsigned long long s_sum;
+    const int tid = (int)threadIdx.x;
+    if (tid == 0) s_sum = 0;
+    __syncthreads();
+    uint64_t sum = 0;
+    for (int f = tid; f < n_frames; f += 1024) {
+        const SideRecord& r = side[f];
+        sum += mix64(r.stamp ^ mix64(((uint64_t)(uint32_t)f << 32) ^ (uint64_t)r.off) ^ mix64(0x5157ull + (uint64_t)(uint32_t)r.n));
+    }
+    if (sum) atomicAdd(&s_sum, (unsigned long long)sum);
+    __syncthreads();
+    const uint64_t stamp = mix64((uint64_t)s_sum ^ (uint64_t)total) | 1ull;
+    for (int f = tid; f < n_frames; f += 1024) side[f].stamp = stamp;
+    if (tid == 0) *reinterpret_cast<uint64_t*>(pts + 2 * total) = stamp;
+}
+
+__global__ void __launch_bounds__(1024)
+order_probe_kernel(FilterParams p, uint32_t* __restrict__ flag, uint32_t* __restrict__ ident_flag)
+{
+    __shared__ uint32_t s_same, s_seen, s_not_ident;
     const int tid = (int)threadIdx.x, lane = tid & 63, wave = tid >> 6;
-    if (tid == 0) s_same = s_seen = 0;
+    if (tid == 0) s_same = s_seen = s_not_ident = 0;
     __syncthreads();
     const int pi = (int)(((long long)wave * p.n_pairs) >> 4);
     const gms_pair pr = p.pairs[pi];
@@ -82,13 +155,18 @@
         const uint32_t cell = lc >= kLCellNever ? 0x10000u + (uint32_t)lane : lc;
         const uint32_t next = (uint32_t)__shfl_down((int)cell, 1);
         const unsigned long long same = __ballot(lane < 63 && cell == next);
+        const unsigned long long moved = __ballot(q != (uint32_t)(start + lane));
         if (lane == 0) {
             atomicAdd(&s_same, (uint32_t)__popcll(same));
             atomicAdd(&s_seen, 63u);
-        }
-    }
-    __syncthreads();
-    if (tid == 0 && s_seen != 0) *flag = 4u * s_same > s_seen ? 1u : 0u;
+            if (moved != 0ull || pr.m != nA) atomicAdd(&s_not_ident, 1u);
+        }
+    }
+    __syncthreads();
+    if (tid == 0 && s_seen != 0) {
+        *flag = 4u * s_same > s_seen ? 1u : 0u;
+        *ident_flag = s_not_ident == 0u ? 1u : 0u;
+    }
 }
 
 size_t filter_lds_bytes(int kpt, uint32_t table_slots)
@@ -225,22 +303,27 @@
     return hipGetLastError();
 }
 
-hipError_t launch_order_probe(const FilterParams& p, uint32_t* flag, hipStream_t stream)
+hipError_t launch_order_probe(const FilterParams& p, uint32_t* flag, uint32_t* ident_flag, hipStream_t stream)
 {
     if (p.n_pairs <= 0) return hipSuccess;
-    hipLaunchKernelGGL(order_probe_kernel, dim3(1), dim3(1024), 0, stream, p, flag);
+    hipLaunchKernelGGL(order_probe_kernel, dim3(1), dim3(1024), 0, stream, p, flag, ident_flag);
     return hipGetLastError();
 }
 
 hipError_t launch_normalize(const void* d_kp, int kp_stride_bytes, const int64_t* d_frame_off, const int32_t* d_wh,
-                            int n_frames, int64_t total_kp, float* d_pts, hipStream_t stream)
+                            int n_frames, int64_t total_kp, float* d_pts, SideRecord* d_side, uint64_t stamp, hipStream_t stream)
 {
     if (total_kp <= 0) return hipSuccess;
     int64_t blocks = (total_kp + 255) / 256;
     if (blocks > 8192) blocks = 8192;
+    float2* pts = reinterpret_cast<float2*>(reinterpret_cast<char*>(d_pts) + kTableHeaderBytes);
+    if (d_side == nullptr || n_frames <= 0) stamp = 0;
     hipLaunchKernelGGL(normalize_kernel, dim3((unsigned)blocks), dim3(256), 0, stream, reinterpret_cast<const char*>(d_kp),
-                       kp_stride_bytes, d_frame_off, d_wh, n_frames, total_kp,
-                       reinterpret_cast<float2*>(reinterpret_cast<char*>(d_pts) + kTableHeaderBytes));
+                       kp_stride_bytes, d_frame_off, d_wh, n_frames, total_kp, pts, (uint64_t)0);
+    if (stamp != 0) {
+        hipLaunchKernelGGL(side_records_kernel, dim3((unsigned)n_frames), dim3(1024), 0, stream, d_frame_off, total_kp, pts, stamp, d_side);
+        hipLaunchKernelGGL(table_stamp_kernel, dim3(1), dim3(1024), 0, stream, d_side, n_frames, total_kp, pts);
+    }
     return hipGetLastError();
 }
 
```

Result: faster. 12.01 million (median of 6 runs) (+4.5%).
